# fx-erick/uncertainty-vit

Hardware: AMD Instinct MI355X
Metric: pretrain images/sec (ViT-B/16 224, bs=128/GPU) (higher is better)
Workload: dtype bf16

## Files before the change

### include/uvit.h

```cpp
#ifndef UVIT_H
#define UVIT_H
#include <stddef.h>
#include <stdint.h>

#ifdef __cplusplus
extern "C" {
#endif

#define UVIT_VERSION 100
#define UVIT_MAX_DEPTH 64

typedef struct uvit_engine uvit_engine;
typedef void* uvit_stream;

typedef struct uvit_config {
    int32_t img_size, patch_size, in_chans, embed_dim, depth, num_heads, mlp_hidden;
    int32_t use_shared_rel_pos_bias;
    int32_t use_abs_pos_emb;
    int32_t batch;
    float ln_eps;
    float attn_drop_rate;
    float drop_path_rate;
    int32_t bias_chunk;
    int32_t two_stream;
// ... 3 lines not shown
    char name[96];
    int64_t offset;
    int64_t numel;
    int32_t ndim;
    int32_t decay;
    int64_t shape[4];
} uvit_layout_entry;

typedef struct uvit_buffers {
    float* params;
    float* grads;
    float* adam_m;
    float* adam_v;
    float* ema;
    void* params_bf16;
    void* params_bf16_t;
    void* ema_bf16;
    const int32_t* rel_index;
    void* workspace;
    int64_t workspace_bytes;
} uvit_buffers;

typedef struct uvit_step_params {
    int32_t target_layers[UVIT_MAX_DEPTH];
    int32_t n_target_layers;
    int32_t target_layer_norm_last;
    int32_t post_target_layer_norm;
    int32_t l2_loss;
    float l1_beta;
    float loss_scale;
    float clip_grad;
    float lr, weight_decay, beta1, beta2, eps;
    int32_t opt_step;
    float ema_decay;
    int32_t do_ema;
    float grad_scale;
    uint32_t seed;
    uint32_t it;
    int32_t train_dropout;
    float lambda_pretraining;
    const float* sched_dev;
    int32_t sched_len, sched_index;
    int32_t layer_results_fc;
    float var_w0, var_margin0;
    int32_t target_batch_norm, target_instance_norm, post_target_instance_norm;
    int32_t n_rows_hint;
} uvit_step_params;

int uvit_version(void);
const char* uvit_source_hash(void);

int uvit_layout_count(const uvit_config* cfg);
int uvit_layout_get(const uvit_config* cfg, int index, uvit_layout_entry* out);
int64_t uvit_arena_numel(const uvit_config* cfg, int64_t* n_decay_out);
int64_t uvit_workspace_bytes(const uvit_config* cfg);

uvit_engine* uvit_engine_create(const uvit_config* cfg, const uvit_buffers* bufs, uvit_stream stream, int* err_out);
void uvit_engine_destroy(uvit_engine* e);

int uvit_engine_sync_shadows(uvit_engine* e, int which, uvit_stream stream);

int uvit_engine_forward_features(uvit_engine* e, int which, const float* images, const int64_t* mask, int batch,
                                 int train_dropout, uint32_t seed, uint32_t it, uvit_stream stream);
int uvit_engine_forward_tail(uvit_engine* e, int which, int batch, int first_layer, int train_dropout, uint32_t seed, uint32_t it,
                             uvit_stream stream);
int uvit_engine_head(uvit_engine* e, int which, int all_tokens, float* out, int32_t* count_dev, uvit_stream stream);

void* uvit_engine_ws_ptr(uvit_engine* e, const char* name, int layer);
int uvit_engine_compact_rows(uvit_engine* e);

int uvit_step_begin(uvit_engine* e, const float* images, const int64_t* mask, const uvit_step_params* hp,
                    uvit_stream stream);
int uvit_step_backward_layer(uvit_engine* e, int layer, const uvit_step_params* hp, uvit_stream stream);
int uvit_step_wait_layer_grads(uvit_engine* e, int layer, uvit_stream stream);
int uvit_step_backward_embed(uvit_engine* e, uvit_stream stream);
int uvit_step_update(uvit_engine* e, const uvit_step_params* hp, uvit_stream stream);
int uvit_train_step(uvit_engine* e, const float* images, const int64_t* mask, const uvit_step_params* hp,
                    uvit_stream stream);
typedef struct uvit_tuning { int32_t nt_variant, tn_variant, tn_split_target, wgrad_group_chunks, nt_group, nt_persist; } uvit_tuning;
void uvit_tuning_default(uvit_tuning* out);
int uvit_engine_set_tuning(uvit_engine* e, const uvit_tuning* t);
int uvit_engine_set_streams(uvit_engine* e, int dual);
int uvit_engine_set_drop_path_rows(uvit_engine* e, int on);
int uvit_drop_path_kept_counts(int depth, float drop_path_rate, int draws_per_block, int batch, uint32_t seed, uint32_t it, int32_t* out);
int uvit_engine_profile(uvit_engine* e, int enable, int max_launches);
int uvit_engine_profile_read(uvit_engine* e, double* total_ms, int* launches, double* flops_per_launch);
int uvit_engine_profile_read_kind(uvit_engine* e, int kind, double* total_ms, int* launches, double* flops_per_launch,
                                  double* bytes_per_launch);
int uvit_engine_read_stats_async(uvit_engine* e, float* host_out2, uvit_stream stream);
int uvit_engine_read_stats(uvit_engine* e, float* host_out2, uvit_stream stream);

typedef struct uvit_gemm_epilogue {
    void* out; void* out2; const float* bias; const float* bias2; const float* gamma; const float* resid;
    const float* rowscale; const void* aux; const int64_t* mask; const float* mask_token;
    int32_t ldo, tokens, patches;
    int32_t row0;
} uvit_gemm_epilogue;
enum { UVIT_EPI_BF16 = 0, UVIT_EPI_QKV = 1, UVIT_EPI_GELU = 2, UVIT_EPI_RESID = 3, UVIT_EPI_F32 = 4,
       UVIT_EPI_PATCH = 5, UVIT_EPI_DGELU = 6, UVIT_EPI_QKV_ELU = 7,
       UVIT_EPI_GELU_DG = 8,
       UVIT_EPI_MULAUX = 9 };

int uvit_op_gemm_nt(int mode, const void* A_bf16, const void* W_bf16, int M, int N, int K, int lda, int ldw,
                    const uvit_gemm_epilogue* epi, uvit_stream stream);
int uvit_op_gemm_nt_tuned(int mode, const void* A_bf16, const void* W_bf16, int M, int N, int K, int lda, int ldw,
                          const uvit_gemm_epilogue* epi, const uvit_tuning* tune, int* tail_rows, uvit_stream stream);
typedef struct uvit_gemm_nt_plan_info { int32_t kernel, rows, grid, tail_rows; } uvit_gemm_nt_plan_info;
int uvit_op_gemm_nt_plan(int mode, int M, int N, int K, int lda, int ldw, int ldo, int row_list,
                         const uvit_tuning* tuning, int num_cu, uvit_gemm_nt_plan_info* out);
int uvit_op_gemm_nt_sched(int mode, const void* A_bf16, const void* W_bf16, int M, int N, int K, int lda, int ldw,
                          const uvit_gemm_epilogue* epi, const uvit_tuning* tune, uint32_t* tile_counters, uvit_stream stream);
int uvit_op_gemm_tn(const void* Y_bf16, const void* X_bf16, int M, int N, int K, int ldy, int ldx, float* C, int ldc,
                    const uvit_tuning* tune, uvit_stream stream);
typedef struct uvit_wgrad_problem {
    const void* Y_bf16; const void* X_bf16; float* C; float* bias; float* bias2;
    int32_t bias_end, bias2_begin, M, N, K, ldy, ldx, ldc;
} uvit_wgrad_problem;
int uvit_op_wgrad_group(const uvit_wgrad_problem* problems, int count, const uvit_tuning* tune, uvit_stream stream);
int uvit_op_attn_fwd(const void* qkv, const float* biasP, void* out, float* lse, int B, int H, int N, int NP,
                     float scale, float p_drop, uint32_t seed, uint32_t layer, uvit_stream stream);
int64_t uvit_op_attn_bwd_ws_bytes(int B, int H, int N);
int uvit_op_attn_bwd(const void* qkv, const void* o_fwd, const void* d_o, const float* biasP, const float* lse,
                           float* delta, void* dqkv, float* dbias_slab, int accumulate_slab, void* ds_workspace, int B, int H,
                           int N, int NP, float scale, float p_drop, uint32_t seed, uint32_t layer, uvit_stream stream);
int uvit_op_attn_fwd_hd(const void* qkv, const float* biasP, void* out, float* lse, int B, int H, int N, int NP, int head_dim,
                        float scale, float p_drop, uint32_t seed, uint32_t layer, uvit_stream stream);
int uvit_op_attn_bwd_hd(const void* qkv, const void* o_fwd, const void* d_o, const float* biasP, const float* lse,
                        float* delta, void* dqkv, float* dbias_slab, int accumulate_slab, void* ds_workspace, int B, int H,
                        int N, int NP, int head_dim, float scale, float p_drop, uint32_t seed, uint32_t layer, uvit_stream stream);
int uvit_op_attn2_fwd(const void* qkv_m, const void* qkv_c, const float* biasP, void* out_m, void* out_c, float* lse, int B, int H,
                      int N, int NP, float scale, float p_drop, uint32_t seed, uint32_t layer, uvit_stream stream);
int64_t uvit_op_attn2_bwd_ws_bytes(int B, int H, int N);
int uvit_op_attn2_bwd(const void* qkv_m, const void* qkv_c, const void* o_m, const void* o_c, const void* d_m, const void* d_c,
                      const float* biasP, const float* lse, float* delta, void* dqkv_m, void* dqkv_c, float* dbias_slab,
                      int accumulate_slab, void* ds_workspace, int B, int H, int N, int NP, float scale, float p_drop, uint32_t seed,
                      uint32_t layer, uvit_stream stream);
int uvit_op_relpos_gather(const float* table, const int32_t* index, float* biasP, int H, int N, int NP, uvit_stream stream);
int uvit_op_relpos_scatter(const float* slab, int nslab, const int32_t* index, float* dtable, int H, int N, int NP,
                           uvit_stream stream);
int uvit_op_ln_fwd(const float* x, const float* w, const float* b, void* y_bf16, float* mean, float* rstd, int M, int C,
                   float eps, uvit_stream stream);
int uvit_op_ln_bwd(const void* dy_bf16, const float* x, const float* mean, const float* rstd, const float* w,
                   const float* dres, float* dx, float* dw, float* db, int M, int C, uvit_stream stream);
int uvit_op_ln_fwd_walk(const float* x, const float* w, const float* b, void* y_bf16, float* mean, float* rstd, int M, int C,
                        float eps, const int32_t* rowidx, const int32_t* count, const int32_t* pos, float* xcopy, int tokens,
                        uvit_stream stream);
typedef struct uvit_ls_rider {
    const void* y; const float* gamma; const float* rowscale; void* dy; float* dgamma; float* dbias;
    int32_t tokens; const int32_t* pos; const int32_t* cnt; int32_t pad_base; void* pad2; int32_t pad2_cols;
} uvit_ls_rider;
int uvit_op_ln_bwd_walk(const void* dy_bf16, const float* x, const float* mean, const float* rstd, const float* w, const float* dres,
                        float* dx, float* dw, float* db, int M, int C, int nrep, int64_t rep_stride, const int32_t* rowidx,
                        const int32_t* count, const int32_t* pos, const uvit_ls_rider* next, uvit_stream stream);
int uvit_op_ls_bwd(const float* dx, const uvit_ls_rider* rider, int M, int C, int nrep, int64_t rep_stride, const int32_t* rowidx,
                   const int32_t* count, uvit_stream stream);
int uvit_op_colsum(const void* y_bf16, int ld, int col0, int ncols, int M, float* out, int nrep, int64_t rep_stride, uvit_stream stream);
int uvit_op_reduce_replicas(const float* rep, float* out, int64_t n, int nrep, int64_t stride, uvit_stream stream);
int uvit_op_droppath_lists(const float* scales, int32_t* pos, int32_t* bmap, int32_t* rows, int32_t* cnt, int nlists, int B, int tokens,
                           int rows_stride, const int32_t* host_counts, uvit_stream stream);
int uvit_op_gemm_nt_rows(int mode, const void* A_bf16, const void* W_bf16, int M, int N, int K, int lda, int ldw,
                         const uvit_gemm_epilogue* epi, const int32_t* rowmap, const int32_t* rowcount, const uvit_tuning* tune,
                         uvit_stream stream);
typedef struct uvit_wgrad_split { float* bias_s1; float* bias2_s1; int32_t s1_row; } uvit_wgrad_split;
int uvit_op_wgrad_group_split(const uvit_wgrad_problem* problems, const uvit_wgrad_split* split, int count, const uvit_tuning* tune,
                              uvit_stream stream);
int uvit_op_token_bwd(const float* dx, const int64_t* mask, void* dpatch_bf16, float* dcls, float* dmask_token, int B, int P, int C,
                      uvit_stream stream);
typedef struct uvit_transpose_desc { const void* src; void* dst; int32_t rows, cols, tile0, pad; } uvit_transpose_desc;
int uvit_op_transpose_batch(const uvit_transpose_desc* descs_dev, int ndesc, int total_tiles, uvit_stream stream);
int uvit_op_ema(float* ema, const float* params, void* ema_bf16, int64_t n, float decay, uvit_stream stream);
int uvit_op_sumsq(const float* g, int64_t n, double* out, uvit_stream stream);
int uvit_op_adamw(float* p, const float* g, float* m, float* v, void* p_bf16, int64_t n, int64_t n_decay, float lr,
                  float wd, float b1, float b2, float eps, int step, const double* sumsq, float max_norm,
                  float grad_scale, float* gnorm_out, uvit_stream stream);
int uvit_op_smooth_l1(const float* out, const float* target, const int32_t* count_dev, float beta, int l2,
                      float loss_scale, float* loss, void* dout_bf16, int Mmax, int C, uvit_stream stream);
int uvit_op_wasserstein_loss(const float* out_m, const float* out_c, const float* tgt_m, const float* tgt_c,
                             const int32_t* count_dev, float lam, float loss_scale, float* scratch, float* loss,
                             void* dout_m_bf16, void* dout_c_bf16, int Mmax, int C, uvit_stream stream);
int uvit_op_target_accum(const float* x, const int32_t* rowidx, const int32_t* count, float* acc, int first, int Mmax,
                         int C, float eps, uvit_stream stream);
int uvit_op_variance_loss(const float* out, const int32_t* count_dev, float w, float margin, float loss_scale, float* scratch,
                          float* loss, float* std_loss0_out, void* dout_bf16, int Mmax, int C, uvit_stream stream);
int uvit_op_target_finalize(float* acc, const int32_t* count, int n_layers, int post_ln, int Mmax, int C, float eps,
                            uvit_stream stream);
int uvit_op_mask_compact(const int64_t* mask, int32_t* rowidx, int32_t* count, int B, int P, uvit_stream stream);
int uvit_op_synth_batch(float* images, int64_t* mask, int B, int chans, int img_size, int patches, int n_mask, uint32_t seed,
                        uint32_t it, uvit_stream stream);
int uvit_op_im2col(const float* img, void* cols_bf16, int B, int Cin, int img_size, int patch, uvit_stream stream);
int uvit_op_droppath(float* scales, const float* rates_dev, int depth, int B, uint32_t seed, uint32_t step,
                     uvit_stream stream);
int uvit_op_cast_bf16(const float* src, void* dst_bf16, int64_t n, uvit_stream stream);

#define UVIT_AUG_LANCZOS 1
#define UVIT_AUG_BILINEAR 2
#define UVIT_AUG_BICUBIC 3
#define UVIT_AUG_HAMMING 5
#define UVIT_AUG_BRIGHTNESS 0
#define UVIT_AUG_CONTRAST 1
#define UVIT_AUG_SATURATION 2
typedef struct uvit_augment_desc {
    int64_t offset;
    int32_t h, w;
    int32_t flip;
    int32_t crop_x, crop_y, crop_w, crop_h;
    int32_t resize_w, resize_h;
    int32_t win_x, win_y;
    int32_t filter;
    int32_t n_jitter;
    int32_t jitter_op[3];
    float jitter_factor[3];
    int32_t reserved;
// ... 116 lines not shown
```

### uncertainty-vit_amd/csrc/attention.hip

```cpp
#include <mutex>
#include <type_traits>
#include "attn_common.h"
#include "uvit_internal.h"

#define IMG_PIECES (ROWS_PAD / 8)

#define TAIL_BYTES (ROWS_PAD * 32)
#define TAIL_PIECES (ROWS_PAD / 32)
__device__ __forceinline__ int tail_off(int row, int slot) { return row * 32 + ((slot ^ ((row >> 2) & 2)) << 3); }

__device__ __forceinline__ void dma_tail32(char* tail, int rb, const bf16* src, size_t stride, int n_valid, int lane) {
    const int row = 32 * rb + (lane >> 1);
    const int half = (lane & 1) ^ ((row >> 3) & 1);
    const int r = row < n_valid ? row : n_valid - 1;
    __builtin_amdgcn_global_load_lds(GLB_PTR(void, src + (size_t)r * stride + 64 + half * 8), LDS_PTR(void, tail + rb * 1024), 16, 0, 0);
}

__device__ __forceinline__ bf16x8 tail_row(const char* tail, int row, int g) {
    const bf16x8 v = *(const bf16x8*)(tail + row * 32 + (((g & 1) ^ ((row >> 3) & 1)) << 4));
    const bf16x8 z = {};
    return g < 2 ? v : z;
}
__device__ __forceinline__ bf16x8 col_frag_tail(const char* tail, int r_lo, int r_hi, int lane) {
    const int g = lane >> 4, q = (lane >> 2) & 3, p = lane & 3;
    const s16x4 lo = __builtin_amdgcn_ds_read_tr16_b64_v4i16(LDS_PTR(s16x4, tail + tail_off(r_lo + 4 * g + q, p)));
    const s16x4 hi = __builtin_amdgcn_ds_read_tr16_b64_v4i16(LDS_PTR(s16x4, tail + tail_off(r_hi + 4 * g + q, p)));
    typedef __attribute__((ext_vector_type(8))) short s16x8;
    const s16x8 v = {lo[0], lo[1], lo[2], lo[3], hi[0], hi[1], hi[2], hi[3]};
    return __builtin_bit_cast(bf16x8, v);
}

#ifdef ATTN_DEBUG
extern "C" int uvit_debug_attn_fwd(const void* qkv, const float* biasP, void* out, float* lse, int B, int H, int N, int NP, float scale,
                                   float p_drop, void* stream) {
    return uvit_attn_fwd_launch(qkv, biasP, out, lse, B, H, N, NP, scale, p_drop, 1u, 0u, (hipStream_t)stream, nullptr);
}
#endif

template <int HDK, int NW, bool HAS_BIAS>
__global__ __launch_bounds__(NW * 64, 4)
void attn_fwd_kernel(const bf16* __restrict__ qkv, const float* __restrict__ biasP, bf16* __restrict__ out,
                     float* __restrict__ lse, int H, int N, int NP, float scale, uint32_t drop_thr,
                     float inv_keep, uint32_t drop_key, int ncu, const int* __restrict__ bmap) {
    constexpr int NDT = HDK / 16;
    extern __shared__ __attribute__((aligned(16))) char smem[];
    char* kimg = smem;
    char* vimg = smem + IMG_BYTES;
    char* ktail = smem + 2 * IMG_BYTES;
    char* vtail = ktail + TAIL_BYTES;
    const int tid = threadIdx.x, lane = tid & 63, wave = __builtin_amdgcn_readfirstlane(tid >> 6);
    const int g = lane >> 4, li = lane & 15;
    const int bh = blockIdx.x, b = bh / H, h = bh - b * H;
    const int C = H * HDK;
    const size_t ld = 3 * (size_t)C;
    const bf16* base = qkv + (size_t)b * N * ld + h * HDK;
    const uint32_t bh_rng = (uint32_t)__builtin_amdgcn_readfirstlane(bmap ? bmap[b] * H + h : bh);
    if (blockIdx.x >= (unsigned)ncu && blockIdx.x < 2u * (unsigned)ncu) __builtin_amdgcn_s_sleep(127);
    bf16x8 qn[2];
    if constexpr (HDK == 64) {
        const int q0 = wave * 16 + li, qr0 = q0 < N ? q0 : N - 1;
        qn[0] = *(const bf16x8*)(base + (size_t)qr0 * ld + g * 8);
        qn[1] = *(const bf16x8*)(base + (size_t)qr0 * ld + 32 + g * 8);
    }
    for (int p = wave; p < 2 * IMG_PIECES; p += NW) {
        const int img = p / IMG_PIECES, rb = p - img * IMG_PIECES;
        dma_rows8(smem + img * IMG_BYTES, rb, base + (size_t)(1 + img) * C, ld, 0, N, lane);
    }
    if constexpr (HDK == 80) {
        for (int p = wave; p < 2 * TAIL_PIECES; p += NW) {
            const int img = p / TAIL_PIECES, rb = p - img * TAIL_PIECES;
            dma_tail32(ktail + img * TAIL_BYTES, rb, base + (size_t)(1 + img) * C, ld, N, lane);
        }
    }
    asm volatile("s_waitcnt vmcnt(0)" ::: "memory");
    if constexpr (HDK == 64) { landed(qn[0]); landed(qn[1]); }
    __syncthreads();
    const int nt = (N + 15) >> 4, nt2 = (nt + 1) >> 1;

    for (int qt = wave; qt < nt; qt += NW) {
        const int q = qt * 16 + li;
        bf16x8 qf[2], qtf;
        if constexpr (HDK == 64) {
            qf[0] = qn[0]; qf[1] = qn[1];
        } else {
            const int qr = q < N ? q : N - 1;
            qf[0] = *(const bf16x8*)(base + (size_t)qr * ld + g * 8);
            qf[1] = *(const bf16x8*)(base + (size_t)qr * ld + 32 + g * 8);
            const bf16x8 qt0 = *(const bf16x8*)(base + (size_t)qr * ld + 64 + 8 * (g & 1)), qz = {};
            qtf = g < 2 ? qt0 : qz;
        }
        float s[NT_MAX][4];
#pragma unroll
        for (int t = 0; t < NT_MAX; ++t) {
            if constexpr (HAS_BIAS) {
                if (t < nt) {
                    const float4 bv = *(const float4*)(biasP + ((size_t)h * NP + q) * NP + t * 16 + 4 * g);
                    s[t][0] = bv.x; s[t][1] = bv.y; s[t][2] = bv.z; s[t][3] = bv.w;
                }
            }
        }
        if constexpr (HDK == 64) {
            if (qt + NW < nt) {
                const int q1 = (qt + NW) * 16 + li, qr1 = q1 < N ? q1 : N - 1;
                qn[0] = *(const bf16x8*)(base + (size_t)qr1 * ld + g * 8);
                qn[1] = *(const bf16x8*)(base + (size_t)qr1 * ld + 32 + g * 8);
            }
        }
        float mx = NEG_BIG;
        const float c = scale * LOG2E;
#pragma unroll
        for (int t = 0; t < NT_MAX; ++t) {
            if (t < nt) {
                f32x4 a = {0.f, 0.f, 0.f, 0.f};
                a = __builtin_amdgcn_mfma_f32_16x16x32_bf16(row_frag(kimg, t * 16 + li, g), qf[0], a, 0, 0, 0);
                a = __builtin_amdgcn_mfma_f32_16x16x32_bf16(row_frag(kimg, t * 16 + li, 4 + g), qf[1], a, 0, 0, 0);
                if constexpr (HDK == 80) a = __builtin_amdgcn_mfma_f32_16x16x32_bf16(tail_row(ktail, t * 16 + li, g), qtf, a, 0, 0, 0);
#pragma unroll
                for (int r = 0; r < 4; ++r) {
                    float bb;
                    if constexpr (HAS_BIAS) bb = s[t][r]; else bb = (t * 16 + 4 * g + r) < N ? 0.f : NEG_BIG;
                    const float v = a[r] * c + bb;
                    s[t][r] = v;
                    mx = fmaxf(mx, v);
                }
            } else {
#pragma unroll
                for (int r = 0; r < 4; ++r) s[t][r] = 0.f;
            }
        }
        mx = group_max4(mx);
        float sum = 0.f;
#pragma unroll
        for (int t = 0; t < NT_MAX; ++t) {
            if (t < nt) {
#pragma unroll
                for (int r = 0; r < 4; ++r) {
                    const float p = __builtin_amdgcn_exp2f(s[t][r] - mx);
                    s[t][r] = p;
                    sum += p;
                }
            }
        }
        sum = group_sum4(sum);
        if (g == 0 && q < N) lse[(size_t)bh * N + q] = mx + __builtin_amdgcn_logf(sum);
        f32x4 o[NDT];
#pragma unroll
        for (int dt = 0; dt < NDT; ++dt) o[dt] = f32x4{0.f, 0.f, 0.f, 0.f};
        const uint32_t rowpair = (bh_rng * N + q) * (uint32_t)(NP >> 1);
#pragma unroll
        for (int ks = 0; ks < (NT_MAX + 1) / 2; ++ks) {
            if (ks < nt2) {
                const int t0 = 2 * ks, t1 = 2 * ks + 1;
                float pa[4], pb[4];
#pragma unroll
                for (int r = 0; r < 4; ++r) { pa[r] = s[t0][r]; pb[r] = t1 < NT_MAX ? s[t1 < NT_MAX ? t1 : 0][r] : 0.f; }
                if (drop_thr) {
                    bool k4[4];
                    keep4(drop_key, rowpair, t0 * 16 + 4 * g, drop_thr, k4);
#pragma unroll
                    for (int r = 0; r < 4; ++r) pa[r] = k4[r] ? pa[r] : 0.f;
                    keep4(drop_key, rowpair, t1 * 16 + 4 * g, drop_thr, k4);
#pragma unroll
                    for (int r = 0; r < 4; ++r) pb[r] = k4[r] ? pb[r] : 0.f;
                }
                const bf16x8 pf = pack8(pa, pb);
#pragma unroll
                for (int dt = 0; dt < 4; ++dt) {
                    const bf16x8 vf = col_frag(vimg, t0 * 16, t1 * 16, dt * 16, lane);
                    o[dt] = __builtin_amdgcn_mfma_f32_16x16x32_bf16(vf, pf, o[dt], 0, 0, 0);
                }
                if constexpr (HDK == 80)
                    o[4] = __builtin_amdgcn_mfma_f32_16x16x32_bf16(col_frag_tail(vtail, t0 * 16, t1 * 16, lane), pf, o[4], 0, 0, 0);
            }
        }
        if constexpr (HDK == 64) {
            asm volatile("s_waitcnt vmcnt(0)" ::: "memory");
            landed(qn[0]); landed(qn[1]);
        }
        if (q < N) {
            const float f = inv_keep / sum;
            bf16* dst = out + ((size_t)b * N + q) * C + h * HDK + 4 * g;
#pragma unroll
            for (int dt = 0; dt < NDT; ++dt) {
                bf16x4 v = {f2bf(o[dt][0] * f), f2bf(o[dt][1] * f), f2bf(o[dt][2] * f), f2bf(o[dt][3] * f)};
                *(bf16x4*)(dst + dt * 16) = v;
            }
        }
    }
}

#define FB_WAVES 13
#define FB_ROWS (NT_MAX * 16)
#ifdef ATTN_STAMP
__device__ unsigned long long g_attn_stamps[2048 * 2 * 16 * 2];
#define ASTAMP(k) do { unsigned long long t_; asm volatile("s_memtime %0\n\ts_waitcnt lgkmcnt(0)" : "=s"(t_) :: "memory"); \
        if (lane == 0 && (wave == 0 || wave == 8) && blockIdx.x < 2048) g_attn_stamps[(blockIdx.x * 2 + (wave >> 3)) * 16 + (k)] = t_; } while (0)
#define BSTAMP(k) do { if (i == 3) { unsigned long long t_; asm volatile("s_memtime %0\n\ts_waitcnt lgkmcnt(0)" : "=s"(t_) :: "memory"); \
        if (lane == 0 && (wave == 0 || wave == 8) && blockIdx.x < 2048) g_attn_stamps[2048 * 32 + (blockIdx.x * 2 + (wave >> 3)) * 16 + (k)] = t_; } } while (0)
#define ASTAMP_ID() do { if (lane == 0 && wave == 0 && blockIdx.x < 2048) \
        g_attn_stamps[blockIdx.x * 32 + 15] = __builtin_amdgcn_s_getreg(4 | (31 << 11)) | ((unsigned long long)__builtin_amdgcn_s_getreg(20 | (31 << 11)) << 32); } while (0)
extern "C" int uvit_debug_attn_stamps(unsigned long long* host_out) {
    return hipMemcpyFromSymbol(host_out, HIP_SYMBOL(g_attn_stamps), sizeof(g_attn_stamps)) == hipSuccess ? 0 : -3;
}
extern "C" int uvit_debug_attn_bwd_fused(const void* qkv, const void* o, const void* d_o, const float* biasP, const float* lse, float* delta,
                                         void* dqkv, void* ds_ws, float* slab, int B, int H, int N, float p_drop, void* stream) {
    (void)slab;
    return uvit_attn_bwd_fused_launch(qkv, o, d_o, biasP, lse, delta, dqkv, ds_ws, ds_ws != nullptr, B, H, N, 208, 0.125f, p_drop, 1u, 0u, (hipStream_t)stream, nullptr);
}
#else
#define ASTAMP(k)
#define BSTAMP(k)
#define ASTAMP_ID()
#endif
#define FB_IMG (FB_ROWS * 128)
#define FB_SB (FB_ROWS * 64)

constexpr int fb_lds(int hd) { return hd == 80 ? 4 * FB_IMG + 4 * TAIL_BYTES + 2 * FB_SB : 4 * FB_IMG + 4 * FB_SB; }

__device__ __forceinline__ int sb_off(int q, int slot) {
    const int f = (((q >> 2) & 1) << 2) | (((q >> 3) & 1) << 1) | ((q >> 1) & 1);
    return q * 64 + ((slot ^ f) << 3);
}
__device__ __forceinline__ bf16x8 sb_col_frag(const char* sb, int r_lo, int r_hi, int tt, bool has_hi, int lane) {
    const int g = lane >> 4, q = (lane >> 2) & 3, p = lane & 3;
    const s16x4 lo = __builtin_amdgcn_ds_read_tr16_b64_v4i16(LDS_PTR(s16x4, sb + sb_off(r_lo + 4 * g + q, 4 * tt + p)));
    s16x4 hi = __builtin_amdgcn_ds_read_tr16_b64_v4i16(LDS_PTR(s16x4, sb + sb_off(r_hi + 4 * g + q, 4 * tt + p)));
    if (!has_hi) hi = s16x4{0, 0, 0, 0};
    typedef __attribute__((ext_vector_type(8))) short s16x8;
    const s16x8 v = {lo[0], lo[1], lo[2], lo[3], hi[0], hi[1], hi[2], hi[3]};
    return __builtin_bit_cast(bf16x8, v);
}

template <int HDK, bool HAS_BIAS, int NT_C>
__global__ __launch_bounds__(FB_WAVES * 64)
void attn_bwd_fused_kernel(const bf16* __restrict__ qkv, const bf16* __restrict__ o_fwd, const bf16* __restrict__ d_o,
                           const float* __restrict__ biasP, const float* __restrict__ lse, float* __restrict__ delta,
                           bf16* __restrict__ dqkv, bf16* __restrict__ ds_out, int H, int N, int NP, float scale,
                           uint32_t drop_thr, float inv_keep, uint32_t drop_key, const int* __restrict__ bmap) {
    constexpr int NDT = HDK / 16;
    constexpr int BW = 2 * NDT;
    extern __shared__ __attribute__((aligned(16))) char smem[];
    char* const kimg = smem;
    char* const vimg = smem + FB_IMG;
    char* const qimg = smem + 2 * FB_IMG;
    char* const doimg = smem + 3 * FB_IMG;
    char* const ktail = smem + 4 * FB_IMG;
    char* const vtail = ktail + TAIL_BYTES;
    char* const qtail = ktail + 2 * TAIL_BYTES;
    char* const dotail = ktail + 3 * TAIL_BYTES;
    char* const pbuf = smem + 4 * FB_IMG + 4 * TAIL_BYTES;
    char* const dbuf = pbuf + FB_SB;
    const int tid = threadIdx.x, lane = tid & 63, wave = __builtin_amdgcn_readfirstlane(tid >> 6);
    const int g = lane >> 4, li = lane & 15;
    const int bh = blockIdx.x, b = bh / H, h = bh - b * H;
    const int C = H * HDK;
    const size_t ld = 3 * (size_t)C;
    const int nt = NT_C ? NT_C : (N + 15) >> 4;
    const int nsteps = (nt + 1) >> 1;
    const bf16* base = qkv + (size_t)b * N * ld + h * HDK;
    const bf16* dobase = d_o + (size_t)b * N * C + h * HDK;
    const bool active = NT_C ? true : wave < nt;
    const int q = wave * 16 + li, qr = q < N ? q : N - 1;
    ASTAMP(0); ASTAMP_ID();

    for (int p = wave; p < 4 * (FB_ROWS / 8); p += FB_WAVES) {
        int img, rb;
        if (p < 2 * (FB_ROWS / 8)) { img = p & 1; rb = p >> 1; } else { img = 2 + (p >= 3 * (FB_ROWS / 8)); rb = p - img * (FB_ROWS / 8); }
        if (rb * 8 >= nt * 16) continue;
        if (img == 3) dma_rows8(doimg, rb, dobase, (size_t)C, 0, N, lane);
        else dma_rows8(smem + img * FB_IMG, rb, base + (img == 2 ? 0 : (size_t)(1 + img) * C), ld, 0, N, lane);
    }
    if constexpr (HDK == 80) {
        for (int p = wave; p < 4 * TAIL_PIECES; p += FB_WAVES) {
            const int img = p / TAIL_PIECES, rb = p - img * TAIL_PIECES;
            if (rb * 32 >= nt * 16) continue;
            if (img == 3) dma_tail32(dotail, rb, dobase, (size_t)C, N, lane);
            else dma_tail32(ktail + img * TAIL_BYTES, rb, base + (img == 2 ? 0 : (size_t)(1 + img) * C), ld, N, lane);
        }
    }
    float dl = 0.f, lse_q = 1e30f;
    if (active) {
        const size_t orow = ((size_t)b * N + qr) * C + h * HDK;
#pragma unroll
        for (int kk = 0; kk < 2; ++kk) {
            const bf16x8 dof = *(const bf16x8*)(d_o + orow + kk * 32 + g * 8);
            const bf16x8 of = *(const bf16x8*)(o_fwd + orow + kk * 32 + g * 8);
#pragma unroll
            for (int j = 0; j < 8; ++j) dl += bf2f(dof[j]) * bf2f(of[j]);
        }
        if constexpr (HDK == 80) {
            const bf16x4 dof = *(const bf16x4*)(d_o + orow + 64 + g * 4);
            const bf16x4 of = *(const bf16x4*)(o_fwd + orow + 64 + g * 4);
#pragma unroll
            for (int j = 0; j < 4; ++j) dl += bf2f(dof[j]) * bf2f(of[j]);
        }
        dl = group_sum4(dl);
        if (q < N) {
            lse_q = lse[(size_t)bh * N + q];
            if (g == 0) delta[(size_t)bh * N + q] = dl;
        }
    }
    const uint32_t bh_rng = (uint32_t)__builtin_amdgcn_readfirstlane(bmap ? bmap[b] * H + h : bh);
    const uint32_t rowpair = (bh_rng * N + q) * (uint32_t)(NP >> 1);
    const float cs = scale * LOG2E;
    const float* brow = HAS_BIAS ? biasP + ((size_t)h * NP + (q < NP ? q : NP - 1)) * NP + 4 * g : nullptr;
    float4 bnext[2];
    auto bias_fetch = [&](int i) {
#pragma unroll
        for (int tt = 0; tt < 2; ++tt) {
            const int t = 2 * i + tt;
            if constexpr (HAS_BIAS) {
                bnext[tt] = (t < nt && active) ? *(const float4*)(brow + t * 16) : make_float4(NEG_BIG, NEG_BIG, NEG_BIG, NEG_BIG);
            } else {
                const int k0 = t * 16 + 4 * g;
                bnext[tt] = make_float4(k0 < N ? 0.f : NEG_BIG, k0 + 1 < N ? 0.f : NEG_BIG, k0 + 2 < N ? 0.f : NEG_BIG, k0 + 3 < N ? 0.f : NEG_BIG);
            }
        }
    };
    bias_fetch(0);
    asm volatile("s_waitcnt vmcnt(0)" ::: "memory");
    ASTAMP(1);
    __syncthreads();
    ASTAMP(2);

    f32x4 dq[NDT];
#pragma unroll
    for (int dt = 0; dt < NDT; ++dt) dq[dt] = f32x4{0.f, 0.f, 0.f, 0.f};
    const int pj = HDK == 64 ? wave >> 2 : wave / 5, dtj = HDK == 64 ? wave & 3 : wave - 5 * pj;

    enum { A_COMPUTE = 1, A_FINISH = 2 };
    float step_p[2][4], step_ds[2][4];
    auto A_step = [&](int i, auto parts, float (&pdv)[2][4], float (&dsv)[2][4]) {
        char* pb = HDK == 64 ? smem + 4 * FB_IMG + (i & 1) * FB_SB : pbuf;
        char* db = HDK == 64 ? pb + 2 * FB_SB : dbuf;
        const int t0 = 2 * i;
        const bool has1 = t0 + 1 < nt;
        if constexpr (decltype(parts)::value & A_COMPUTE) {
            const float4 bcur[2] = {bnext[0], bnext[1]};
            if (i + 1 < nsteps) bias_fetch(i + 1);
            BSTAMP(4);
            bool k4[2][4] = {{true, true, true, true}, {true, true, true, true}};
#ifndef ATTN_HAZARD_DEMO
            if (drop_thr) {
                keep4(drop_key, rowpair, t0 * 16 + 4 * g, drop_thr, k4[0]);
                keep4(drop_key, rowpair, t0 * 16 + 16 + 4 * g, drop_thr, k4[1]);
            }
#endif
            BSTAMP(5);
            const int row0 = t0 * 16 + li, row1 = (has1 ? t0 + 1 : t0) * 16 + li;
            f32x4 sacc[2], dp[2];
            {
                const bf16x8 k00 = row_frag(kimg, row0, g), k01 = row_frag(kimg, row0, 4 + g);
                const bf16x8 k10 = row_frag(kimg, row1, g), k11 = row_frag(kimg, row1, 4 + g);
                const bf16x8 qf0 = row_frag(qimg, q, g), qf1 = row_frag(qimg, q, 4 + g);
                const f32x4 z = {0.f, 0.f, 0.f, 0.f};
                sacc[0] = __builtin_amdgcn_mfma_f32_16x16x32_bf16(k00, qf0, z, 0, 0, 0);
                sacc[1] = __builtin_amdgcn_mfma_f32_16x16x32_bf16(k10, qf0, z, 0, 0, 0);
                sacc[0] = __builtin_amdgcn_mfma_f32_16x16x32_bf16(k01, qf1, sacc[0], 0, 0, 0);
                sacc[1] = __builtin_amdgcn_mfma_f32_16x16x32_bf16(k11, qf1, sacc[1], 0, 0, 0);
                if constexpr (HDK == 80) {
                    const bf16x8 qt = tail_row(qtail, q, g);
                    sacc[0] = __builtin_amdgcn_mfma_f32_16x16x32_bf16(tail_row(ktail, row0, g), qt, sacc[0], 0, 0, 0);
                    sacc[1] = __builtin_amdgcn_mfma_f32_16x16x32_bf16(tail_row(ktail, row1, g), qt, sacc[1], 0, 0, 0);
                }
            }
            __builtin_amdgcn_sched_barrier(0);
            BSTAMP(6);
            {
                const bf16x8 v00 = row_frag(vimg, row0, g), v01 = row_frag(vimg, row0, 4 + g);
                const bf16x8 v10 = row_frag(vimg, row1, g), v11 = row_frag(vimg, row1, 4 + g);
                const bf16x8 do0 = row_frag(doimg, q, g), do1 = row_frag(doimg, q, 4 + g);
                const f32x4 z = {0.f, 0.f, 0.f, 0.f};
                dp[0] = __builtin_amdgcn_mfma_f32_16x16x32_bf16(v00, do0, z, 0, 0, 0);
                dp[1] = __builtin_amdgcn_mfma_f32_16x16x32_bf16(v10, do0, z, 0, 0, 0);
                dp[0] = __builtin_amdgcn_mfma_f32_16x16x32_bf16(v01, do1, dp[0], 0, 0, 0);
                dp[1] = __builtin_amdgcn_mfma_f32_16x16x32_bf16(v11, do1, dp[1], 0, 0, 0);
                if constexpr (HDK == 80) {
                    const bf16x8 dot = tail_row(dotail, q, g);
                    dp[0] = __builtin_amdgcn_mfma_f32_16x16x32_bf16(tail_row(vtail, row0, g), dot, dp[0], 0, 0, 0);
                    dp[1] = __builtin_amdgcn_mfma_f32_16x16x32_bf16(tail_row(vtail, row1, g), dot, dp[1], 0, 0, 0);
                }
            }
            BSTAMP(7);
#ifdef ATTN_HAZARD_DEMO
            if (drop_thr) {
                keep4(drop_key, rowpair, t0 * 16 + 4 * g, drop_thr, k4[0]);
                keep4(drop_key, rowpair, t0 * 16 + 16 + 4 * g, drop_thr, k4[1]);
            }
#endif
#pragma unroll
            for (int tt = 0; tt < 2; ++tt) {
                const float bb[4] = {bcur[tt].x, bcur[tt].y, bcur[tt].z, bcur[tt].w};
#pragma unroll
                for (int r = 0; r < 4; ++r) {
                    const float p = __builtin_amdgcn_exp2f(sacc[tt][r] * cs + bb[r] - lse_q);
                    const float pd = k4[tt][r] ? p * inv_keep : 0.f;
                    pdv[tt][r] = pd;
                    dsv[tt][r] = pd * dp[tt][r] - p * dl;
                }
            }
        }
        if constexpr (decltype(parts)::value & A_FINISH) {
#pragma unroll
            for (int tt = 0; tt < 2; ++tt) {
                if (tt == 0 || has1) {
                    const bf16x4 pv = {f2bf(pdv[tt][0]), f2bf(pdv[tt][1]), f2bf(pdv[tt][2]), f2bf(pdv[tt][3])};
                    const bf16x4 dv = {f2bf(dsv[tt][0]), f2bf(dsv[tt][1]), f2bf(dsv[tt][2]), f2bf(dsv[tt][3])};
                    *(bf16x4*)(pb + sb_off(q, 4 * tt + g)) = pv;
                    *(bf16x4*)(db + sb_off(q, 4 * tt + g)) = dv;
                }
            }
            const bf16x8 dsf = pack8(dsv[0], dsv[1]);
            __builtin_amdgcn_sched_barrier(0);
            BSTAMP(8);
#pragma unroll
            for (int dt = 0; dt < 4; ++dt) {
                const bf16x8 kt = col_frag(kimg, t0 * 16, has1 ? t0 * 16 + 16 : t0 * 16, dt * 16, lane);
                dq[dt] = __builtin_amdgcn_mfma_f32_16x16x32_bf16(kt, dsf, dq[dt], 0, 0, 0);
            }
            if constexpr (HDK == 80)
                dq[4] = __builtin_amdgcn_mfma_f32_16x16x32_bf16(col_frag_tail(ktail, t0 * 16, has1 ? t0 * 16 + 16 : t0 * 16, lane),
                                                                 dsf, dq[4], 0, 0, 0);
            BSTAMP(9);
        }
    };

    auto B_step = [&](int i) {
        const char* pb = HDK == 64 ? smem + 4 * FB_IMG + (i & 1) * FB_SB : pbuf;
        const char* sb = pj ? (HDK == 64 ? pb + 2 * FB_SB : dbuf) : pb;
        const char* img = pj ? qimg : doimg;
        const char* timg = pj ? qtail : dotail;
        const bool has1 = 2 * i + 1 < nt;
        f32x4 acc[2] = {f32x4{0.f, 0.f, 0.f, 0.f}, f32x4{0.f, 0.f, 0.f, 0.f}};
        auto kstep = [&](int ks, auto is_tail) {
            const bool hk = 2 * ks + 1 < nt;
            const int r_lo = 32 * ks, r_hi = hk ? r_lo + 16 : r_lo;
            bf16x8 a;
            if constexpr (decltype(is_tail)::value) a = col_frag_tail(timg, r_lo, r_hi, lane);
            else a = col_frag(img, r_lo, r_hi, dtj * 16, lane);
            const bf16x8 b0 = sb_col_frag(sb, r_lo, r_hi, 0, hk, lane);
            const bf16x8 b1 = sb_col_frag(sb, r_lo, r_hi, 1, hk, lane);
            acc[0] = __builtin_amdgcn_mfma_f32_16x16x32_bf16(a, b0, acc[0], 0, 0, 0);
            acc[1] = __builtin_amdgcn_mfma_f32_16x16x32_bf16(a, b1, acc[1], 0, 0, 0);
        };
        auto kloop = [&](auto is_tail) {
            if constexpr (NT_C != 0) {
#pragma unroll
                for (int ks = 0; ks < (NT_C + 1) / 2; ++ks) kstep(ks, is_tail);
            } else {
                for (int ks = 0; ks < nsteps; ++ks) kstep(ks, is_tail);
            }
        };
        if constexpr (HDK == 80) {
            if (dtj == 4) kloop(std::true_type{});
            else kloop(std::false_type{});
        } else if constexpr (NT_C != 0) {
#pragma unroll
            for (int ks = 0; ks < (NT_C + 1) / 2; ++ks) kstep(ks, std::false_type{});
        } else {
            for (int ks = 0; ks < nsteps; ++ks) kstep(ks, std::false_type{});
        }
        HAZARD_PAD();
        char* dst = pj ? kimg : vimg;
        char* tdst = pj ? ktail : vtail;
        const float sc = pj ? scale : 1.0f;
#pragma unroll
        for (int tt = 0; tt < 2; ++tt) {
            if (tt == 0 || has1) {
                const int row = 32 * i + 16 * tt + li;
                const bf16x4 v = {f2bf(acc[tt][0] * sc), f2bf(acc[tt][1] * sc), f2bf(acc[tt][2] * sc), f2bf(acc[tt][3] * sc)};
                if (HDK == 80 && dtj == 4) *(bf16x4*)(tdst + tail_off(row, g)) = v;
                else *(bf16x4*)(dst + img_off(row, 2 * dtj + (g >> 1)) + ((g & 1) << 3)) = v;
            }
        }
    };
    auto store_rows = [&](int i, int sw) {
        for (int c = sw; c < 2 * NDT; c += FB_WAVES - BW) {
            if (HDK == 80 && c >= 8) {
                const int img = c - 8, row = 32 * i + (lane >> 1), hl = lane & 1;
// ... 38 lines not shown
            if (i > 0) stream_ds(i - 1, sw);
            BSTAMP(2);
            if constexpr (HDK == 64) if (i < nsteps && active) A_step(i, Both{}, step_p, step_ds);
        }
        if constexpr (HDK == 80) {
            if (i < nsteps && active) A_step(i, Compute{}, step_p, step_ds);
            asm volatile("s_waitcnt lgkmcnt(0)" ::: "memory");
            __builtin_amdgcn_s_barrier();
            asm volatile("" ::: "memory");
            if (i < nsteps && active) A_step(i, Finish{}, step_p, step_ds);
        }
        asm volatile("s_waitcnt lgkmcnt(0)" ::: "memory");
        BSTAMP(10);
        __builtin_amdgcn_s_barrier();
        asm volatile("" ::: "memory");
        BSTAMP(11);
        ASTAMP(3 + i);
    }
    if (wave >= BW) store_rows(nsteps - 1, wave - BW);
    if (active) {
        if constexpr (HDK == 80) {
            const bf16x4 v = {f2bf(dq[4][0] * scale), f2bf(dq[4][1] * scale), f2bf(dq[4][2] * scale), f2bf(dq[4][3] * scale)};
            if (q < N) *(bf16x4*)(dqkv + ((size_t)b * N + q) * ld + h * HDK + 64 + 4 * g) = v;
        }
#pragma unroll
        for (int dt = 0; dt < 4; ++dt) {
            const bf16x4 v = {f2bf(dq[dt][0] * scale), f2bf(dq[dt][1] * scale), f2bf(dq[dt][2] * scale), f2bf(dq[dt][3] * scale)};
            *(bf16x4*)(qimg + img_off(q, 2 * dt + (g >> 1)) + ((g & 1) << 3)) = v;
        }
        asm volatile("s_waitcnt lgkmcnt(0)" ::: "memory");
#pragma unroll
        for (int k = 0; k < 2; ++k) {
            const int row = wave * 16 + (lane >> 3) + 8 * k, ch = lane & 7;
            const uint4 v = *(const uint4*)(qimg + img_off(row, ch));
            if (row < N) *(uint4*)(dqkv + ((size_t)b * N + row) * ld + h * HDK + ch * 8) = v;
        }
    }
    ASTAMP(13);
}

#define DBR_PARTS 4
__global__ __launch_bounds__(256)
void attn_dbias_reduce_kernel(const bf16* __restrict__ ds, float* __restrict__ slab, int B, int H, int N, int NP) {
    __shared__ float tile[32][65];
    const int nt = (N + 15) >> 4, nsteps = (nt + 1) >> 1;
    const int qb = blockIdx.x & 3, hi = blockIdx.x >> 2, i = hi % nsteps, h = hi / nsteps;
    const int tid = threadIdx.x, ql = tid >> 2, c = tid & 3, q = qb * 64 + ql;
    const int per = (B + DBR_PARTS - 1) / DBR_PARTS, b0 = blockIdx.y * per, b1 = min(B, b0 + per);
    float acc[8];
#pragma unroll
    for (int j = 0; j < 8; ++j) acc[j] = 0.f;
    if (q < N) {
        const char* p = (const char*)ds + ((size_t)h * nsteps + i) * FB_SB + q * 64 + c * 16;
        const size_t bstride = (size_t)H * nsteps * FB_SB;
#pragma unroll 8
        for (int b = b0; b < b1; ++b) {
            const bf16x8 v = *(const bf16x8*)(p + b * bstride);
#pragma unroll
            for (int j = 0; j < 8; ++j) acc[j] += bf2f(v[j]);
        }
    }
    const int f = (((q >> 2) & 1) << 2) | (((q >> 3) & 1) << 1) | ((q >> 1) & 1);
#pragma unroll
    for (int e = 0; e < 2; ++e) {
        const int slot = (2 * c + e) ^ f;
#pragma unroll
        for (int j = 0; j < 4; ++j) tile[4 * slot + j][ql] = acc[4 * e + j];
    }
    __syncthreads();
    const int lane = tid & 63, w = tid >> 6, qo = qb * 64 + lane;
#pragma unroll
    for (int k = 0; k < 8; ++k) {
        const int key = 32 * i + w * 8 + k;
        if (key < N && qo < N) atomicAdd(slab + ((size_t)h * NP + key) * NP + qo, tile[w * 8 + k][lane]);
    }
}


#define FWD_WAVES 7
constexpr int fwd_lds(int hd) { return 2 * IMG_BYTES + (hd == 80 ? 2 * TAIL_BYTES : 0); }

template <int HDK>
struct AttnKernels {
    static auto fwd(bool has_bias) { return has_bias ? attn_fwd_kernel<HDK, FWD_WAVES, true> : attn_fwd_kernel<HDK, FWD_WAVES, false>; }
    static auto bwd(bool has_bias, bool full) {
        if (full) return has_bias ? attn_bwd_fused_kernel<HDK, true, NT_MAX> : attn_bwd_fused_kernel<HDK, false, NT_MAX>;
        return has_bias ? attn_bwd_fused_kernel<HDK, true, 0> : attn_bwd_fused_kernel<HDK, false, 0>;
    }
    static void lds_init() {
        for (bool has_bias : {false, true}) {
            (void)hipFuncSetAttribute((const void*)fwd(has_bias), hipFuncAttributeMaxDynamicSharedMemorySize, fwd_lds(HDK));
            for (bool full : {false, true})
                (void)hipFuncSetAttribute((const void*)bwd(has_bias, full), hipFuncAttributeMaxDynamicSharedMemorySize, fb_lds(HDK));
        }
    }
};

static std::once_flag g_attn_once;
static int g_attn_ncu = 256;
static void attn_init_impl() {
    int dev = 0; hipDeviceProp_t prop;
    if (hipGetDevice(&dev) == hipSuccess && hipGetDeviceProperties(&prop, dev) == hipSuccess && prop.multiProcessorCount > 0)
        g_attn_ncu = prop.multiProcessorCount;
    AttnKernels<64>::lds_init();
    AttnKernels<80>::lds_init();
}
static void attn_init_once() { std::call_once(g_attn_once, attn_init_impl); }

static int attn_check(int B, int H, int N, int head_dim) {
    if ((head_dim != 64 && head_dim != 80) || B <= 0 || H <= 0 || N <= 0 || N > NT_MAX * 16) return UVIT_ERR_SHAPE;
    return UVIT_OK;
}

template <int HDK>
static void attn_fwd_go(const void* qkv, const float* biasP, void* out, float* lse, int B, int H, int N, int NP, float scale,
                        uint32_t thr, float inv_keep, uint32_t key, hipStream_t s, const int* bmap) {
    hipLaunchKernelGGL(AttnKernels<HDK>::fwd(biasP != nullptr), dim3(B * H), dim3(FWD_WAVES * 64), fwd_lds(HDK), s, (const bf16*)qkv,
                       biasP, (bf16*)out, lse, H, N, NP, scale, thr, inv_keep, key, g_attn_ncu, bmap);
}

int uvit_attn_fwd_launch(const void* qkv, const float* biasP, void* out, float* lse, int B, int H, int N, int NP,
                         float scale, float p_drop, uint32_t seed, uint32_t layer, hipStream_t s, const int* bmap, int head_dim) {
    int rc = attn_check(B, H, N, head_dim); if (rc) return rc;
    attn_init_once();
    const uint32_t thr = p_drop > 0.f ? uvit_drop_threshold16(p_drop) : 0u;
    const float inv_keep = p_drop > 0.f ? 1.0f / (1.0f - p_drop) : 1.0f;
    const uint32_t key = uvit_layer_key(seed, layer);
    if (head_dim == 80) attn_fwd_go<80>(qkv, biasP, out, lse, B, H, N, NP, scale, thr, inv_keep, key, s, bmap);
    else attn_fwd_go<64>(qkv, biasP, out, lse, B, H, N, NP, scale, thr, inv_keep, key, s, bmap);
    return uvit_check_launch();
}

size_t uvit_attn_bwd_fused_ws_bytes(int B, int H, int N) {
    const int nt = (N + 15) / 16, nsteps = (nt + 1) / 2;
    return (size_t)B * H * nsteps * FB_SB;
}

template <int HDK>
static void attn_bwd_go(const void* qkv, const void* o_fwd, const void* d_o, const float* biasP, const float* lse, float* delta,
                        void* dqkv, bf16* dsw, int B, int H, int N, int NP, float scale, uint32_t thr, float inv_keep, uint32_t key,
                        hipStream_t s, const int* bmap) {
    hipLaunchKernelGGL(AttnKernels<HDK>::bwd(biasP != nullptr, (N + 15) / 16 == NT_MAX), dim3(B * H), dim3(FB_WAVES * 64), fb_lds(HDK), s,
                       (const bf16*)qkv, (const bf16*)o_fwd, (const bf16*)d_o, biasP, lse, delta, (bf16*)dqkv, dsw, H, N, NP, scale, thr,
                       inv_keep, key, bmap);
}

int uvit_attn_bwd_fused_launch(const void* qkv, const void* o_fwd, const void* d_o, const float* biasP, const float* lse,
                               float* delta, void* dqkv, void* ds_ws, int want_ds, int B, int H, int N, int NP, float scale,
                               float p_drop, uint32_t seed, uint32_t layer, hipStream_t s, const int* bmap, int head_dim) {
    int rc = attn_check(B, H, N, head_dim); if (rc) return rc;
    if (NP < NT_MAX * 16 || (want_ds && !ds_ws)) return UVIT_ERR_ARG;
    attn_init_once();
    const uint32_t thr = p_drop > 0.f ? uvit_drop_threshold16(p_drop) : 0u;
    const float inv_keep = p_drop > 0.f ? 1.0f / (1.0f - p_drop) : 1.0f;
    const uint32_t key = uvit_layer_key(seed, layer);
    bf16* dsw = want_ds ? (bf16*)ds_ws : nullptr;
    if (head_dim == 80) attn_bwd_go<80>(qkv, o_fwd, d_o, biasP, lse, delta, dqkv, dsw, B, H, N, NP, scale, thr, inv_keep, key, s, bmap);
    else attn_bwd_go<64>(qkv, o_fwd, d_o, biasP, lse, delta, dqkv, dsw, B, H, N, NP, scale, thr, inv_keep, key, s, bmap);
    return uvit_check_launch();
}

int uvit_attn_dbias_reduce_launch(const void* ds_ws, float* dbias_slab, int accumulate, int B, int H, int N, int NP, hipStream_t s) {
    int rc = attn_check(B, H, N, 64); if (rc) return rc;
    if (!ds_ws || !dbias_slab || NP < NT_MAX * 16) return UVIT_ERR_ARG;
    if (!accumulate) { rc = uvit_zero_launch(dbias_slab, (size_t)H * NP * NP * sizeof(float), s); if (rc) return rc; }
    const int nt = (N + 15) / 16, nsteps = (nt + 1) / 2;
    hipLaunchKernelGGL(attn_dbias_reduce_kernel, dim3(H * nsteps * 4, DBR_PARTS), dim3(256), 0, s, (const bf16*)ds_ws, dbias_slab, B, H, N, NP);
    return uvit_check_launch();
}
```

### uncertainty-vit_amd/csrc/attn_common.h

```cpp
#pragma once
#include "common.h"

#ifdef ATTN_NO_HAZARD_PAD
#define HAZARD_PAD()
#else
#define HAZARD_PAD() asm volatile("s_nop 15\n\ts_nop 7" ::: "memory")
#endif
#define NT_MAX 13
#define ROWS_PAD 224
#define IMG_BYTES (ROWS_PAD * 128)
#define LOG2E 1.4426950408889634f
#define NEG_BIG (-1e30f)

__device__ __forceinline__ int img_off(int row, int chunk) { return row * 128 + ((chunk ^ (row & 7)) << 4); }

__device__ __forceinline__ bf16x8 row_frag(const char* img, int row, int chunk) {
    return *(const bf16x8*)(img + img_off(row, chunk));
}

__device__ __forceinline__ bf16x8 col_frag(const char* img, int r_lo, int r_hi, int col0, int lane) {
    const int g = lane >> 4, q = (lane >> 2) & 3, p = lane & 3;
    const int chunk = (col0 >> 3) + (p >> 1), within = (p & 1) << 3;
    const int ra = r_lo + 4 * g + q, rb = r_hi + 4 * g + q;
    const s16x4 lo = __builtin_amdgcn_ds_read_tr16_b64_v4i16(LDS_PTR(s16x4, img + img_off(ra, chunk) + within));
    const s16x4 hi = __builtin_amdgcn_ds_read_tr16_b64_v4i16(LDS_PTR(s16x4, img + img_off(rb, chunk) + within));
    typedef __attribute__((ext_vector_type(8))) short s16x8;
    const s16x8 v = {lo[0], lo[1], lo[2], lo[3], hi[0], hi[1], hi[2], hi[3]};
    return __builtin_bit_cast(bf16x8, v);
}

__device__ __forceinline__ void dma_rows8(char* img, int rb, const bf16* src, size_t stride, int row0, int n_valid, int lane) {
    const int row = row0 + 8 * rb + (lane >> 3);
    const int chunk = (lane & 7) ^ (lane >> 3);
    const int r = row < n_valid ? row : n_valid - 1;
    __builtin_amdgcn_global_load_lds(GLB_PTR(void, src + (size_t)r * stride + chunk * 8), LDS_PTR(void, img + rb * 1024), 16, 0, 0);
}

__device__ __forceinline__ void landed(bf16x8& v) { asm volatile("" : "+v"(v)); }

__device__ __forceinline__ bf16x8 pack8(const float* a, const float* b) {
    bf16x8 v = {f2bf(a[0]), f2bf(a[1]), f2bf(a[2]), f2bf(a[3]), f2bf(b[0]), f2bf(b[1]), f2bf(b[2]), f2bf(b[3])};
    return v;
}

__device__ __forceinline__ uint32_t pair_hash(uint32_t key32, uint32_t pidx) {
    uint32_t x = (pidx ^ key32) * 0x9E3779B1u;
    x ^= x >> 15; x *= 0x85EBCA77u; x ^= x >> 13;
    return x;
}
__device__ __forceinline__ void keep4(uint32_t key32, uint32_t rowpair, int kbase, uint32_t thr16, bool (&k)[4]) {
    const uint32_t h0 = pair_hash(key32, rowpair + (kbase >> 1)), h1 = pair_hash(key32, rowpair + (kbase >> 1) + 1);
    k[0] = (h0 & 0xFFFFu) >= thr16; k[1] = (h0 >> 16) >= thr16;
    k[2] = (h1 & 0xFFFFu) >= thr16; k[3] = (h1 >> 16) >= thr16;
}
__device__ __forceinline__ bool keep1(uint32_t key32, uint32_t rowpair, int key, uint32_t thr16) {
    const uint32_t h = pair_hash(key32, rowpair + (key >> 1));
    return ((key & 1) ? (h >> 16) : (h & 0xFFFFu)) >= thr16;
}

__device__ __forceinline__ float group_sum4(float v) {
    v += __shfl_xor(v, 16, 64);
    v += __shfl_xor(v, 32, 64);
    return v;
}
__device__ __forceinline__ float group_max4(float v) {
    v = fmaxf(v, __shfl_xor(v, 16, 64));
    v = fmaxf(v, __shfl_xor(v, 32, 64));
    return v;
}
```

### uncertainty-vit_amd/csrc/engine.hip

```cpp
#include <hip/hip_runtime.h>
#include <math.h>
#include <stdio.h>
#include <stdlib.h>
#include <string.h>

#include <string>
#include <vector>

#include "../../include/uvit.h"
#include "common.h"
#include "uvit_internal.h"

#define CHECK(x) do { int _rc = (x); if (_rc) return _rc; } while (0)
#define NREP 32
#define RP(off) (e->grep + ((off) - e->lo.n_decay))
#define HIPCHECK(x) do { if ((x) != hipSuccess) return UVIT_ERR_LAUNCH; } while (0)
#define GEMM_NT(...) uvit_gemm_nt_launch(__VA_ARGS__, &e->tune)
#define GEMM_TN(...) uvit_gemm_tn_launch(__VA_ARGS__, &e->tune)
#define GEMM_TN_GROUP(...) uvit_gemm_tn_group_launch(__VA_ARGS__, &e->tune)

struct LayerOff { size_t n1w, n1b, qkvw, qb[2], vb[2], projw[2], projb[2], g1, n2w, n2b, fc1w, fc1b, fc2w, fc2b, g2, cqkvw; };
struct Layout {
    size_t cls[2], mask_tok[2], pew[2], peb[2], relt, normw, normb, lmw[2], lmb[2], pos;
    LayerOff L[UVIT_MAX_DEPTH];
    size_t n_total, n_decay, n_live;
    std::vector<uvit_layout_entry> entries;
};

static size_t align64(size_t x) { return (x + 63) & ~(size_t)63; }

static int cfg_ok(const uvit_config* c) {
    if (!c) return UVIT_ERR_ARG;
    if (c->depth < 1 || c->depth > UVIT_MAX_DEPTH || c->num_heads < 1) return UVIT_ERR_SHAPE;
    if (c->embed_dim != c->num_heads * 64 && (c->two_stream || c->embed_dim != c->num_heads * 80)) return UVIT_ERR_SHAPE;
    if (c->embed_dim % 64 || c->mlp_hidden % 64 || c->patch_size % 8 || c->img_size % c->patch_size) return UVIT_ERR_SHAPE;
    if ((c->in_chans * c->patch_size * c->patch_size) % 64) return UVIT_ERR_SHAPE;
    const int g = c->img_size / c->patch_size;
    if (g * g + 1 > 208 || c->batch < 1) return UVIT_ERR_SHAPE;
    if (c->use_abs_pos_emb && c->two_stream) return UVIT_ERR_SHAPE;
    return UVIT_OK;
}

static void build_layout(const uvit_config* c, Layout& lo) {
    const int64_t C = c->embed_dim, Hd = c->mlp_hidden, g = c->img_size / c->patch_size;
    size_t off = 0;
    auto add = [&](const std::string& name, std::vector<int64_t> shape, int decay) -> size_t {
        uvit_layout_entry e;
        memset(&e, 0, sizeof(e));
        snprintf(e.name, sizeof(e.name), "%s", name.c_str());
        e.offset = (int64_t)off; e.ndim = (int)shape.size(); e.decay = decay; e.numel = 1;
        for (size_t i = 0; i < shape.size(); ++i) { e.shape[i] = shape[i]; e.numel *= shape[i]; }
        lo.entries.push_back(e);
        const size_t at = off;
        off = align64(off + (size_t)e.numel);
        return at;
    };
    auto blk = [](int i, const char* s) { return "blocks." + std::to_string(i) + "." + s; };
    const bool two = c->two_stream != 0;
    lo.mask_tok[0] = add("mask_token", {1, 1, C}, 1);
    if (two) lo.mask_tok[1] = add("cov_mask_token", {1, 1, C}, 1);
    if (two) lo.cls[1] = add("cov_cls_token", {1, 1, C}, 1);
    if (c->use_shared_rel_pos_bias) lo.relt = add("rel_pos_bias.relative_position_bias_table", {(2 * g - 1) * (2 * g - 1) + 3, c->num_heads}, 1);
    else lo.relt = (size_t)-1;
    lo.pew[0] = add("patch_embed.proj.weight", {C, c->in_chans, c->patch_size, c->patch_size}, 1);
    if (two) lo.pew[1] = add("cov_patch_embed.proj.weight", {C, c->in_chans, c->patch_size, c->patch_size}, 1);
    for (int i = 0; i < c->depth; ++i) {
        lo.L[i].qkvw = add(blk(i, "attn.qkv.weight"), {3 * C, C}, 1);
        lo.L[i].projw[0] = add(blk(i, "attn.proj.weight"), {C, C}, 1);
        if (two) lo.L[i].projw[1] = add(blk(i, "attn.cov_proj.weight"), {C, C}, 1);
        lo.L[i].fc1w = add(blk(i, "mlp.fc1.weight"), {Hd, C}, 1);
        lo.L[i].fc2w = add(blk(i, "mlp.fc2.weight"), {C, Hd}, 1);
    }
    lo.lmw[0] = add("lm_head.weight", {C, C}, 1);
    if (two) lo.lmw[1] = add("cov_lm_head.weight", {C, C}, 1);
    lo.n_decay = off;
    lo.cls[0] = add("cls_token", {1, 1, C}, 0);
    lo.pos = c->use_abs_pos_emb ? add("pos_embed", {1, g * g + 1, C}, 0) : (size_t)-1;
    lo.peb[0] = add("patch_embed.proj.bias", {C}, 0);
    if (two) lo.peb[1] = add("cov_patch_embed.proj.bias", {C}, 0);
    for (int i = 0; i < c->depth; ++i) {
        lo.L[i].g1 = add(blk(i, "gamma_1"), {C}, 0);
        lo.L[i].g2 = add(blk(i, "gamma_2"), {C}, 0);
        lo.L[i].n1w = add(blk(i, "norm1.weight"), {C}, 0);
        lo.L[i].n1b = add(blk(i, "norm1.bias"), {C}, 0);
        lo.L[i].qb[0] = add(blk(i, "attn.q_bias"), {C}, 0);
        lo.L[i].vb[0] = add(blk(i, "attn.v_bias"), {C}, 0);
        if (two) { lo.L[i].qb[1] = add(blk(i, "attn.cov_q_bias"), {C}, 0); lo.L[i].vb[1] = add(blk(i, "attn.cov_v_bias"), {C}, 0); }
        lo.L[i].projb[0] = add(blk(i, "attn.proj.bias"), {C}, 0);
        if (two) lo.L[i].projb[1] = add(blk(i, "attn.cov_proj.bias"), {C}, 0);
        lo.L[i].n2w = add(blk(i, "norm2.weight"), {C}, 0);
        lo.L[i].n2b = add(blk(i, "norm2.bias"), {C}, 0);
        lo.L[i].fc1b = add(blk(i, "mlp.fc1.bias"), {Hd}, 0);
        lo.L[i].fc2b = add(blk(i, "mlp.fc2.bias"), {C}, 0);
    }
    lo.normw = add("norm.weight", {C}, 0);
    lo.normb = add("norm.bias", {C}, 0);
    lo.lmb[0] = add("lm_head.bias", {C}, 0);
    if (two) lo.lmb[1] = add("cov_lm_head.bias", {C}, 0);
    lo.n_live = off;
    if (two)
        for (int i = 0; i < c->depth; ++i) lo.L[i].cqkvw = add(blk(i, "attn.cov_qkv.weight"), {3 * C, C}, 2);
    lo.n_total = off;
}

struct LayerActs {
    bf16 *ln1, *qkv, *attn, *projout, *ln2, *h, *a, *mlpout;
    float *mean1, *rstd1, *mean2, *rstd2, *lse;
};

struct uvit_engine {
    uvit_config cfg;
    uvit_buffers buf;
    Layout lo;
    int B, P, N, NP, C, Hd, H, Kpe, M, Mpad, BP, BPpad;
    int head_dim;
    float attn_scale;
    int S;
    GemmTune tune;
    int cur_B;
    int tail_which = -1, tail_B = 0, tail_first = 0;
    bf16* cols;
    float* X[UVIT_MAX_DEPTH + 1];
    float* XM[UVIT_MAX_DEPTH];
    LayerActs acts[UVIT_MAX_DEPTH];
    LayerActs tacts;
    float *tX[2], *tXM;
    int *rowidx, *count;
    bf16 *normed[2], *dout[2], *dnormed[2], *dpatch[2];
    float *meanF[2], *rstdF[2], *outputs[2], *targets[2];
    float *biasP_s, *biasP_t, *slabs, *delta;
    void* ds_ws[2] = {nullptr, nullptr};
    float *dXa, *dXb;
    bf16 *dY1[2], *dY2[2], *dH[2], *dLN, *dAttn, *dqkv[2];
    float *dp_scales, *dp_rates;
    int *dpl_pos = nullptr, *dpl_bmap = nullptr, *dpl_rows = nullptr, *dpl_cnt = nullptr;
    size_t dpl_stride = 0;
    int dpl_K[128] = {};
    bool dpl_enable = true;
    bool dpl_on = false;
    std::vector<float> dp_rates_host;
    float *loss, *gnorm; double* sumsq;
    float* wl_scratch;
    float *dense_v, *dense_acc; int *idrows, *idcount;
    float* var_scratch;
    int* poisoned;
    TransposeDesc* tdesc; int n_tdesc, n_ttiles;
    int64_t* mask_copy;
    unsigned* tile_cnt = nullptr;
    float* grep;
    size_t n_nd;
    bool slab_started;
    bool last_dropout; uint32_t last_seed;
    int bwd_next = -1;
    int compact_R = 0;
    bool dual = true;
    hipStream_t aux = nullptr, aux_eq = nullptr, aux_lo = nullptr;
    hipEvent_t ev_fork = nullptr, ev_teacher = nullptr, ev_x = nullptr;
    hipEvent_t ev_wdone[UVIT_MAX_DEPTH] = {};
    hipEvent_t ev_ds = nullptr;
    bool prof_on = false;
    std::vector<hipEvent_t> prof_ev;
    std::vector<int> prof_kind;
    std::vector<int> prof_rows;
    size_t prof_used = 0;
    size_t rows_all() const { return (size_t)(S - 1) * Mpad + M; }
    size_t rows_alloc() const { return (size_t)S * Mpad; }
};

struct Bump {
    char* base; size_t off, cap;
    template <typename T> T* take(size_t n) {
        off = (off + 255) & ~(size_t)255;
        T* p = base ? (T*)(base + off) : nullptr;
        off += n * sizeof(T);
        return p;
    }
};

static size_t roundup(size_t x, size_t m) { return (x + m - 1) / m * m; }
static std::vector<float> dp_rates_linspace(int depth, float rate);

static void plan_workspace(uvit_engine* e, Bump& b) {
    const uvit_config& c = e->cfg;
    const size_t Mp = e->rows_alloc(), C = e->C, Hd = e->Hd, BPp = e->BPpad;
    auto acts = [&](LayerActs& a) {
        a.ln1 = b.take<bf16>(Mp * C); a.qkv = b.take<bf16>(Mp * 3 * C); a.attn = b.take<bf16>(Mp * C);
        a.projout = b.take<bf16>(Mp * C); a.ln2 = b.take<bf16>(Mp * C); a.h = b.take<bf16>(Mp * Hd);
        a.a = b.take<bf16>(Mp * Hd); a.mlpout = b.take<bf16>(Mp * C);
        a.mean1 = b.take<float>(Mp); a.rstd1 = b.take<float>(Mp); a.mean2 = b.take<float>(Mp); a.rstd2 = b.take<float>(Mp);
        a.lse = b.take<float>((size_t)e->B * e->H * e->N);
    };
    e->cols = b.take<bf16>(BPp * e->Kpe);
    for (int i = 0; i <= c.depth; ++i) e->X[i] = b.take<float>(Mp * C);
    for (int i = 0; i < c.depth; ++i) { e->XM[i] = b.take<float>(Mp * C); acts(e->acts[i]); }
    acts(e->tacts);
    e->tX[0] = b.take<float>(Mp * C); e->tX[1] = b.take<float>(Mp * C); e->tXM = b.take<float>(Mp * C);
    e->rowidx = b.take<int>(e->BP + 64); e->count = b.take<int>(64);
    for (int st = 0; st < e->S; ++st) {
        e->normed[st] = b.take<bf16>(BPp * C); e->dout[st] = b.take<bf16>(BPp * C); e->dnormed[st] = b.take<bf16>(BPp * C);
        e->dpatch[st] = b.take<bf16>(BPp * C);
        e->meanF[st] = b.take<float>(BPp); e->rstdF[st] = b.take<float>(BPp);
        e->outputs[st] = b.take<float>(BPp * C); e->targets[st] = b.take<float>(BPp * C);
    }
    const size_t bias_n = (size_t)e->H * e->NP * e->NP;
    e->biasP_s = b.take<float>(bias_n); e->biasP_t = b.take<float>(bias_n);
    e->slabs = b.take<float>(bias_n);
    e->delta = b.take<float>((size_t)e->B * e->H * e->N);
    if (e->cfg.use_shared_rel_pos_bias)
        for (int k = 0; k < 2; ++k)
            e->ds_ws[k] = b.take<char>(e->S == 1 ? uvit_attn_bwd_fused_ws_bytes(e->B, e->H, e->N) : uvit_attn2_bwd_ws_bytes(e->B, e->H, e->N));
    e->dXa = b.take<float>(Mp * C); e->dXb = b.take<float>(Mp * C);
    for (int k = 0; k < 2; ++k) {
        e->dY1[k] = b.take<bf16>(Mp * C); e->dY2[k] = b.take<bf16>(Mp * C); e->dH[k] = b.take<bf16>(Mp * Hd);
        e->dqkv[k] = b.take<bf16>(Mp * 3 * C);
    }
    e->dLN = b.take<bf16>(Mp * C); e->dAttn = b.take<bf16>(Mp * C);
    e->dp_scales = b.take<float>((size_t)c.depth * 2 * e->S * e->B); e->dp_rates = b.take<float>(c.depth);
    if ((size_t)c.depth * 2 * e->S <= 128) {
        const size_t nl = (size_t)c.depth * 2 * e->S;
        e->dpl_stride = roundup((size_t)e->B * e->N, 64);
        e->dpl_pos = b.take<int>(nl * e->B); e->dpl_bmap = b.take<int>(nl * e->B);
        e->dpl_rows = b.take<int>(nl * e->dpl_stride); e->dpl_cnt = b.take<int>(2 * nl + 64);
    }
    e->loss = b.take<float>(64); e->gnorm = e->loss + 1; e->sumsq = (double*)(e->loss + 2);
    e->wl_scratch = b.take<float>(16 + BPp);
    e->poisoned = b.take<int>(64);
    e->var_scratch = b.take<float>(2 * C + 16);
    e->dense_v = b.take<float>(BPp * C); e->dense_acc = b.take<float>(BPp * C);
    e->idrows = b.take<int>(e->BP + 64); e->idcount = b.take<int>(64);
    e->tdesc = b.take<TransposeDesc>(7 * c.depth + 4);
    e->mask_copy = b.take<int64_t>(e->BP + 64);
    e->grep = b.take<float>((size_t)NREP * e->n_nd);
    e->tile_cnt = b.take<unsigned>(64);
}

// ... 11 lines not shown
    e->n_nd = tmp_lo.n_live - tmp_lo.n_decay;
}

extern "C" void uvit_engine_destroy(uvit_engine* e);
extern "C" int uvit_version(void) { return UVIT_VERSION; }
#ifndef UVIT_SRC_HASH
#define UVIT_SRC_HASH "unknown"
#endif
extern "C" const char* uvit_source_hash(void) { return UVIT_SRC_HASH; }

extern "C" int uvit_layout_count(const uvit_config* cfg) {
    if (cfg_ok(cfg)) return UVIT_ERR_SHAPE;
    Layout lo; build_layout(cfg, lo);
    return (int)lo.entries.size();
}
extern "C" int uvit_layout_get(const uvit_config* cfg, int index, uvit_layout_entry* out) {
    if (cfg_ok(cfg) || !out) return UVIT_ERR_SHAPE;
    Layout lo; build_layout(cfg, lo);
    if (index < 0 || index >= (int)lo.entries.size()) return UVIT_ERR_ARG;
    *out = lo.entries[index];
    return UVIT_OK;
}
extern "C" int64_t uvit_arena_numel(const uvit_config* cfg, int64_t* n_decay_out) {
    if (cfg_ok(cfg)) return UVIT_ERR_SHAPE;
    Layout lo; build_layout(cfg, lo);
    if (n_decay_out) *n_decay_out = (int64_t)lo.n_decay;
    return (int64_t)lo.n_total;
}
extern "C" int64_t uvit_workspace_bytes(const uvit_config* cfg) {
    if (cfg_ok(cfg)) return UVIT_ERR_SHAPE;
    uvit_engine tmp;
    tmp.cfg = *cfg;
    fill_dims(&tmp);
    Bump b{nullptr, 0, 0};
    plan_workspace(&tmp, b);
    return (int64_t)roundup(b.off, 4096) + 4096;
}

extern "C" uvit_engine* uvit_engine_create(const uvit_config* cfg, const uvit_buffers* bufs, uvit_stream stream, int* err_out) {
    auto fail = [&](int rc) -> uvit_engine* { if (err_out) *err_out = rc; return nullptr; };
    if (cfg_ok(cfg) || !bufs) return fail(UVIT_ERR_SHAPE);
    if (!bufs->params || !bufs->grads || !bufs->adam_m || !bufs->adam_v || !bufs->ema || !bufs->params_bf16 ||
        !bufs->params_bf16_t || !bufs->ema_bf16 || !bufs->workspace) return fail(UVIT_ERR_ARG);
    if (cfg->use_shared_rel_pos_bias && !bufs->rel_index) return fail(UVIT_ERR_ARG);
    if (bufs->workspace_bytes < uvit_workspace_bytes(cfg)) return fail(UVIT_ERR_WORKSPACE);
    uvit_engine* e = new uvit_engine();
    e->cfg = *cfg; e->buf = *bufs;
    fill_dims(e);
    build_layout(cfg, e->lo);
    Bump b{(char*)bufs->workspace, 0, (size_t)bufs->workspace_bytes};
    plan_workspace(e, b);
    hipStream_t s = (hipStream_t)stream;
    if (hipMemsetAsync(bufs->workspace, 0, b.off, s) != hipSuccess) { delete e; return fail(UVIT_ERR_LAUNCH); }
    std::vector<float> rates = dp_rates_linspace(cfg->depth, cfg->drop_path_rate);
    e->dp_rates_host = rates;
    if (const char* v = getenv("UVIT_DP_ROWS")) e->dpl_enable = v[0] != '0';
    std::vector<TransposeDesc> td;
    int tiles = 0;
    const char* src = (const char*)bufs->params_bf16; char* dst = (char*)bufs->params_bf16_t;
    auto addT = [&](size_t off, int rows, int cols) {
        TransposeDesc d; d.src = src + off * 2; d.dst = dst + off * 2; d.rows = rows; d.cols = cols; d.tile0 = tiles; d.pad = 0;
        tiles += ((rows + 63) / 64) * ((cols + 63) / 64);
        td.push_back(d);
    };
    for (int i = 0; i < cfg->depth; ++i) {
        addT(e->lo.L[i].qkvw, 3 * e->C, e->C); addT(e->lo.L[i].projw[0], e->C, e->C);
        addT(e->lo.L[i].fc1w, e->Hd, e->C); addT(e->lo.L[i].fc2w, e->C, e->Hd);
        if (e->S == 2) addT(e->lo.L[i].projw[1], e->C, e->C);
    }
    for (int st = 0; st < e->S; ++st) addT(e->lo.lmw[st], e->C, e->C);
    e->n_tdesc = (int)td.size(); e->n_ttiles = tiles;
    {
        std::vector<int> idr(e->BP);
        for (int i = 0; i < e->BP; ++i) idr[i] = i;
        const int cnt = e->BP;
        if (hipMemcpyAsync(e->idrows, idr.data(), idr.size() * sizeof(int), hipMemcpyHostToDevice, s) != hipSuccess ||
            hipMemcpyAsync(e->idcount, &cnt, sizeof(int), hipMemcpyHostToDevice, s) != hipSuccess ||
            hipStreamSynchronize(s) != hipSuccess) { delete e; return fail(UVIT_ERR_LAUNCH); }
    }
    if (hipMemcpyAsync(e->dp_rates, rates.data(), rates.size() * sizeof(float), hipMemcpyHostToDevice, s) != hipSuccess ||
        hipMemcpyAsync(e->tdesc, td.data(), td.size() * sizeof(TransposeDesc), hipMemcpyHostToDevice, s) != hipSuccess ||
        hipStreamSynchronize(s) != hipSuccess) { delete e; return fail(UVIT_ERR_LAUNCH); }
    e->slab_started = false; e->last_dropout = false; e->last_seed = 0;
    {
        const char* env = getenv("UVIT_SINGLE_STREAM");
        e->dual = !(env && env[0] == '1');
        int lo = 0, hi = 0; (void)hipDeviceGetStreamPriorityRange(&lo, &hi);
        bool ok = hipStreamCreateWithFlags(&e->aux_eq, hipStreamNonBlocking) == hipSuccess &&
                  hipStreamCreateWithPriority(&e->aux_lo, hipStreamNonBlocking, lo) == hipSuccess;
        e->aux = e->aux_eq;
        auto mk = [&](hipEvent_t* ev) { ok = ok && hipEventCreateWithFlags(ev, hipEventDisableTiming) == hipSuccess; };
        mk(&e->ev_fork); mk(&e->ev_teacher); mk(&e->ev_ds); mk(&e->ev_x);
        for (int i = 0; i < cfg->depth; ++i) mk(&e->ev_wdone[i]);
        if (!ok) { uvit_engine_destroy(e); return fail(UVIT_ERR_LAUNCH); }
    }
    if (err_out) *err_out = UVIT_OK;
    return e;
}

extern "C" void uvit_engine_destroy(uvit_engine* e) {
    if (!e) return;
    for (hipEvent_t ev : e->prof_ev) (void)hipEventDestroy(ev);
    if (e->aux_eq) { (void)hipStreamSynchronize(e->aux_eq); (void)hipStreamDestroy(e->aux_eq); }
    if (e->aux_lo) { (void)hipStreamSynchronize(e->aux_lo); (void)hipStreamDestroy(e->aux_lo); }
    if (e->ev_fork) (void)hipEventDestroy(e->ev_fork);
    if (e->ev_teacher) (void)hipEventDestroy(e->ev_teacher);
    if (e->ev_ds) (void)hipEventDestroy(e->ev_ds);
    if (e->ev_x) (void)hipEventDestroy(e->ev_x);
    for (int i = 0; i < UVIT_MAX_DEPTH; ++i) if (e->ev_wdone[i]) (void)hipEventDestroy(e->ev_wdone[i]);
    delete e;
}

static int tune_from_abi(const uvit_tuning* t, GemmTune& g) {
    if (!t) { g = GemmTune(); return UVIT_OK; }
    if ((t->nt_variant != 0 && t->nt_variant != 1 && t->nt_variant != 3 && t->nt_variant != 5 && t->nt_variant != 6 && t->nt_variant != 7) ||
        (t->tn_variant != 0 && t->tn_variant != 1 && t->tn_variant != 3) || t->tn_split_target < 0 || t->wgrad_group_chunks < 0 || t->nt_group < 0 || t->nt_group > 64 || (t->nt_persist != 0 && t->nt_persist != 1))
        return UVIT_ERR_ARG;
    g.nt_variant = t->nt_variant; g.tn_variant = t->tn_variant;
    g.tn_target = t->tn_split_target > 0 ? t->tn_split_target : 512; g.group_chunks = t->wgrad_group_chunks; g.nt_group = t->nt_group; g.nt_persist = t->nt_persist;
    return UVIT_OK;
}

extern "C" void uvit_tuning_default(uvit_tuning* out) {
    if (!out) return;
    const GemmTune d;
    out->nt_variant = d.nt_variant; out->tn_variant = d.tn_variant; out->tn_split_target = d.tn_target; out->wgrad_group_chunks = d.group_chunks; out->nt_group = d.nt_group; out->nt_persist = d.nt_persist;
}

extern "C" int uvit_engine_set_tuning(uvit_engine* e, const uvit_tuning* t) {
    if (!e) return UVIT_ERR_ARG;
    return tune_from_abi(t, e->tune);
}

extern "C" int uvit_engine_set_streams(uvit_engine* e, int dual) {
    if (!e || dual < 0 || dual > 2) return UVIT_ERR_ARG;
    hipStream_t next = dual == 2 ? e->aux_lo : e->aux_eq;
    if (next != e->aux && e->aux) HIPCHECK(hipStreamSynchronize(e->aux));
    e->aux = next;
    e->dual = dual != 0;
    return UVIT_OK;
}

extern "C" int uvit_engine_set_drop_path_rows(uvit_engine* e, int on) {
    if (!e) return UVIT_ERR_ARG;
    e->dpl_enable = on != 0;
    return UVIT_OK;
}

extern "C" int uvit_engine_profile(uvit_engine* e, int enable, int max_launches) {
    if (!e) return UVIT_ERR_ARG;
    if (enable && e->prof_ev.empty()) {
        e->prof_ev.resize((size_t)(max_launches > 0 ? max_launches : 4096) * 2);
        e->prof_kind.assign(e->prof_ev.size() / 2, -1);
        e->prof_rows.assign(e->prof_ev.size() / 2, 0);
        for (auto& ev : e->prof_ev) if (hipEventCreate(&ev) != hipSuccess) return UVIT_ERR_LAUNCH;
    }
    e->prof_on = enable != 0;
    if (enable) e->prof_used = 0;
    return UVIT_OK;
}

enum { UVIT_PROF_FC1_T = 0, UVIT_PROF_FC1_S = 1, UVIT_PROF_PROJ = 2, UVIT_PROF_FC2 = 3, UVIT_PROF_KINDS = 4 };

extern "C" int uvit_engine_profile_read_kind(uvit_engine* e, int kind, double* total_ms, int* launches, double* flops_per_launch,
                                             double* bytes_per_launch) {
    if (!e || !total_ms || !launches || kind >= UVIT_PROF_KINDS) return UVIT_ERR_ARG;
    double t = 0.0, rows = 0.0; int n = 0;
    for (size_t i = 0; i + 1 < e->prof_used; i += 2) {
        const int k = e->prof_kind[i / 2];
        if (kind < 0 ? (k != UVIT_PROF_FC1_T && k != UVIT_PROF_FC1_S) : k != kind) continue;
        float ms = 0.f;
        if (hipEventElapsedTime(&ms, e->prof_ev[i], e->prof_ev[i + 1]) != hipSuccess) return UVIT_ERR_LAUNCH;
        t += ms; ++n; rows += e->prof_rows[i / 2];
    }
    *total_ms = t; *launches = n;
    const double M1 = n ? rows / n : (double)e->cur_B * e->N, Mall = M1, C = e->C, Hd = e->Hd;
    double fl = 0.0, by = 0.0;
    if (kind < 0 || kind == UVIT_PROF_FC1_T || kind == UVIT_PROF_FC1_S) {
        fl = 2.0 * Mall * Hd * C;
        by = 2.0 * (Mall * C + Hd * C + Mall * Hd * (kind == UVIT_PROF_FC1_T ? 1.0 : kind == UVIT_PROF_FC1_S ? 2.0 : 1.5));
    } else if (kind == UVIT_PROF_PROJ) {
        fl = 2.0 * M1 * C * C;
        by = 2.0 * (M1 * C + C * C) + 8.0 * M1 * C;
    } else {
        fl = 2.0 * M1 * C * Hd;
        by = 2.0 * (M1 * Hd + C * Hd) + 8.0 * M1 * C;
    }
    if (flops_per_launch) *flops_per_launch = fl;
    if (bytes_per_launch) *bytes_per_launch = by;
    return UVIT_OK;
}
extern "C" int uvit_engine_profile_read(uvit_engine* e, double* total_ms, int* launches, double* flops_per_launch) {
    return uvit_engine_profile_read_kind(e, -1, total_ms, launches, flops_per_launch, nullptr);
}

extern "C" int uvit_engine_sync_shadows(uvit_engine* e, int which, uvit_stream stream) {
    if (!e) return UVIT_ERR_ARG;
    hipStream_t s = (hipStream_t)stream;
    if (which & 1) {
        CHECK(uvit_cast_bf16_launch(e->buf.params, e->buf.params_bf16, e->lo.n_total, s));
        CHECK(uvit_transpose_batch_launch(e->tdesc, e->n_tdesc, e->n_ttiles, s));
    }
    if (which & 2) CHECK(uvit_cast_bf16_launch(e->buf.ema, e->buf.ema_bf16, e->lo.n_total, s));
    return UVIT_OK;
}

struct Weights { const float* f; const bf16* b; };
static Weights weights_of(const uvit_engine* e, int which) {
    return which ? Weights{e->buf.ema, (const bf16*)e->buf.ema_bf16} : Weights{e->buf.params, (const bf16*)e->buf.params_bf16};
}

static int dp_draw(const uvit_engine* e, int l, int st, int branch) { return 2 * e->S * l + 2 * st + branch; }
static const float* dp_ptr(uvit_engine* e, bool on, int l, int st, int branch, int Bc) {
    return on ? e->dp_scales + (size_t)dp_draw(e, l, st, branch) * Bc : nullptr;
}

struct DpList { const int *pos, *bmap, *rows, *cnt; int K; };
static void dp_list_get(const uvit_engine* e, int l, int st, int branch, DpList& d) {
    const int lb = dp_draw(e, l, st, branch);
    d.pos = e->dpl_pos + (size_t)lb * e->B; d.bmap = e->dpl_bmap + (size_t)lb * e->B;
    d.rows = e->dpl_rows + (size_t)lb * e->dpl_stride; d.cnt = e->dpl_cnt + lb; d.K = e->dpl_K[lb];
}
static void dp_kept_counts(const float* rates, int depth, int nbr, int B, uint32_t seed, uint32_t it, int* out) {
    for (int l = 0; l < depth; ++l)
        for (int br = 0; br < nbr; ++br) {
            const float r = rates[l];
            int K = B;
            if (r > 0.f) {
// ... 37 lines not shown
enum Pass { PASS_DENSE, PASS_TEACHER, PASS_STUDENT };
struct BranchRows {
    RowMode mode = ROWS_ALL;
    int K = 0;
    int n[2] = {0, 0};
    size_t off[2] = {0, 0};
    int rows = 0;
    int red = 0;
    DpList d[2] = {};
    const int* rowmap[2] = {nullptr, nullptr};
    const int* rowcnt[2] = {nullptr, nullptr};
};
static BranchRows branch_rows(const uvit_engine* e, int l, int branch, Pass pass, int Bc) {
    const int S = e->S;
    BranchRows r;
    r.K = Bc; r.n[0] = r.n[1] = Bc * e->N; r.off[1] = e->Mpad;
    if (pass != PASS_DENSE && branch == 1 && l == e->cfg.depth - 1 && e->compact_R > 0) {
        r.mode = ROWS_MASKED; r.n[0] = e->compact_R; r.rowmap[0] = e->rowidx; r.rowcnt[0] = e->count;
    } else if (pass == PASS_STUDENT && e->dpl_on && (S == 1 || branch == 1)) {
        DpList d[2] = {};
        bool none = false, some = false;
        for (int st = 0; st < S; ++st) {
            dp_list_get(e, l, st, branch, d[st]);
            none = none || d[st].K == 0; some = some || d[st].K < e->B;
        }
        if (!none && some) {
            r.mode = S == 1 ? ROWS_LIST : ROWS_LIST2;
            r.K = d[0].K;
            for (int st = 0; st < S; ++st) { r.d[st] = d[st]; r.n[st] = d[st].K * e->N; r.rowmap[st] = d[st].rows; r.rowcnt[st] = d[st].cnt; }
            r.off[1] = r.n[0];
        }
    }
    r.rows = (int)(r.off[S - 1] + r.n[S - 1]);
    r.red = (int)roundup(r.rows, 64);
    return r;
}

struct Draw { bool on; uint32_t seed, it; };
struct FwdPass {
    Pass kind;
    Pass rows;
    int which;
    Weights w;
    float* biasP;
    unsigned* tile_cnt;
    Draw draw;
    bool dp_on; float pdrop;
    uint32_t aseed;
    int Bc; hipStream_t s;
    const uvit_step_params* hp;
    bool dense;
};
static FwdPass fwd_pass(uvit_engine* e, Pass kind, int which, int Bc, Draw draw, const uvit_step_params* hp, hipStream_t s) {
    FwdPass p;
    p.kind = kind; p.which = which; p.w = weights_of(e, which); p.biasP = which ? e->biasP_t : e->biasP_s;
    p.tile_cnt = e->tile_cnt + (kind == PASS_TEACHER ? 16 : 0);
    const bool train = draw.on && !which;
    p.dp_on = train && e->cfg.drop_path_rate > 0.f; p.pdrop = train ? e->cfg.attn_drop_rate : 0.f;
    p.aseed = uvit_hash32(draw.seed ^ (draw.it * 0x85EBCA6Bu + 0x1234567u));
    p.draw = draw; p.Bc = Bc; p.s = s; p.hp = hp;
    p.dense = hp && (hp->target_batch_norm || hp->target_instance_norm || hp->post_target_instance_norm || !hp->target_layer_norm_last);
    p.rows = p.dense ? PASS_DENSE : kind;
    return p;
}

static int forward_layer(uvit_engine* e, const FwdPass& p, int l, const float* x_in, float* x_mid, float* x_out, LayerActs& a) {
    const LayerOff& o = e->lo.L[l];
    const Weights& w = p.w; hipStream_t s = p.s;
    const int Bc = p.Bc, M = Bc * e->N, C = e->C, Hd = e->Hd, S = e->S;
    const size_t Mp = e->Mpad;
    const bool save = p.kind == PASS_STUDENT;
    const BranchRows at = branch_rows(e, l, 0, p.rows, Bc), ml = branch_rows(e, l, 1, p.rows, Bc);
    LnFwd n1; n1.x = x_in; n1.w = w.f + o.n1w; n1.b = w.f + o.n1b; n1.y = a.ln1; n1.mean = a.mean1; n1.rstd = a.rstd1; n1.M = at.rows; n1.C = C;
    n1.eps = e->cfg.ln_eps;
    if (at.mode == ROWS_LIST) { n1.pos = at.d[0].pos; n1.xcopy = x_mid; n1.tokens = e->N; n1.M = M; }
    CHECK(uvit_ln_fwd_launch(n1, s));
    for (int st = 0; st < S; ++st) {
        GemmEpi q; q.out = a.qkv + at.off[st] * 3 * C; q.bias = w.f + o.qb[st]; q.bias2 = w.f + o.vb[st]; q.ldo = 3 * C;
        q.tile_counter = p.tile_cnt;
        CHECK(GEMM_NT(st ? EPI_QKV_ELU : EPI_QKV, a.ln1 + at.off[st] * C, w.b + o.qkvw, at.n[st], 3 * C, C, C, C, &q, s));
    }
    if (S == 1) {
        CHECK(uvit_attn_fwd_launch(a.qkv, p.biasP, a.attn, a.lse, at.K, e->H, e->N, e->NP, e->attn_scale, p.pdrop, p.aseed, (uint32_t)l, s, at.d[0].bmap,
                                   e->head_dim));
    } else {
        CHECK(uvit_attn2_fwd_launch(a.qkv, a.qkv + Mp * 3 * C, p.biasP, a.attn, a.attn + Mp * C, a.lse, Bc, e->H, e->N, e->NP, 0.125f,
                                    p.pdrop, p.aseed, (uint32_t)l, s));
    }
    auto prof_begin = [&](int kind, int rows) -> bool {
        if (!(e->prof_on && e->prof_used + 2 <= e->prof_ev.size())) return false;
        e->prof_kind[e->prof_used / 2] = kind; e->prof_rows[e->prof_used / 2] = rows;
        (void)hipEventRecord(e->prof_ev[e->prof_used], s);
        return true;
    };
    auto prof_end = [&](bool on) { if (on) { (void)hipEventRecord(e->prof_ev[e->prof_used + 1], s); e->prof_used += 2; } };
    for (int st = 0; st < S; ++st) {
        GemmEpi pj; pj.out = x_mid + st * Mp * C; pj.out2 = save ? a.projout + st * Mp * C : nullptr; pj.bias = w.f + o.projb[st];
        pj.gamma = w.f + o.g1; pj.resid = x_in + st * Mp * C; pj.rowscale = dp_ptr(e, p.dp_on, l, st, 0, Bc); pj.ldo = C; pj.tokens = e->N;
        pj.rowmap = at.rowmap[st]; pj.rowcount = at.rowcnt[st];
        const bool pp = prof_begin(UVIT_PROF_PROJ, at.n[st]);
        CHECK(GEMM_NT(EPI_RESID, a.attn + at.off[st] * C, w.b + o.projw[st], at.n[st], C, C, C, C, &pj, s));
        prof_end(pp);
    }
    LnFwd n2; n2.x = x_mid; n2.w = w.f + o.n2w; n2.b = w.f + o.n2b; n2.y = a.ln2; n2.mean = a.mean2; n2.rstd = a.rstd2; n2.M = ml.rows; n2.C = C;
    n2.eps = e->cfg.ln_eps;
    if (ml.mode == ROWS_LIST || ml.mode == ROWS_LIST2) {
        n2.tokens = e->N; n2.M = M;
        for (int st = 0; st < S; ++st) {
            n2.x = x_mid + st * Mp * C; n2.pos = ml.d[st].pos; n2.xcopy = x_out + st * Mp * C;
            n2.y = a.ln2 + ml.off[st] * C; n2.mean = a.mean2 + ml.off[st]; n2.rstd = a.rstd2 + ml.off[st];
            CHECK(uvit_ln_fwd_launch(n2, s));
        }
    } else {
        n2.rowidx = ml.rowmap[0]; n2.count = ml.rowcnt[0];
        CHECK(uvit_ln_fwd_launch(n2, s));
    }
    GemmEpi f1; f1.out = a.a; f1.out2 = save ? a.h : nullptr; f1.bias = w.f + o.fc1b; f1.ldo = Hd; f1.tile_counter = p.tile_cnt;
    const bool prof = prof_begin(save ? UVIT_PROF_FC1_S : UVIT_PROF_FC1_T, ml.rows);
    CHECK(GEMM_NT(save ? EPI_GELU_DG : EPI_GELU, a.ln2, w.b + o.fc1w, ml.rows, Hd, C, C, C, &f1, s));
    prof_end(prof);
    for (int st = 0; st < S; ++st) {
        GemmEpi f2; f2.out = x_out + st * Mp * C; f2.out2 = save ? a.mlpout + st * Mp * C : nullptr; f2.bias = w.f + o.fc2b;
        f2.gamma = w.f + o.g2; f2.resid = x_mid + st * Mp * C; f2.rowscale = dp_ptr(e, p.dp_on, l, st, 1, Bc); f2.ldo = C; f2.tokens = e->N;
        f2.rowmap = ml.rowmap[st]; f2.rowcount = ml.rowcnt[st];
        const bool pf2 = prof_begin(UVIT_PROF_FC2, ml.n[st]);
        CHECK(GEMM_NT(EPI_RESID, a.a + ml.off[st] * Hd, w.b + o.fc2w, ml.n[st], C, Hd, Hd, Hd, &f2, s));
        prof_end(pf2);
    }
    return UVIT_OK;
}

static int embed(uvit_engine* e, const Weights& w, const int64_t* mask, float* x0, int Bc, hipStream_t s) {
    for (int st = 0; st < e->S; ++st) {
        float* x = x0 + (size_t)st * e->Mpad * e->C;
        GemmEpi pe; pe.out = x; pe.bias = w.f + e->lo.peb[st]; pe.mask = mask; pe.mask_token = w.f + e->lo.mask_tok[st]; pe.ldo = e->C; pe.patches = e->P;
        CHECK(GEMM_NT(EPI_PATCH, e->cols, w.b + e->lo.pew[st], Bc * e->P, e->C, e->Kpe, e->Kpe, e->Kpe, &pe, s));
        CHECK(uvit_set_cls_launch(x, w.f + e->lo.cls[st], nullptr, Bc, e->N, e->C, s));
        if (e->cfg.use_abs_pos_emb) CHECK(uvit_add_pos_launch(x, w.f + e->lo.pos, Bc, e->N, e->C, s));
    }
    return UVIT_OK;
}

struct TargetBuild { bool dense; int n; };
static int targets_after_layer(uvit_engine* e, const FwdPass& p, TargetBuild& t, int l, const float* xout) {
    const uvit_step_params* hp = p.hp; const int Bc = p.Bc; hipStream_t s = p.s;
    if (t.dense && Bc != e->B) return UVIT_ERR_ARG;
    for (int k = 0; k < hp->n_target_layers; ++k) {
        if (hp->target_layers[k] != l) continue;
        const float* sub = hp->layer_results_fc ? e->tXM : nullptr;
        for (int st = t.dense ? 1 : 0; st < e->S; ++st)
            CHECK(uvit_target_accum_launch(xout + (size_t)st * e->Mpad * e->C, e->rowidx, e->count, e->targets[st], t.n == 0,
                                           Bc * e->P, e->C, 1e-5f, s, sub ? sub + (size_t)st * e->Mpad * e->C : nullptr,
                                           hp->target_layer_norm_last ? 1 : 0));
        if (t.dense) {
            CHECK(uvit_gather_patch_rows_launch(xout, sub, e->dense_v, Bc, e->P, e->C, s));
            if (hp->target_batch_norm) CHECK(uvit_colnorm_launch(e->dense_v, 1, Bc * e->P, e->C, 1e-5f, s));
            if (hp->target_instance_norm) CHECK(uvit_colnorm_launch(e->dense_v, Bc, e->P, e->C, 1e-5f, s));
            if (hp->target_layer_norm_last)
                CHECK(uvit_target_accum_launch(e->dense_v, e->idrows, e->idcount, e->dense_acc, t.n == 0, Bc * e->P, e->C, 1e-5f, s));
            else CHECK(uvit_axpy_rows_launch(e->dense_acc, e->dense_v, t.n == 0, (size_t)Bc * e->P * e->C, s));
        }
        ++t.n;
    }
    return UVIT_OK;
}
static int targets_finalize(uvit_engine* e, const FwdPass& p, const TargetBuild& t) {
    const uvit_step_params* hp = p.hp; const int Bc = p.Bc; hipStream_t s = p.s;
    if (t.n != hp->n_target_layers) return UVIT_ERR_ARG;
    for (int st = t.dense ? 1 : 0; st < e->S; ++st)
        CHECK(uvit_target_finalize_launch(e->targets[st], e->count, t.n, hp->post_target_layer_norm, Bc * e->P, e->C, 1e-5f, s));
    if (t.dense) {
        const bool pin = hp->post_target_instance_norm != 0;
        CHECK(uvit_target_finalize_launch(e->dense_acc, e->idcount, t.n, hp->post_target_layer_norm && !pin, Bc * e->P, e->C, 1e-5f, s));
        if (pin) {
            CHECK(uvit_colnorm_launch(e->dense_acc, Bc, e->P, e->C, 1e-5f, s));
            if (hp->post_target_layer_norm)
                CHECK(uvit_target_finalize_launch(e->dense_acc, e->idcount, 1, 1, Bc * e->P, e->C, 1e-5f, s));
        }
        CHECK(uvit_gather_masked_rows_launch(e->dense_acc, e->rowidx, e->count, e->targets[0], Bc * e->P, e->P, e->C, s));
    }
    return UVIT_OK;
}

static int run_forward(uvit_engine* e, const FwdPass& p, const float* images, const int64_t* mask) {
    const int Bc = p.Bc; hipStream_t s = p.s;
    if (Bc < 1 || Bc > e->B) return UVIT_ERR_SHAPE;
    if (p.kind == PASS_DENSE) CHECK(uvit_im2col_launch(images, e->cols, Bc, e->cfg.in_chans, e->cfg.img_size, e->cfg.patch_size, s));
    CHECK(uvit_relpos_gather_launch(e->cfg.use_shared_rel_pos_bias ? p.w.f + e->lo.relt : nullptr, e->buf.rel_index, p.biasP,
                                    e->H, e->N, e->NP, s));
    if (p.dp_on) CHECK(uvit_droppath_launch(e->dp_scales, e->dp_rates, e->cfg.depth, 2 * e->S, Bc, p.draw.seed, p.draw.it, s));
    if (!p.which) {
        e->dpl_on = false;
        if (p.dp_on && p.kind == PASS_STUDENT && e->dpl_enable && Bc == e->B) CHECK(dp_lists_begin(e, p.draw.seed, p.draw.it, Bc, s));
        e->last_dropout = p.draw.on; e->last_seed = p.aseed;
    }
    const bool keep = p.kind != PASS_TEACHER;
    CHECK(embed(e, p.w, mask, keep ? e->X[0] : e->tX[0], Bc, s));
    TargetBuild tb{p.dense, 0};
    for (int l = 0; l < e->cfg.depth; ++l) {
        float* xout = keep ? e->X[l + 1] : e->tX[(l + 1) & 1];
        CHECK(forward_layer(e, p, l, keep ? e->X[l] : e->tX[l & 1], keep ? e->XM[l] : e->tXM, xout, keep ? e->acts[l] : e->tacts));
        if (!keep) CHECK(targets_after_layer(e, p, tb, l, xout));
    }
    if (!keep) CHECK(targets_finalize(e, p, tb));
    e->cur_B = Bc;
    return UVIT_OK;
}

extern "C" int uvit_engine_forward_features(uvit_engine* e, int which, const float* images, const int64_t* mask, int batch,
                                            int train_dropout, uint32_t seed, uint32_t it, uvit_stream stream) {
    if (!e || !images || (which != 0 && which != 1)) return UVIT_ERR_ARG;
    hipStream_t s = (hipStream_t)stream;
    e->tail_which = -1;
    if (mask) CHECK(uvit_mask_compact_launch(mask, e->rowidx, e->count, batch, e->P, s));
    const FwdPass drop_in = fwd_pass(e, PASS_DENSE, which, batch, Draw{train_dropout != 0, seed, it}, nullptr, s);
    CHECK(run_forward(e, drop_in, images, mask));
    e->tail_which = which; e->tail_B = batch; e->tail_first = e->cfg.depth;
    return UVIT_OK;
}

extern "C" int uvit_engine_forward_tail(uvit_engine* e, int which, int batch, int first_layer, int train_dropout, uint32_t seed,
                                        uint32_t it, uvit_stream stream) {
    if (!e || (which != 0 && which != 1)) return UVIT_ERR_ARG;
    if (e->S != 1) return UVIT_ERR_SHAPE;
    if (first_layer < 0 || first_layer >= e->cfg.depth) return UVIT_ERR_ARG;
    if (e->tail_which != which || e->tail_B != batch || batch < 1 || batch > e->B) return UVIT_ERR_ARG;
    if (first_layer > e->tail_first) return UVIT_ERR_ARG;
    hipStream_t s = (hipStream_t)stream;
    FwdPass p = fwd_pass(e, PASS_DENSE, which, batch, Draw{train_dropout != 0, seed, it}, nullptr, s);
    p.dp_on = false;
    e->tail_which = -1;
    for (int l = first_layer; l < e->cfg.depth; ++l)
        CHECK(forward_layer(e, p, l, e->X[l], e->XM[l], e->X[l + 1], e->acts[l]));
    e->tail_which = which; e->tail_first = first_layer;
    return UVIT_OK;
}

static int head_forward(uvit_engine* e, const Weights& w, int Bc, int st, bool all_tokens, float* out, hipStream_t s, int rows = 0) {
    const int BP = rows > 0 ? rows : Bc * e->P;
    const float* x = e->X[e->cfg.depth] + (size_t)st * e->Mpad * e->C;
    const size_t lmw = e->lo.lmw[st], lmb = e->lo.lmb[st];
    LnFwd fn; fn.x = x; fn.w = w.f + e->lo.normw; fn.b = w.f + e->lo.normb; fn.C = e->C; fn.eps = e->cfg.ln_eps;
    if (all_tokens) {
        fn.y = e->acts[0].ln1; fn.mean = e->acts[0].mean1; fn.rstd = e->acts[0].rstd1; fn.M = Bc * e->N;
        CHECK(uvit_ln_fwd_launch(fn, s));
        for (int b = 0; b < Bc; ++b) {
            GemmEpi h; h.out = out + (size_t)b * e->P * e->C; h.bias = w.f + lmb; h.ldo = e->C;
            CHECK(GEMM_NT(EPI_F32, e->acts[0].ln1 + ((size_t)b * e->N + 1) * e->C, w.b + lmw, e->P, e->C, e->C,
                                      e->C, e->C, &h, s));
        }
        return UVIT_OK;
    }
    fn.rowidx = e->rowidx; fn.count = e->count; fn.y = e->normed[st]; fn.mean = e->meanF[st]; fn.rstd = e->rstdF[st]; fn.M = BP;
    CHECK(uvit_ln_fwd_launch(fn, s));
    GemmEpi h; h.out = out; h.bias = w.f + lmb; h.ldo = e->C;
    CHECK(GEMM_NT(EPI_F32, e->normed[st], w.b + lmw, BP, e->C, e->C, e->C, e->C, &h, s));
    return UVIT_OK;
}

extern "C" int uvit_engine_head(uvit_engine* e, int which, int all_tokens, float* out, int32_t* count_dev, uvit_stream stream) {
    if (!e || !out) return UVIT_ERR_ARG;
    hipStream_t s = (hipStream_t)stream;
    const int st = (which >> 1) & 1;
    if (st >= e->S) return UVIT_ERR_ARG;
    CHECK(head_forward(e, weights_of(e, which & 1), e->cur_B, st, all_tokens != 0, out, s));
    if (count_dev && !all_tokens) HIPCHECK(hipMemcpyAsync(count_dev, e->count, sizeof(int), hipMemcpyDeviceToDevice, s));
    return UVIT_OK;
}

extern "C" int uvit_engine_compact_rows(uvit_engine* e) { return e ? e->compact_R : 0; }

extern "C" void* uvit_engine_ws_ptr(uvit_engine* e, const char* name, int layer) {
    if (!e || !name) return nullptr;
    const std::string n(name);
    const size_t cov = (size_t)e->Mpad * e->C;
    if (n == "x" && layer >= 0 && layer <= e->cfg.depth) return e->X[layer];
    if (n == "xm" && layer >= 0 && layer < e->cfg.depth) return e->XM[layer];
// ... 81 lines not shown
        CHECK(GEMM_NT(EPI_BF16, e->dout[st], wt + lmw, Rh, C, C, C, C, &d, s));
        LnBwd fn; fn.dy = e->dnormed[st]; fn.x = e->X[e->cfg.depth] + (size_t)st * e->Mpad * C; fn.rowidx = e->rowidx; fn.count = e->count;
        fn.mean = e->meanF[st]; fn.rstd = e->rstdF[st]; fn.w = e->buf.params + lo.normw; fn.dx = e->dXa + (size_t)st * e->Mpad * C;
        fn.dw = RP(lo.normw); fn.db = RP(lo.normb); fn.M = Rh; fn.C = C; fn.nrep = NREP; fn.rep_stride = e->n_nd;
        CHECK(uvit_ln_bwd_launch(fn, s));
    }
    return UVIT_OK;
}

extern "C" int uvit_step_backward_layer(uvit_engine* e, int l, const uvit_step_params* hp, uvit_stream stream) {
    if (!e || l < 0 || l >= e->cfg.depth || l != e->bwd_next) return UVIT_ERR_ARG;
    (void)hp;
    e->bwd_next = l - 1;
    hipStream_t s = (hipStream_t)stream;
    const LayerOff& o = e->lo.L[l];
    LayerActs& a = e->acts[l];
    const int M = e->M, C = e->C, Hd = e->Hd, S = e->S;
    const size_t Mp = e->Mpad;
    float* g = e->buf.grads;
    const float* pf = e->buf.params;
    const bf16* wt = (const bf16*)e->buf.params_bf16_t;
    const bool dp_on = e->last_dropout && e->cfg.drop_path_rate > 0.f;
    const float pdrop = e->last_dropout ? e->cfg.attn_drop_rate : 0.f;
    const int par = l & 1;
    hipStream_t ws = e->dual ? e->aux : s;
    if (e->dual && l + 2 < e->cfg.depth) HIPCHECK(hipStreamWaitEvent(s, e->ev_wdone[l + 2], 0));
    bf16 *dY1 = e->dY1[par], *dY2 = e->dY2[par], *dH = e->dH[par], *dqkv = e->dqkv[par];
    const BranchRows at = branch_rows(e, l, 0, PASS_STUDENT, e->B), ml = branch_rows(e, l, 1, PASS_STUDENT, e->B);
    const BranchRows nx = l > 0 ? branch_rows(e, l - 1, 1, PASS_STUDENT, e->B) : BranchRows{};
    const int Mmlp = ml.mode == ROWS_ALL ? ml.rows : ml.red;
    if (S == 2 && ml.mode == ROWS_ALL && Mp > (size_t)M) CHECK(uvit_zero_launch(dY1 + (size_t)M * C, (Mp - M) * C * sizeof(bf16), s));
    TnProb wg[UVIT_TN_GROUP_MAX];
    int nwg = 0;
    {
        TnProb& f2 = wg[nwg++]; f2.Y = dY1; f2.X = a.a; f2.C = g + o.fc2w; f2.M = ml.red; f2.Nn = C; f2.Kk = Hd; f2.ldy = C; f2.ldx = Hd; f2.ldc = Hd;
        TnProb& f1 = wg[nwg++]; f1.Y = dH; f1.X = a.ln2; f1.C = g + o.fc1w; f1.M = ml.red; f1.Nn = Hd; f1.Kk = C; f1.ldy = Hd; f1.ldx = C; f1.ldc = C;
        f1.bias = RP(o.fc1b); f1.bias_end = Hd;
        for (int st = 0; st < S; ++st) {
            TnProb& pj = wg[nwg++]; pj.Y = dY2 + at.off[st] * C; pj.X = a.attn + at.off[st] * C; pj.C = g + o.projw[st];
            pj.M = (int)roundup(at.n[st], 64); pj.Nn = C; pj.Kk = C; pj.ldy = C; pj.ldx = C; pj.ldc = C;
        }
        TnProb& qk = wg[nwg++]; qk.Y = dqkv; qk.X = a.ln1; qk.C = g + o.qkvw; qk.M = at.red; qk.Nn = 3 * C; qk.Kk = C; qk.ldy = 3 * C; qk.ldx = C; qk.ldc = C;
        qk.bias = RP(o.qb[0]); qk.bias_end = C; qk.bias2 = RP(o.vb[0]); qk.bias2_begin = 2 * C;
        if (S == 2) { qk.bias_s1 = RP(o.qb[1]); qk.bias2_s1 = RP(o.vb[1]); qk.s1_row = (int)Mp; }
    }
    auto mlp_rider = [&](int layer, int st, const BranchRows& br, bf16* dY) {
        const LayerOff& L = e->lo.L[layer];
        LsNext n; n.y = e->acts[layer].mlpout + st * Mp * C; n.gamma = pf + L.g2; n.rowscale = dp_ptr(e, dp_on, layer, st, 1, e->B);
        n.dy = dY + br.off[st] * C; n.dgamma = RP(L.g2); n.dbias = RP(L.fc2b); n.tokens = e->N;
        return n;
    };
    if (l == e->cfg.depth - 1)
        for (int st = 0; st < S; ++st)
            CHECK(uvit_ls_bwd_launch(e->dXa + st * Mp * C, mlp_rider(l, st, ml, dY1), (ml.mode == ROWS_ALL || st + 1 < S) ? ml.n[st] : ml.red - (int)ml.off[st],
                                     C, NREP, e->n_nd, s, ml.rowmap[st], ml.rowcnt[st]));
    GemmEpi d1; d1.out = dH; d1.aux = a.h; d1.ldo = Hd;
    CHECK(GEMM_NT(EPI_MULAUX, dY1, wt + o.fc2w, Mmlp, Hd, C, C, C, &d1, s));
    GemmEpi d2; d2.out = e->dLN; d2.ldo = C;
    CHECK(GEMM_NT(EPI_BF16, dH, wt + o.fc1w, Mmlp, C, Hd, Hd, Hd, &d2, s));
    const bool ln2_samples = ml.mode != ROWS_MASKED && (ml.mode != ROWS_ALL || at.mode == ROWS_LIST);
    for (int st = 0; st < S; ++st) {
        const size_t eo = st * Mp * C;
        LnBwd b; b.dy = e->dLN + ml.off[st] * C; b.x = e->XM[l] + eo; b.mean = a.mean2 + ml.off[st]; b.rstd = a.rstd2 + ml.off[st]; b.w = pf + o.n2w;
        b.dres = e->dXa + eo; b.dx = e->dXb + eo; b.dw = RP(o.n2w); b.db = RP(o.n2b); b.C = C; b.nrep = NREP; b.rep_stride = e->n_nd;
        LsNext& n = b.next;
        n.y = a.projout + eo; n.gamma = pf + o.g1; n.rowscale = dp_ptr(e, dp_on, l, st, 0, e->B); n.dy = dY2 + at.off[st] * C;
        n.dgamma = RP(o.g1); n.dbias = RP(o.projb[st]); n.tokens = e->N; n.pos = at.d[st].pos;
        if (ln2_samples) { b.M = M; b.pos = ml.d[st].pos; n.cnt = at.d[st].cnt; if (at.mode == ROWS_LIST) { n.pad2 = dqkv; n.pad2_cols = 3 * C; } }
        else { b.M = ml.n[st]; b.rowidx = ml.rowmap[st]; b.count = ml.rowcnt[st]; }
        CHECK(uvit_ln_bwd_launch(b, s));
    }
    for (int st = 0; st < S; ++st) {
        GemmEpi d3; d3.out = e->dAttn + at.off[st] * C; d3.ldo = C;
        CHECK(GEMM_NT(EPI_BF16, dY2 + at.off[st] * C, wt + o.projw[st], at.n[st], C, C, C, C, &d3, s));
    }
    const float* biasP = e->biasP_s;
    float* slabs = e->cfg.use_shared_rel_pos_bias ? e->slabs : nullptr;
    {
        void* dsw = slabs ? e->ds_ws[par] : nullptr;
        if (S == 1) {
            if (at.mode == ROWS_LIST && ml.mode == ROWS_MASKED && at.red > at.rows)
                CHECK(uvit_zero_launch(dqkv + (size_t)at.rows * 3 * C, (size_t)(at.red - at.rows) * 3 * C * sizeof(bf16), s));
            CHECK(uvit_attn_bwd_fused_launch(a.qkv, a.attn, e->dAttn, biasP, a.lse, e->delta, dqkv, dsw, dsw != nullptr, at.K, e->H,
                                             e->N, e->NP, e->attn_scale, pdrop, e->last_seed, (uint32_t)l, s, at.d[0].bmap, e->head_dim));
        } else {
            CHECK(uvit_attn2_bwd_launch(a.qkv, a.qkv + Mp * 3 * C, a.attn, a.attn + Mp * C, e->dAttn, e->dAttn + Mp * C, biasP, a.lse,
                                        e->delta, dqkv, dqkv + Mp * 3 * C, dsw, dsw != nullptr, e->B, e->H, e->N, e->NP, 0.125f, pdrop,
                                        e->last_seed, (uint32_t)l, s));
        }
        if (dsw) {
            if (e->dual) { HIPCHECK(hipEventRecord(e->ev_ds, s)); HIPCHECK(hipStreamWaitEvent(ws, e->ev_ds, 0)); }
            if (S == 1) CHECK(uvit_attn_dbias_reduce_launch(dsw, slabs, e->slab_started ? 1 : 0, at.K, e->H, e->N, e->NP, ws));
            else CHECK(uvit_attn2_dbias_reduce_launch(dsw, slabs, e->slab_started ? 1 : 0, e->B, e->H, e->N, e->NP, ws));
        }
    }
    e->slab_started = true;
    if (e->dual) { HIPCHECK(hipEventRecord(e->ev_x, s)); HIPCHECK(hipStreamWaitEvent(ws, e->ev_x, 0)); }
    CHECK(wgrad(e, wg, nwg, ws));
    if (e->dual) HIPCHECK(hipEventRecord(e->ev_wdone[l], ws));
    GemmEpi d4; d4.out = e->dLN; d4.ldo = C;
    CHECK(GEMM_NT(EPI_BF16, dqkv, wt + o.qkvw, at.rows, C, 3 * C, 3 * C, 3 * C, &d4, s));
    if (l > 0 && e->dual && l + 1 < e->cfg.depth) HIPCHECK(hipStreamWaitEvent(s, e->ev_wdone[l + 1], 0));
    const bool ln1_samples = at.mode == ROWS_LIST || nx.mode != ROWS_ALL;
    for (int st = 0; st < (l > 0 ? S : 1); ++st) {
        const size_t ro = st * Mp, eo = ro * C;
        LnBwd b; b.dy = e->dLN + eo; b.x = e->X[l] + eo; b.mean = a.mean1 + ro; b.rstd = a.rstd1 + ro; b.w = pf + o.n1w; b.dres = e->dXb + eo;
        b.dx = e->dXa + eo; b.dw = RP(o.n1w); b.db = RP(o.n1b); b.M = l > 0 ? M : (int)e->rows_all(); b.C = C; b.nrep = NREP;
        b.rep_stride = e->n_nd;
        if (ln1_samples) { b.pos = at.d[st].pos; b.next.tokens = e->N; }
        if (l > 0) {
            b.next = mlp_rider(l - 1, st, nx, e->dY1[(l - 1) & 1]);
            b.next.pos = nx.d[st].pos;
            if (st + 1 == S && nx.d[st].cnt) { b.next.cnt = nx.d[st].cnt; b.next.pad_base = (int)nx.off[st]; }
        }
        CHECK(uvit_ln_bwd_launch(b, s));
    }
    return UVIT_OK;
}

extern "C" int uvit_step_backward_embed(uvit_engine* e, uvit_stream stream) {
    if (!e) return UVIT_ERR_ARG;
    hipStream_t s = (hipStream_t)stream;
    Layout& lo = e->lo;
    float* g = e->buf.grads;
    const int C = e->C, BP = e->BP;
    TnProb pe[2];
    for (int st = 0; st < e->S; ++st) {
        CHECK(uvit_token_bwd_launch(e->dXa + (size_t)st * e->Mpad * C, e->mask_copy, e->dpatch[st], g + lo.cls[st], g + lo.mask_tok[st], e->B, e->P, C, s));
        TnProb& q = pe[st]; q.Y = e->dpatch[st]; q.X = e->cols; q.C = g + lo.pew[st]; q.M = (int)roundup(BP, 64); q.Nn = C; q.Kk = e->Kpe;
        q.ldy = C; q.ldx = e->Kpe; q.ldc = e->Kpe; q.bias = RP(lo.peb[st]); q.bias_end = C;
    }
    CHECK(wgrad(e, pe, e->S, s));
    if (e->cfg.use_abs_pos_emb) CHECK(uvit_pos_bwd_launch(e->dXa, g + lo.pos, e->B, e->N, C, s));
    if (e->dual) HIPCHECK(hipStreamWaitEvent(s, e->ev_wdone[0], 0));
    if (e->cfg.use_shared_rel_pos_bias && e->slab_started)
        CHECK(uvit_relpos_scatter_launch(e->slabs, 1, e->buf.rel_index, g + lo.relt, e->H, e->N, e->NP, s));
    CHECK(uvit_reduce_replicas_launch(e->grep, g + lo.n_decay, e->n_nd, NREP, e->n_nd, s));
    CHECK(uvit_poison_if_nonfinite_launch(e->loss, g + lo.n_decay, e->poisoned, s));
    return UVIT_OK;
}

extern "C" int uvit_step_wait_layer_grads(uvit_engine* e, int layer, uvit_stream stream) {
    if (!e || layer < 0 || layer >= e->cfg.depth) return UVIT_ERR_ARG;
    if (e->dual) HIPCHECK(hipStreamWaitEvent((hipStream_t)stream, e->ev_wdone[layer], 0));
    return UVIT_OK;
}

extern "C" int uvit_step_update(uvit_engine* e, const uvit_step_params* hp, uvit_stream stream) {
    if (!e || !hp) return UVIT_ERR_ARG;
    if (hp->sched_dev && (hp->sched_len < 1 || hp->sched_index < 0 || hp->sched_index >= hp->sched_len)) return UVIT_ERR_ARG;
    hipStream_t s = (hipStream_t)stream;
    Layout& lo = e->lo;
    HIPCHECK(hipMemsetAsync(e->sumsq, 0, sizeof(double), s));
    CHECK(uvit_sumsq_launch(e->buf.grads, lo.n_live, e->sumsq, s));
    const float gs = hp->grad_scale > 0.f ? hp->grad_scale : 1.0f;
    CHECK(uvit_adamw_launch(e->buf.params, e->buf.grads, e->buf.adam_m, e->buf.adam_v, e->buf.params_bf16, lo.n_live, lo.n_decay,
                            hp->lr, hp->weight_decay, hp->beta1, hp->beta2, hp->eps, hp->opt_step, e->sumsq, hp->clip_grad, gs,
                            e->gnorm, s, e->loss, (hp->do_ema || hp->sched_dev) ? e->buf.ema : nullptr, e->buf.ema_bf16, hp->ema_decay, e->poisoned,
                            hp->sched_dev, hp->sched_len, hp->sched_index));
    CHECK(uvit_transpose_batch_launch(e->tdesc, e->n_tdesc, e->n_ttiles, s));
    return UVIT_OK;
}

extern "C" int uvit_train_step(uvit_engine* e, const float* images, const int64_t* mask, const uvit_step_params* hp,
                               uvit_stream stream) {
    CHECK(uvit_step_begin(e, images, mask, hp, stream));
    for (int l = e->cfg.depth - 1; l >= 0; --l) CHECK(uvit_step_backward_layer(e, l, hp, stream));
// ... 35 lines not shown
extern "C" int uvit_op_gemm_nt_plan(int mode, int M, int N, int K, int lda, int ldw, int ldo, int row_list, const uvit_tuning* tune,
                                    int num_cu, uvit_gemm_nt_plan_info* out) {
    if (!out || num_cu <= 0) return UVIT_ERR_ARG;
    GemmTune tu;
    const int trc = tune_from_abi(tune, tu);
    if (trc) return trc;
    NtPlan p;
    const int rc = uvit_gemm_nt_plan(mode, M, N, K, lda, ldw, ldo, row_list != 0, &tu, num_cu, &p);
    if (rc == UVIT_OK) { out->kernel = p.kind; out->rows = p.rows; out->grid = p.grid; out->tail_rows = p.tail_rows; }
    return rc;
}
extern "C" int uvit_op_gemm_nt(int mode, const void* A, const void* W, int M, int N, int K, int lda, int ldw,
                               const uvit_gemm_epilogue* ep, uvit_stream st) {
    return uvit_op_gemm_nt_tuned(mode, A, W, M, N, K, lda, ldw, ep, nullptr, nullptr, st);
}
extern "C" int uvit_op_gemm_nt_sched(int mode, const void* A, const void* W, int M, int N, int K, int lda, int ldw,
                                     const uvit_gemm_epilogue* ep, const uvit_tuning* tune, uint32_t* tile_counters, uvit_stream st) {
    if (!ep || !A || !W || !ep->out) return UVIT_ERR_ARG;
    GemmTune tu;
    const int trc = tune_from_abi(tune, tu);
    if (trc) return trc;
    GemmEpi g = epi_from_abi(ep);
    g.tile_counter = tile_counters;
    return uvit_gemm_nt_launch(mode, A, W, M, N, K, lda, ldw, &g, S(st), &tu, nullptr);
}
extern "C" int uvit_op_wgrad_group(const uvit_wgrad_problem* problems, int count, const uvit_tuning* tune, uvit_stream st) {
    if (!problems || count < 1 || count > UVIT_TN_GROUP_MAX) return UVIT_ERR_ARG;
    GemmTune tu;
    const int trc = tune_from_abi(tune, tu);
    if (trc) return trc;
    TnProb pr[UVIT_TN_GROUP_MAX];
    for (int i = 0; i < count; ++i) {
        const uvit_wgrad_problem& q = problems[i];
        if (!q.Y_bf16 || !q.X_bf16 || !q.C) return UVIT_ERR_ARG;
        pr[i].Y = q.Y_bf16; pr[i].X = q.X_bf16; pr[i].C = q.C; pr[i].bias = q.bias; pr[i].bias2 = q.bias2;
        pr[i].bias_end = q.bias_end; pr[i].bias2_begin = q.bias2_begin;
        pr[i].M = q.M; pr[i].Nn = q.N; pr[i].Kk = q.K; pr[i].ldy = q.ldy; pr[i].ldx = q.ldx; pr[i].ldc = q.ldc;
    }
    return uvit_gemm_tn_group_launch(pr, count, S(st), &tu);
}

extern "C" int uvit_op_gemm_tn(const void* Y, const void* X, int M, int N, int K, int ldy, int ldx, float* C, int ldc,
                               const uvit_tuning* tune, uvit_stream st) {
    if (!Y || !X || !C) return UVIT_ERR_ARG;
    GemmTune tu;
    const int trc = tune_from_abi(tune, tu);
    if (trc) return trc;
    if (hipMemsetAsync(C, 0, (size_t)N * ldc * sizeof(float), S(st)) != hipSuccess) return UVIT_ERR_LAUNCH;
    return uvit_gemm_tn_launch(Y, X, M, N, K, ldy, ldx, C, ldc, 1, S(st), &tu);
}
extern "C" int uvit_op_attn_fwd(const void* qkv, const float* biasP, void* out, float* lse, int B, int H, int N, int NP,
                                float scale, float p_drop, uint32_t seed, uint32_t layer, uvit_stream st) {
    if (!qkv || !out || !lse) return UVIT_ERR_ARG;
    return uvit_attn_fwd_launch(qkv, biasP, out, lse, B, H, N, NP, scale, p_drop, seed, layer, S(st));
}
extern "C" int64_t uvit_op_attn_bwd_ws_bytes(int B, int H, int N) {
    if (B < 1 || H < 1 || N < 1 || N > 208) return UVIT_ERR_SHAPE;
    return (int64_t)uvit_attn_bwd_fused_ws_bytes(B, H, N);
}
extern "C" int uvit_op_attn_bwd(const void* qkv, const void* o_fwd, const void* d_o, const float* biasP, const float* lse,
                                      float* delta, void* dqkv, float* slab, int acc, void* ds_ws, int B, int H, int N, int NP,
                                      float scale, float p_drop, uint32_t seed, uint32_t layer, uvit_stream st) {
    if (!qkv || !o_fwd || !d_o || !lse || !delta || !dqkv || (slab && !ds_ws)) return UVIT_ERR_ARG;
    CHECK(uvit_attn_bwd_fused_launch(qkv, o_fwd, d_o, biasP, lse, delta, dqkv, ds_ws, slab != nullptr, B, H, N, NP, scale, p_drop, seed, layer, S(st)));
    if (slab) CHECK(uvit_attn_dbias_reduce_launch(ds_ws, slab, acc, B, H, N, NP, S(st)));
    return UVIT_OK;
}
extern "C" int uvit_op_attn_fwd_hd(const void* qkv, const float* biasP, void* out, float* lse, int B, int H, int N, int NP, int head_dim,
                                   float scale, float p_drop, uint32_t seed, uint32_t layer, uvit_stream st) {
    if (!qkv || !out || !lse) return UVIT_ERR_ARG;
    if (head_dim != 64 && head_dim != 80) return UVIT_ERR_SHAPE;
    return uvit_attn_fwd_launch(qkv, biasP, out, lse, B, H, N, NP, scale, p_drop, seed, layer, S(st), nullptr, head_dim);
}
extern "C" int uvit_op_attn_bwd_hd(const void* qkv, const void* o_fwd, const void* d_o, const float* biasP, const float* lse,
                                   float* delta, void* dqkv, float* slab, int acc, void* ds_ws, int B, int H, int N, int NP, int head_dim,
                                   float scale, float p_drop, uint32_t seed, uint32_t layer, uvit_stream st) {
    if (!qkv || !o_fwd || !d_o || !lse || !delta || !dqkv || (slab && !ds_ws)) return UVIT_ERR_ARG;
    if (head_dim != 64 && head_dim != 80) return UVIT_ERR_SHAPE;
    CHECK(uvit_attn_bwd_fused_launch(qkv, o_fwd, d_o, biasP, lse, delta, dqkv, ds_ws, slab != nullptr, B, H, N, NP, scale, p_drop, seed, layer,
                                     S(st), nullptr, head_dim));
    if (slab) CHECK(uvit_attn_dbias_reduce_launch(ds_ws, slab, acc, B, H, N, NP, S(st)));
    return UVIT_OK;
}
extern "C" int uvit_op_attn2_fwd(const void* qkv_m, const void* qkv_c, const float* biasP, void* out_m, void* out_c, float* lse, int B,
                                 int H, int N, int NP, float scale, float p_drop, uint32_t seed, uint32_t layer, uvit_stream st) {
    if (!qkv_m || !qkv_c || !out_m || !out_c || !lse) return UVIT_ERR_ARG;
    return uvit_attn2_fwd_launch(qkv_m, qkv_c, biasP, out_m, out_c, lse, B, H, N, NP, scale, p_drop, seed, layer, S(st));
}
extern "C" int64_t uvit_op_attn2_bwd_ws_bytes(int B, int H, int N) {
    if (B <= 0 || H <= 0 || N <= 0) return UVIT_ERR_SHAPE;
    return (int64_t)uvit_attn2_bwd_ws_bytes(B, H, N);
}
extern "C" int uvit_op_attn2_bwd(const void* qkv_m, const void* qkv_c, const void* o_m, const void* o_c, const void* d_m, const void* d_c,
                                 const float* biasP, const float* lse, float* delta, void* dqkv_m, void* dqkv_c, float* slab, int acc,
                                 void* ds_ws, int B, int H, int N, int NP, float scale, float p_drop, uint32_t seed, uint32_t layer,
                                 uvit_stream st) {
    if (!qkv_m || !qkv_c || !o_m || !o_c || !d_m || !d_c || !lse || !delta || !dqkv_m || !dqkv_c || (slab && !ds_ws)) return UVIT_ERR_ARG;
    CHECK(uvit_attn2_bwd_launch(qkv_m, qkv_c, o_m, o_c, d_m, d_c, biasP, lse, delta, dqkv_m, dqkv_c, ds_ws, slab != nullptr, B, H, N, NP,
                                scale, p_drop, seed, layer, S(st)));
    if (slab) CHECK(uvit_attn2_dbias_reduce_launch(ds_ws, slab, acc, B, H, N, NP, S(st)));
    return UVIT_OK;
}
extern "C" int uvit_op_relpos_gather(const float* t, const int32_t* idx, float* biasP, int H, int N, int NP, uvit_stream st) {
    return uvit_relpos_gather_launch(t, idx, biasP, H, N, NP, S(st));
}
extern "C" int uvit_op_relpos_scatter(const float* slab, int nslab, const int32_t* idx, float* dt, int H, int N, int NP, uvit_stream st) {
    return uvit_relpos_scatter_launch(slab, nslab, idx, dt, H, N, NP, S(st));
}
extern "C" int uvit_op_ln_fwd(const float* x, const float* w, const float* b, void* y, float* mean, float* rstd, int M, int C,
                              float eps, uvit_stream st) {
    LnFwd p; p.x = x; p.w = w; p.b = b; p.y = (bf16*)y; p.mean = mean; p.rstd = rstd; p.M = M; p.C = C; p.eps = eps;
    return uvit_ln_fwd_launch(p, S(st));
}
extern "C" int uvit_op_ln_bwd(const void* dy, const float* x, const float* mean, const float* rstd, const float* w,
                              const float* dres, float* dx, float* dw, float* db, int M, int C, uvit_stream st) {
    LnBwd p; p.dy = (const bf16*)dy; p.x = x; p.mean = mean; p.rstd = rstd; p.w = w; p.dres = dres; p.dx = dx; p.dw = dw; p.db = db; p.M = M; p.C = C;
    return uvit_ln_bwd_launch(p, S(st));
}
static LsNext ls_from_abi(const uvit_ls_rider* r) {
    LsNext n;
    if (!r) return n;
    n.y = (const bf16*)r->y; n.gamma = r->gamma; n.rowscale = r->rowscale; n.dy = (bf16*)r->dy; n.dgamma = r->dgamma; n.dbias = r->dbias;
    n.tokens = r->tokens; n.pos = r->pos; n.cnt = r->cnt; n.pad_base = r->pad_base; n.pad2 = (bf16*)r->pad2; n.pad2_cols = r->pad2_cols;
    return n;
}
extern "C" int uvit_op_ln_fwd_walk(const float* x, const float* w, const float* b, void* y, float* mean, float* rstd, int M, int C, float eps,
                                   const int32_t* rowidx, const int32_t* count, const int32_t* pos, float* xcopy, int tokens, uvit_stream st) {
    if (!x || !w || !b || !y || (!mean != !rstd)) return UVIT_ERR_ARG;
    LnFwd p; p.x = x; p.w = w; p.b = b; p.y = (bf16*)y; p.mean = mean; p.rstd = rstd; p.M = M; p.C = C; p.eps = eps;
    p.rowidx = rowidx; p.count = count; p.pos = pos; p.xcopy = xcopy; p.tokens = tokens;
    return uvit_ln_fwd_launch(p, S(st));
}
extern "C" int uvit_op_ln_bwd_walk(const void* dy, const float* x, const float* mean, const float* rstd, const float* w, const float* dres,
                                   float* dx, float* dw, float* db, int M, int C, int nrep, int64_t rep_stride, const int32_t* rowidx,
                                   const int32_t* count, const int32_t* pos, const uvit_ls_rider* next, uvit_stream st) {
    if (!dy || !x || !mean || !rstd || !w || !dx || !dw || !db || nrep < 1 || rep_stride < 0) return UVIT_ERR_ARG;
    if (next && next->dy && (!next->y || !next->gamma || !next->dgamma || !next->dbias)) return UVIT_ERR_ARG;
    LnBwd p; p.dy = (const bf16*)dy; p.x = x; p.mean = mean; p.rstd = rstd; p.w = w; p.dres = dres; p.dx = dx; p.dw = dw; p.db = db;
    p.M = M; p.C = C; p.nrep = nrep; p.rep_stride = (size_t)rep_stride; p.rowidx = rowidx; p.count = count; p.pos = pos;
    p.next = ls_from_abi(next);
    return uvit_ln_bwd_launch(p, S(st));
}
extern "C" int uvit_op_ls_bwd(const float* dx, const uvit_ls_rider* r, int M, int C, int nrep, int64_t rep_stride, const int32_t* rowidx,
                              const int32_t* count, uvit_stream st) {
    if (!dx || !r || !r->y || !r->gamma || !r->dy || !r->dgamma || !r->dbias || nrep < 1 || rep_stride < 0) return UVIT_ERR_ARG;
    if (M <= 0 || C <= 0 || r->tokens <= 0) return UVIT_ERR_SHAPE;
    return uvit_ls_bwd_launch(dx, ls_from_abi(r), M, C, nrep, (size_t)rep_stride, S(st), rowidx, count);
}
extern "C" int uvit_op_colsum(const void* y, int ld, int col0, int ncols, int M, float* out, int nrep, int64_t rep_stride, uvit_stream st) {
    if (!y || !out || nrep < 1 || rep_stride < 0) return UVIT_ERR_ARG;
    if (M <= 0 || ncols <= 0 || col0 < 0 || col0 + ncols > ld) return UVIT_ERR_SHAPE;
    return uvit_colsum_launch(y, ld, col0, ncols, M, out, nrep, (size_t)rep_stride, S(st));
}
extern "C" int uvit_op_reduce_replicas(const float* rep, float* out, int64_t n, int nrep, int64_t stride, uvit_stream st) {
    if (!rep || !out || n < 0 || nrep < 0 || stride < 0) return UVIT_ERR_ARG;
    return uvit_reduce_replicas_launch(rep, out, (size_t)n, nrep, (size_t)stride, S(st));
}
extern "C" int uvit_op_droppath_lists(const float* scales, int32_t* pos, int32_t* bmap, int32_t* rows, int32_t* cnt, int nlists, int B,
                                      int tokens, int rows_stride, const int32_t* host_counts, uvit_stream st) {
    if (!scales || !pos || !bmap || !rows || !cnt || !host_counts || B < 1 || tokens < 1) return UVIT_ERR_ARG;
    return uvit_droppath_lists_launch(scales, pos, bmap, rows, cnt, nlists, B, tokens, rows_stride, host_counts, S(st));
}
extern "C" int uvit_op_gemm_nt_rows(int mode, const void* A, const void* W, int M, int N, int K, int lda, int ldw, const uvit_gemm_epilogue* ep,
                                    const int32_t* rowmap, const int32_t* rowcount, const uvit_tuning* tune, uvit_stream st) {
    if (!A || !W || !ep || !ep->out || !ep->resid || !rowmap || !rowcount || mode != UVIT_EPI_RESID) return UVIT_ERR_ARG;
    GemmTune tu;
// ... 80 lines not shown
```

### uncertainty-vit_amd/csrc/uvit_internal.h

```cpp
#pragma once
#include <hip/hip_runtime.h>
#include <stdint.h>
#include "common.h"

enum { EPI_BF16 = 0, EPI_QKV = 1, EPI_GELU = 2, EPI_RESID = 3, EPI_F32 = 4, EPI_PATCH = 5, EPI_DGELU = 6, EPI_QKV_ELU = 7,
       EPI_GELU_DG = 8,
       EPI_MULAUX = 9 };

struct GemmEpi {
    void* out = nullptr;
    void* out2 = nullptr;
    const float* bias = nullptr;
    const float* bias2 = nullptr;
    const float* gamma = nullptr;
    const float* resid = nullptr;
    const float* rowscale = nullptr;
    const void* aux = nullptr;
    const int64_t* mask = nullptr;
    const float* mask_token = nullptr;
    int ldo = 0;
    int tokens = 1;
    int patches = 1;
    int row0 = 0;
    int ngroup = 0;
    const int* rowmap = nullptr;
    const int* rowcount = nullptr;
    unsigned* tile_counter = nullptr;
};

struct GemmTune {
    int nt_variant = 3;
    int tn_variant = 3;
    int tn_target = 512;
    int group_chunks = 0;
    int nt_group = 0;
    int nt_persist = 1;
};
enum { NT_128 = 0, NT_256 = 1, NT_256P = 2, NT_320 = 3, NT_RING128 = 4, NT_RING160 = 5, NT_KINDS = 6 };
struct NtPlan { int kind; int rows; int grid; int tail_rows; };
int uvit_gemm_nt_plan(int mode, int M, int N, int K, int lda, int ldw, int ldo, bool row_list, const GemmTune* tune, int num_cu,
                      NtPlan* out);
int uvit_gemm_nt_launch(int mode, const void* A, const void* W, int M, int N, int K, int lda, int ldw,
                        const GemmEpi* epi, hipStream_t s, const GemmTune* tune = nullptr, int* tail_rows_out = nullptr);
int uvit_gemm_tn_launch(const void* Y, const void* X, int M, int Nn, int Kk, int ldy, int ldx, float* C,
                        int ldc, int allow_split, hipStream_t s, const GemmTune* tune = nullptr);

#define UVIT_TN_GROUP_MAX 6
struct TnProb {
    const void* Y = nullptr;
    const void* X = nullptr;
    float* C = nullptr;
    float* bias = nullptr;
    float* bias2 = nullptr;
    int bias_end = 0, bias2_begin = 0;
    float* bias_s1 = nullptr; float* bias2_s1 = nullptr; int s1_row = 0;
    int M = 0, Nn = 0, Kk = 0, ldy = 0, ldx = 0, ldc = 0;
    int nm = 0, tiles_n = 0, tiles_k = 0, chunk_steps = 0, chunks = 0;
};
struct TnGroup { TnProb p[UVIT_TN_GROUP_MAX]; int nprob = 0; int max_chunks = 0; };
bool uvit_gemm_tn_group_ok(const TnProb* probs, int n, const GemmTune* tune = nullptr);
int uvit_gemm_tn_group_launch(const TnProb* probs, int n, hipStream_t s, const GemmTune* tune = nullptr);

int uvit_attn_fwd_launch(const void* qkv, const float* biasP, void* out, float* lse, int B, int H, int N, int NP,
                         float scale, float p_drop, uint32_t seed, uint32_t layer, hipStream_t s, const int* bmap = nullptr,
                         int head_dim = 64);
size_t uvit_attn_bwd_fused_ws_bytes(int B, int H, int N);
int uvit_attn_bwd_fused_launch(const void* qkv, const void* o_fwd, const void* d_o, const float* biasP, const float* lse,
                               float* delta, void* dqkv, void* ds_ws, int want_ds, int B, int H, int N, int NP, float scale,
                               float p_drop, uint32_t seed, uint32_t layer, hipStream_t s, const int* bmap = nullptr,
                               int head_dim = 64);
int uvit_attn_dbias_reduce_launch(const void* ds_ws, float* dbias_slab, int accumulate, int B, int H, int N, int NP, hipStream_t s);

int uvit_attn2_fwd_launch(const void* qkv_m, const void* qkv_c, const float* biasP, void* out_m, void* out_c, float* lse,
                          int B, int H, int N, int NP, float scale, float p_drop, uint32_t seed, uint32_t layer, hipStream_t s);
size_t uvit_attn2_bwd_ws_bytes(int B, int H, int N);
int uvit_attn2_bwd_launch(const void* qkv_m, const void* qkv_c, const void* o_m, const void* o_c, const void* d_m, const void* d_c,
                          const float* biasP, const float* lse, float* delta, void* dqkv_m, void* dqkv_c, void* ds_ws, int want_ds,
                          int B, int H, int N, int NP, float scale, float p_drop, uint32_t seed, uint32_t layer, hipStream_t s);
int uvit_attn2_dbias_reduce_launch(const void* ds_ws, float* dbias_slab, int accumulate, int B, int H, int N, int NP, hipStream_t s);

struct LnFwd {
    const float* x = nullptr;
    const float* w = nullptr;
    const float* b = nullptr;
    bf16* y = nullptr;
    float* mean = nullptr;
    float* rstd = nullptr;
    int M = 0, C = 0;
    float eps = 0.f;
    const int* rowidx = nullptr;
    const int* count = nullptr;
    const int* pos = nullptr;
    float* xcopy = nullptr;
    int tokens = 0;
};
int uvit_ln_fwd_launch(const LnFwd& p, hipStream_t s);

struct LsNext {
    const bf16* y = nullptr;
    const float* gamma = nullptr;
    const float* rowscale = nullptr;
    bf16* dy = nullptr;
    float* dgamma = nullptr;
    float* dbias = nullptr;
    int tokens = 0;
    const int* pos = nullptr;
    const int* cnt = nullptr;
    int pad_base = 0;
    bf16* pad2 = nullptr;
    int pad2_cols = 0;
};
struct LnBwd {
    const bf16* dy = nullptr;
    const float* x = nullptr;
    const float* mean = nullptr;
    const float* rstd = nullptr;
    const float* w = nullptr;
    const float* dres = nullptr;
    float* dx = nullptr;
    float* dw = nullptr;
    float* db = nullptr;
    int M = 0, C = 0;
    int nrep = 1;
    size_t rep_stride = 0;
    const int* rowidx = nullptr;
    const int* count = nullptr;
    const int* pos = nullptr;
    LsNext next;
};
int uvit_ln_bwd_launch(const LnBwd& p, hipStream_t s);
int uvit_reduce_replicas_launch(const float* rep, float* out, size_t n, int nrep, size_t stride, hipStream_t s);
int uvit_target_accum_launch(const float* x, const int* rowidx, const int* count, float* acc, int first, int Mmax,
                             int C, float eps, hipStream_t s, const float* sub = nullptr,
                             int ln = 1);
int uvit_variance_loss_launch(const float* out, const int* count, float w, float margin, float loss_scale, float* scratch,
                              float* loss, float* std_loss0_out, void* dout_bf16, int Mmax, int C, hipStream_t s);
int uvit_gather_patch_rows_launch(const float* x, const float* sub, float* v, int B, int P, int C, hipStream_t s);
int uvit_colnorm_launch(float* v, int groups, int rows, int C, float eps, hipStream_t s);
int uvit_axpy_rows_launch(float* acc, const float* v, int first, size_t n, hipStream_t s);
int uvit_gather_masked_rows_launch(const float* dense, const int* rowidx, const int* count, float* out, int Mmax, int P, int C,
                                   hipStream_t s);
int uvit_target_finalize_launch(float* acc, const int* count, int n_layers, int post_ln, int Mmax, int C, float eps,
                                hipStream_t s);

int uvit_im2col_launch(const float* img, void* cols_bf16, int B, int Cin, int img_size, int patch, hipStream_t s);
int uvit_mask_compact_launch(const int64_t* mask, int* rowidx, int* count, int B, int P, hipStream_t s);
int uvit_set_cls_launch(float* x, const float* cls, const float* pos, int B, int N, int C, hipStream_t s);
int uvit_relpos_gather_launch(const float* table, const int* index, float* biasP, int H, int N, int NP, hipStream_t s);
int uvit_relpos_scatter_launch(const float* slab, int nslab, const int* index, float* dtable, int H, int N, int NP,
                               hipStream_t s);
int uvit_ls_bwd_launch(const float* dx, const LsNext& ls, int M, int C, int nrep, size_t rep_stride, hipStream_t s,
                       const int* rowidx = nullptr, const int* count = nullptr);
int uvit_rows_guard_launch(const int* count, int limit, float* loss, hipStream_t s);
// ... 35 lines not shown
```

### uncertainty-vit_amd/modeling_cyclical.py

```python
import ctypes as C
import math
import weakref
from functools import partial

import numpy as np
import torch
import torch.nn as nn

from . import native
from .native import Buffers, Config, LayoutEntry, check, cur_stream, lib, ptr

__all__ = ["beit_base_patch16_224", "dist_beit_base_patch16_224", "beit_large_patch16_224", "dist_beit_large_patch16_224",
           "beit_huge_patch16_224", "create_model", "register_model",
           "VisionTransformerForCyclicalTraining", "DistVisionTransformerForCyclicalTraining"]


def _cfg(url="", **kwargs):
    return {"url": url, "num_classes": 1000, "input_size": (3, 224, 224), "pool_size": None, "crop_pct": 0.9,
            "interpolation": "bicubic", "mean": (0.5, 0.5, 0.5), "std": (0.5, 0.5, 0.5), **kwargs}


def trunc_normal_(tensor, mean=0.0, std=1.0):
    with torch.no_grad():
        lo = (1.0 + math.erf(-1.0 / math.sqrt(2.0))) / 2.0
        hi = (1.0 + math.erf(1.0 / math.sqrt(2.0))) / 2.0
        tensor.uniform_(2 * lo - 1, 2 * hi - 1).erfinv_().mul_(std * math.sqrt(2.0)).add_(mean)
        tensor.clamp_(min=mean - std, max=mean + std)
    return tensor


def relative_position_index(ws):
    n_rel = (2 * ws - 1) * (2 * ws - 1) + 3
    ys, xs = np.meshgrid(np.arange(ws), np.arange(ws), indexing="ij")
    ys, xs = ys.reshape(-1), xs.reshape(-1)
    idx = np.zeros((ws * ws + 1,) * 2, dtype=np.int64)
    idx[1:, 1:] = (ys[:, None] - ys[None, :] + ws - 1) * (2 * ws - 1) + (xs[:, None] - xs[None, :] + ws - 1)
    idx[0, :] = n_rel - 3
    idx[:, 0] = n_rel - 2
    idx[0, 0] = n_rel - 1
    return torch.from_numpy(idx)


class _Holder(nn.Module):
    """Container that only exists to give parameters their reference state-dict names."""


class _PatchEmbedInfo(_Holder):
    def __init__(self, img_size, patch_size):
        super().__init__()
        self.img_size = (img_size, img_size)
        self.patch_size = (patch_size, patch_size)
        self.patch_shape = (img_size // patch_size, img_size // patch_size)
        self.num_patches = self.patch_shape[0] * self.patch_shape[1]
        self.proj = _Holder()


class NativeEngine:

    def __init__(self, model, teacher, batch, adam_m=None, adam_v=None):
        L = lib()
        dev = model._arena.device
        if dev.type != "cuda":
            raise native.UvitError("the HIP path needs the model on a GPU (no CPU fallback)")
        n = model._arena.numel()
        self._model, self.teacher, self.batch = weakref.ref(model), teacher, batch
        self.cfg = model._native_config(batch)
        z = lambda dt=torch.float32, k=n: torch.zeros(k, dtype=dt, device=dev)
        self.grads = model._grad_arena if model._grad_arena is not None else z()
        model._grad_arena = self.grads
        self.adam_m = adam_m if adam_m is not None else z()
        self.adam_v = adam_v if adam_v is not None else z()
        self.ema = teacher._arena if teacher is not None else model._arena
        self.params_bf16, self.params_bf16_t, self.ema_bf16 = z(torch.bfloat16), z(torch.bfloat16), z(torch.bfloat16)
        self.rel_index = None
        if model.rel_pos_bias is not None:
            self.rel_index = model.rel_pos_bias.relative_position_index.to(dev, torch.int32).contiguous().view(-1)
        ws = L.uvit_workspace_bytes(C.byref(self.cfg))
        if ws < 0:
            check(int(ws), "uvit_workspace_bytes")
        self.workspace = torch.empty(ws, dtype=torch.uint8, device=dev)
        b = Buffers(model._arena.data_ptr(), self.grads.data_ptr(), self.adam_m.data_ptr(), self.adam_v.data_ptr(),
                    self.ema.data_ptr(), self.params_bf16.data_ptr(), self.params_bf16_t.data_ptr(),
                    self.ema_bf16.data_ptr(), 0 if self.rel_index is None else self.rel_index.data_ptr(),
                    self.workspace.data_ptr(), ws)
        err = C.c_int(0)
        with torch.cuda.device(dev):
            self.h = L.uvit_engine_create(C.byref(self.cfg), C.byref(b), cur_stream(), C.byref(err))
        if not self.h:
            check(err.value or -1, "uvit_engine_create")
        self.h = C.c_void_p(self.h)
        import os
        import torch.distributed as dist
        world = dist.get_world_size() if dist.is_available() and dist.is_initialized() else 1
        self.stream_mode = 0 if os.environ.get("UVIT_SINGLE_STREAM") == "1" else (2 if world == 1 else 1)
        if os.environ.get("UVIT_STREAM_MODE"):
            self.stream_mode = int(os.environ["UVIT_STREAM_MODE"])
        check(L.uvit_engine_set_streams(self.h, self.stream_mode), "set_streams")
        self.drop_path_rows = bool(getattr(model, "drop_path_rows", os.environ.get("UVIT_DP_ROWS", "1") != "0"))
        self.set_drop_path_rows(self.drop_path_rows)
        self.sync_shadows(3)

    @property
    def model(self):
        return self._model()

    def set_drop_path_rows(self, on):
        self.drop_path_rows = bool(on)
        check(lib().uvit_engine_set_drop_path_rows(self.h, 1 if on else 0), "set_drop_path_rows")

    def sync_shadows(self, which=3):
        check(lib().uvit_engine_sync_shadows(self.h, which, cur_stream()), "sync_shadows")

    def compact_rows(self):
        return int(lib().uvit_engine_compact_rows(self.h))

    def ws_tensor(self, name, layer, shape, dtype=torch.float32):
        p = lib().uvit_engine_ws_ptr(self.h, name.encode(), layer)
        if not p:
            raise native.UvitError(f"no workspace buffer {name}[{layer}]")
        off = p - self.workspace.data_ptr()
        n = int(np.prod(shape)) * torch.empty((), dtype=dtype).element_size()
        return self.workspace[off:off + n].view(dtype).view(*shape)

    def __del__(self):
        try:
            if getattr(self, "h", None):
                lib().uvit_engine_destroy(self.h)
                self.h = None
        except Exception:
            pass


class VisionTransformerForCyclicalTraining(nn.Module):
    _two_stream = False

    def __init__(self, img_size=224, patch_size=16, in_chans=3, embed_dim=768, depth=12, num_heads=12, mlp_ratio=4.0,
                 qkv_bias=True, qk_scale=None, drop_rate=0.0, attn_drop_rate=0.0, drop_path_rate=0.0, norm_layer=None,
                 init_values=None, attn_head_dim=None, use_abs_pos_emb=True, use_rel_pos_bias=False,
                 use_shared_rel_pos_bias=False, init_std=0.02, gp_layer=False, gumbel_softmax=False, sinkformer=False,
                 h_sto_trans=False, stosa=False):
        super().__init__()
        self._ctor = dict(img_size=img_size, patch_size=patch_size, in_chans=in_chans, embed_dim=embed_dim, depth=depth,
                          num_heads=num_heads, mlp_ratio=mlp_ratio, qkv_bias=qkv_bias, attn_drop_rate=attn_drop_rate,
                          drop_path_rate=drop_path_rate, norm_layer=norm_layer, init_values=init_values,
                          use_abs_pos_emb=use_abs_pos_emb, use_shared_rel_pos_bias=use_shared_rel_pos_bias, init_std=init_std)
        unsupported = dict(qk_scale=qk_scale, attn_head_dim=attn_head_dim, gp_layer=gp_layer, gumbel_softmax=gumbel_softmax,
                           sinkformer=sinkformer, h_sto_trans=h_sto_trans, stosa=stosa, use_rel_pos_bias=use_rel_pos_bias,
                           use_abs_pos_emb=use_abs_pos_emb and self._two_stream)
        bad = [k for k, v in unsupported.items() if v]
        if bad or not qkv_bias or drop_rate:
            raise NotImplementedError(f"not on the MI355X hot path (SURVEY.md section 8): {bad or 'qkv_bias/drop_rate'}")
        if init_values is None or not init_values > 0:
            raise TypeError("init_values must be > 0 (LayerScale is part of the configured path)")
        head_dims = (64,) if self._two_stream else (64, 80)
        if embed_dim not in [num_heads * d for d in head_dims]:
            raise NotImplementedError(
                f"attention kernels support head_dim {' or '.join(map(str, head_dims))} for this model "
                f"(ViT-B/L: 64, ViT-H: 80); got embed_dim {embed_dim} / num_heads {num_heads}")
        self.num_features = self.embed_dim = embed_dim
        self.depth, self.num_heads, self.mlp_hidden = depth, num_heads, int(embed_dim * mlp_ratio)
        self.img_size, self.in_chans = img_size, in_chans
        self.attn_drop_rate, self.drop_path_rate, self.init_values = attn_drop_rate, drop_path_rate, init_values
        self.ln_eps = 1e-6
        if norm_layer is not None:
            probe = norm_layer(4)
            self.ln_eps = float(getattr(probe, "eps", 1e-6))
        self.init_std = init_std
        self.patch_embed = _PatchEmbedInfo(img_size, patch_size)
        self.stosa = False
        self.use_abs_pos_emb = bool(use_abs_pos_emb)
        if not self.use_abs_pos_emb:
            self.pos_embed = None
        ws = self.patch_embed.patch_shape[0]

        cfg = self._native_config(1)
        L = lib()
        nd = C.c_int64()
        n = L.uvit_arena_numel(C.byref(cfg), C.byref(nd))
        if n < 0:
            check(int(n), "uvit_arena_numel (unsupported model shape)")
        self._n_decay = nd.value
        self._arena = torch.zeros(n, dtype=torch.float32)
        self._grad_arena = None
        self._layout = []
        for i in range(L.uvit_layout_count(C.byref(cfg))):
            e = LayoutEntry()
            check(L.uvit_layout_get(C.byref(cfg), i, C.byref(e)), "uvit_layout_get")
            self._layout.append((e.name.decode(), int(e.offset), int(e.numel), tuple(e.shape[:e.ndim]), int(e.decay)))
        self.blocks = nn.ModuleList()
        for _ in range(depth):
            blk = _Holder()
# ... 272 lines not shown
```

### uncertainty-vit_amd/native.py

```python
import ctypes as C
import os
import subprocess

import torch

_HERE = os.path.dirname(os.path.abspath(__file__))
LIB_PATH = os.path.join(_HERE, "libuvit.so")
MAX_DEPTH = 64


class UvitError(RuntimeError):
    pass


_ERR = {-1: "bad argument", -2: "unsupported shape", -3: "HIP launch/runtime error", -4: "workspace too small"}


def check(rc, what=""):
    if rc != 0:
        raise UvitError(f"libuvit: {what} failed: {_ERR.get(rc, rc)} ({rc})")


class Config(C.Structure):
    _fields_ = [(n, C.c_int32) for n in ("img_size", "patch_size", "in_chans", "embed_dim", "depth", "num_heads",
# ... 26 lines not shown
                ("n_rows_hint", C.c_int32)]


class WgradProblem(C.Structure):
    _fields_ = [("Y", C.c_void_p), ("X", C.c_void_p), ("C", C.c_void_p), ("bias", C.c_void_p), ("bias2", C.c_void_p),
                ("bias_end", C.c_int32), ("bias2_begin", C.c_int32), ("M", C.c_int32), ("N", C.c_int32), ("K", C.c_int32),
                ("ldy", C.c_int32), ("ldx", C.c_int32), ("ldc", C.c_int32)]


class GemmEpilogue(C.Structure):
    _fields_ = [(n, C.c_void_p) for n in ("out", "out2", "bias", "bias2", "gamma", "resid", "rowscale", "aux", "mask",
                                           "mask_token")] + [("ldo", C.c_int32), ("tokens", C.c_int32), ("patches", C.c_int32),
                                                             ("row0", C.c_int32)]


class Tuning(C.Structure):
    _fields_ = [("nt_variant", C.c_int32), ("tn_variant", C.c_int32), ("tn_split_target", C.c_int32),
                ("wgrad_group_chunks", C.c_int32), ("nt_group", C.c_int32), ("nt_persist", C.c_int32)]

    @classmethod
    def default(cls, **over):
        t = cls()
        lib().uvit_tuning_default(C.byref(t))
        for k, v in over.items():
            setattr(t, k, v)
        return t


class GemmNtPlanInfo(C.Structure):
    _fields_ = [("kernel", C.c_int32), ("rows", C.c_int32), ("grid", C.c_int32), ("tail_rows", C.c_int32)]


class LsRider(C.Structure):
    _fields_ = [(n, C.c_void_p) for n in ("y", "gamma", "rowscale", "dy", "dgamma", "dbias")] + \
               [("tokens", C.c_int32), ("pos", C.c_void_p), ("cnt", C.c_void_p), ("pad_base", C.c_int32), ("pad2", C.c_void_p),
                ("pad2_cols", C.c_int32)]


class WgradSplit(C.Structure):
    _fields_ = [("bias_s1", C.c_void_p), ("bias2_s1", C.c_void_p), ("s1_row", C.c_int32)]


class TransposeDesc(C.Structure):
    _fields_ = [("src", C.c_void_p), ("dst", C.c_void_p), ("rows", C.c_int32), ("cols", C.c_int32), ("tile0", C.c_int32),
                ("pad", C.c_int32)]


class AugmentDesc(C.Structure):
    _fields_ = [("offset", C.c_int64)] + \
               [(n, C.c_int32) for n in ("h", "w", "flip", "crop_x", "crop_y", "crop_w", "crop_h", "resize_w", "resize_h", "win_x",
                                          "win_y", "filter", "n_jitter")] + \
               [("jitter_op", C.c_int32 * 3), ("jitter_factor", C.c_float * 3), ("reserved", C.c_int32)]


_vp, _i, _i64, _f, _u32 = C.c_void_p, C.c_int, C.c_int64, C.c_float, C.c_uint32
_PROTOTYPES = {
    "uvit_version": (_i, []),
    "uvit_source_hash": (C.c_char_p, []),
    "uvit_layout_count": (_i, [_vp]),
    "uvit_layout_get": (_i, [_vp, _i, _vp]),
    "uvit_arena_numel": (_i64, [_vp, _vp]),
    "uvit_workspace_bytes": (_i64, [_vp]),
    "uvit_engine_create": (_vp, [_vp, _vp, _vp, _vp]),
    "uvit_engine_destroy": (None, [_vp]),
    "uvit_engine_sync_shadows": (_i, [_vp, _i, _vp]),
    "uvit_engine_forward_features": (_i, [_vp, _i, _vp, _vp, _i, _i, _u32, _u32, _vp]),
    "uvit_engine_forward_tail": (_i, [_vp, _i, _i, _i, _i, _u32, _u32, _vp]),
    "uvit_engine_head": (_i, [_vp, _i, _i, _vp, _vp, _vp]),
    "uvit_engine_ws_ptr": (_vp, [_vp, C.c_char_p, _i]),
    "uvit_engine_compact_rows": (_i, [_vp]),
    "uvit_step_begin": (_i, [_vp, _vp, _vp, _vp, _vp]),
    "uvit_step_backward_layer": (_i, [_vp, _i, _vp, _vp]),
    "uvit_step_backward_embed": (_i, [_vp, _vp]),
    "uvit_step_wait_layer_grads": (_i, [_vp, _i, _vp]),
    "uvit_step_update": (_i, [_vp, _vp, _vp]),
    "uvit_train_step": (_i, [_vp, _vp, _vp, _vp, _vp]),
    "uvit_engine_read_stats": (_i, [_vp, _vp, _vp]),
    "uvit_engine_read_stats_async": (_i, [_vp, _vp, _vp]),
    "uvit_tuning_default": (None, [_vp]),
    "uvit_engine_set_tuning": (_i, [_vp, _vp]),
    "uvit_op_wgrad_group": (_i, [_vp, _i, _vp, _vp]),
    "uvit_engine_set_streams": (_i, [_vp, _i]),
    "uvit_engine_set_drop_path_rows": (_i, [_vp, _i]),
    "uvit_drop_path_kept_counts": (_i, [_i, _f, _i, _i, _u32, _u32, _vp]),
    "uvit_engine_profile": (_i, [_vp, _i, _i]),
    "uvit_engine_profile_read": (_i, [_vp, _vp, _vp, _vp]),
    "uvit_engine_profile_read_kind": (_i, [_vp, _i, _vp, _vp, _vp, _vp]),
    "uvit_op_gemm_nt": (_i, [_i, _vp, _vp, _i, _i, _i, _i, _i, _vp, _vp]),
    "uvit_op_gemm_nt_tuned": (_i, [_i, _vp, _vp, _i, _i, _i, _i, _i, _vp, _vp, _vp, _vp]),
    "uvit_op_gemm_nt_plan": (_i, [_i, _i, _i, _i, _i, _i, _i, _i, _vp, _i, _vp]),
    "uvit_op_gemm_nt_sched": (_i, [_i, _vp, _vp, _i, _i, _i, _i, _i, _vp, _vp, _vp, _vp]),
    "uvit_op_gemm_tn": (_i, [_vp, _vp, _i, _i, _i, _i, _i, _vp, _i, _vp, _vp]),
    "uvit_op_wasserstein_loss": (_i, [_vp, _vp, _vp, _vp, _vp, _f, _f, _vp, _vp, _vp, _vp, _i, _i, _vp]),
    "uvit_op_attn_fwd": (_i, [_vp, _vp, _vp, _vp, _i, _i, _i, _i, _f, _f, _u32, _u32, _vp]),
    "uvit_op_attn_bwd_ws_bytes": (_i64, [_i, _i, _i]),
    "uvit_op_attn_bwd": (_i, [_vp, _vp, _vp, _vp, _vp, _vp, _vp, _vp, _i, _vp, _i, _i, _i, _i, _f, _f, _u32, _u32, _vp]),
    "uvit_op_attn_fwd_hd": (_i, [_vp, _vp, _vp, _vp, _i, _i, _i, _i, _i, _f, _f, _u32, _u32, _vp]),
    "uvit_op_attn_bwd_hd": (_i, [_vp, _vp, _vp, _vp, _vp, _vp, _vp, _vp, _i, _vp, _i, _i, _i, _i, _i, _f, _f, _u32, _u32, _vp]),
    "uvit_op_attn2_fwd": (_i, [_vp, _vp, _vp, _vp, _vp, _vp, _i, _i, _i, _i, _f, _f, _u32, _u32, _vp]),
    "uvit_op_attn2_bwd_ws_bytes": (_i64, [_i, _i, _i]),
    "uvit_op_attn2_bwd": (_i, [_vp] * 12 + [_i, _vp, _i, _i, _i, _i, _f, _f, _u32, _u32, _vp]),
    "uvit_op_relpos_gather": (_i, [_vp, _vp, _vp, _i, _i, _i, _vp]),
    "uvit_op_relpos_scatter": (_i, [_vp, _i, _vp, _vp, _i, _i, _i, _vp]),
    "uvit_op_ln_fwd": (_i, [_vp, _vp, _vp, _vp, _vp, _vp, _i, _i, _f, _vp]),
    "uvit_op_ln_bwd": (_i, [_vp, _vp, _vp, _vp, _vp, _vp, _vp, _vp, _vp, _i, _i, _vp]),
    "uvit_op_ln_fwd_walk": (_i, [_vp, _vp, _vp, _vp, _vp, _vp, _i, _i, _f, _vp, _vp, _vp, _vp, _i, _vp]),
    "uvit_op_ln_bwd_walk": (_i, [_vp] * 9 + [_i, _i, _i, _i64, _vp, _vp, _vp, _vp, _vp]),
    "uvit_op_ls_bwd": (_i, [_vp, _vp, _i, _i, _i, _i64, _vp, _vp, _vp]),
    "uvit_op_colsum": (_i, [_vp, _i, _i, _i, _i, _vp, _i, _i64, _vp]),
    "uvit_op_reduce_replicas": (_i, [_vp, _vp, _i64, _i, _i64, _vp]),
    "uvit_op_droppath_lists": (_i, [_vp, _vp, _vp, _vp, _vp, _i, _i, _i, _i, _vp, _vp]),
    "uvit_op_gemm_nt_rows": (_i, [_i, _vp, _vp, _i, _i, _i, _i, _i, _vp, _vp, _vp, _vp, _vp]),
    "uvit_op_wgrad_group_split": (_i, [_vp, _vp, _i, _vp, _vp]),
    "uvit_op_token_bwd": (_i, [_vp, _vp, _vp, _vp, _vp, _i, _i, _i, _vp]),
    "uvit_op_transpose_batch": (_i, [_vp, _i, _i, _vp]),
    "uvit_op_ema": (_i, [_vp, _vp, _vp, _i64, _f, _vp]),
    "uvit_op_sumsq": (_i, [_vp, _i64, _vp, _vp]),
    "uvit_op_adamw": (_i, [_vp, _vp, _vp, _vp, _vp, _i64, _i64, _f, _f, _f, _f, _f, _i, _vp, _f, _f, _vp, _vp]),
    "uvit_op_smooth_l1": (_i, [_vp, _vp, _vp, _f, _i, _f, _vp, _vp, _i, _i, _vp]),
    "uvit_op_target_accum": (_i, [_vp, _vp, _vp, _vp, _i, _i, _i, _f, _vp]),
    "uvit_op_variance_loss": (_i, [_vp, _vp, _f, _f, _f, _vp, _vp, _vp, _vp, _i, _i, _vp]),
    "uvit_op_target_finalize": (_i, [_vp, _vp, _i, _i, _i, _i, _f, _vp]),
    "uvit_op_mask_compact": (_i, [_vp, _vp, _vp, _i, _i, _vp]),
    "uvit_op_im2col": (_i, [_vp, _vp, _i, _i, _i, _i, _vp]),
    "uvit_op_synth_batch": (_i, [_vp, _vp, _i, _i, _i, _i, _i, _u32, _u32, _vp]),
    "uvit_op_droppath": (_i, [_vp, _vp, _i, _i, _u32, _u32, _vp]),
    "uvit_op_cast_bf16": (_i, [_vp, _vp, _i64, _vp]),
    "uvit_op_augment_ws_bytes": (_i64, [_vp, _i, _i]),
    "uvit_op_augment_batch": (_i, [_vp, _i64, _vp, _i, _i, _vp, _vp, _vp, _vp, _i64, _vp]),
    "uvit_op_probe_pool_ws_bytes": (_i64, [_i, _i, _i]),
    "uvit_op_probe_pool_norm": (_i, [_vp, _vp, _vp, _i, _i, _i, _f, _vp]),
    "uvit_op_probe_logits": (_i, [_vp, _vp, _vp, _vp, _i, _i, _i, _vp]),
    "uvit_op_probe_ce": (_i, [_vp, _vp, _f, _vp, _vp, _vp, _vp, _i, _i, _vp]),
    "uvit_op_probe_head_grad": (_i, [_vp, _vp, _vp, _vp, _i, _i, _i, _vp]),
    "uvit_op_calib_softmax": (_i, [_vp, _vp, _i, _i, _vp]),
    "uvit_op_calib_confidence": (_i, [_vp, _vp, _vp, _i, _i, _vp, _vp, _vp, _vp, _vp, _i, _i, _vp]),
    "uvit_op_calib_tace": (_i, [_vp, _vp, C.c_double, _i, _i, _vp, _vp, _i, _i, _vp]),
    "uvit_op_calib_auroc": (_i, [_vp, _vp, _vp, _vp, _i, _i, _vp]),
    "uvit_op_stability_ranks": (_i, [_vp, _vp, _i, _i, _vp]),
    "uvit_op_stability_sequences": (_i, [_vp, _vp, _i, _i, _i, _i, _vp]),
    "uvit_op_gp_features": (_i, [_vp] * 5 + [_f, _f] + [_vp] * 3 + [_i, _i, _i, _vp]),
    "uvit_op_gp_precision_update": (_i, [_vp, _vp, _i, _i, C.c_double, _vp]),
    "uvit_op_gp_ln_grad_ws_bytes": (_i64, [_i, _i, _i]),
    "uvit_op_gp_ln_grad": (_i, [_vp] * 5 + [_f] + [_vp] * 3 + [_i, _i, _i, _i, _vp]),
    "uvit_op_gp_variance": (_i, [_vp, _vp, C.c_double, _vp, _i, _i, _vp]),
    "uvit_op_gp_mean_field": (_i, [_vp, _vp, C.c_double, _vp, _i, _i, _vp]),
    "uvit_op_het_noise": (_i, [_vp, _vp, _i, _i, _i, _i, _u32, _i, _vp]),
    "uvit_op_het_mc_ws_bytes": (_i64, [_i, _i, _i, _i]),
    "uvit_op_het_mc_forward": (_i, [_vp] * 5 + [_i, _i, _i, _i, _f, _f, _u32, _i, _vp]),
    "uvit_op_het_mc_backward": (_i, [_vp] * 5 + [_i, _i, _i, _i, _f, _f, _u32, _i, _vp]),
    "uvit_op_ens_bag_weights": (_i, [_vp, _i, _i, _u32, _vp]),
    "uvit_op_ens_ce": (_i, [_vp, _vp, _vp, _f, _vp, _vp, _vp, _vp, _i, _i, _i, _vp]),
    "uvit_op_ens_clip": (_i, [_vp, _vp, _i, _i, _i, _f, _vp]),
    "uvit_op_ens_combine": (_i, [_vp, _i, _vp, _vp, _i, _i, _i, _vp]),
    "uvit_op_detect_rows": (_i, [_vp, _vp, _vp, _i64, _i64, _vp, _i, _i, _vp]),
    "uvit_op_detect_column": (_i, [_vp, _i, _i64, _vp, _i, _vp]),
    "uvit_op_detect_ws_bytes": (_i64, [_i, _i]),
    "uvit_op_detect_metrics": (_i, [_vp, _i64, _vp, _i, _i, _vp, _vp, _vp, _i64, _vp]),
    "uvit_op_ts_ws_bytes": (_i64, [_i, _i]),
    "uvit_op_ts_fit": (_i, [_vp, _i64, _vp, _i, _i, C.c_double, C.c_double, C.c_double, _i, _vp, _vp, _i64, _vp]),
    "uvit_op_ts_scale": (_i, [_vp, _vp, _i64, _i64, _vp, _i, _i, _vp]),
    "uvit_op_cp_scores": (_i, [_vp, _i64, _vp, _vp, _i, _i, _i, C.c_double, _i, _vp, _vp]),
    "uvit_op_cp_ws_bytes": (_i64, [_i, _i]),
    "uvit_op_cp_quantile": (_i, [_vp, _i, _vp, _i, _vp, _vp, _i64, _vp]),
    "uvit_op_cp_counter_count": (_i64, [_i, _i]),
    "uvit_op_cp_sets": (_i, [_vp, _i64, _vp, _vp, _i, _i, _i, C.c_double, _i, _vp, _i, _vp, _vp, _vp, _i64, _vp]),
    "uvit_op_cp_finish": (_i, [_vp, _vp, _i, _i, _vp]),
    "uvit_op_lap_factors_ws_bytes": (_i64, [_i, _i, _i]),
    "uvit_op_lap_factors": (_i, [_vp, _vp, _i64, _vp, _vp, _vp, _vp, _vp, _i64, _i, _i, _i, _vp]),
    "uvit_op_lap_prepare": (_i, [_vp, _vp, _vp, C.c_double, _vp, _i, _i, _vp]),
    "uvit_op_lap_variance_ws_bytes": (_i64, [_i, _i, _i]),
    "uvit_op_lap_variance": (_i, [_vp, _vp, _vp, _vp, _vp, _i64, _i, _i, _i, _vp]),
    "uvit_op_lap_probit": (_i, [_vp, _i64, _vp, C.c_double, _vp, _i64, _vp, _i, _i, _vp]),
    "uvit_op_maha_accumulate_ws_bytes": (_i64, [_i, _i, _i]),
    "uvit_op_maha_accumulate": (_i, [_vp] * 8 + [_i64, _i, _i, _i, _vp]),
    "uvit_op_maha_scores_ws_bytes": (_i64, [_i, _i, _i]),
    "uvit_op_maha_scores": (_i, [_vp] * 10 + [_i64, _vp, _vp, _vp, _i64, _i, _i, _i, _vp]),
    "uvit_op_knn_rows": (_i, [_vp] * 5 + [_i, _i, _i, _vp]),
    "uvit_op_knn_search_ws_bytes": (_i64, [_i, _i, _i, _i, _i]),
    "uvit_op_knn_search": (_i, [_vp] * 6 + [_i64, _vp, _i64, _i, _i, _i, _i, _i, _vp]),
    "uvit_op_knn_scores": (_i, [_vp, _vp, _i64, _vp, _i, _vp, _vp, _vp, _i64, _vp, _vp, _i, _i, _i, C.c_double, _vp]),
# ... 89 lines not shown
```

Baseline: 5586.

## Store attention dropout keep bits in forward and reuse them in backward

The forward attention kernel now records the dropout keep mask as packed bits per query row in a workspace buffer. The backward kernel reads those bits instead of re-hashing the RNG for every score element. The forward kernel also gets a specialization for the full tile count with a scheduling barrier. The aim is to remove repeated hash work in backward, at the cost of extra global writes and reads for the bit buffer plus more kernel instantiations. The feature is on by default for student passes.

```diff
diff --git a/include/uvit.h b/include/uvit.h
--- a/include/uvit.h
+++ b/include/uvit.h
@@ -109,6 +109,7 @@
 int uvit_engine_set_tuning(uvit_engine* e, const uvit_tuning* t);
 int uvit_engine_set_streams(uvit_engine* e, int dual);
 int uvit_engine_set_drop_path_rows(uvit_engine* e, int on);
+int uvit_engine_set_attn_keep_bits(uvit_engine* e, int on);
 int uvit_drop_path_kept_counts(int depth, float drop_path_rate, int draws_per_block, int batch, uint32_t seed, uint32_t it, int32_t* out);
 int uvit_engine_profile(uvit_engine* e, int enable, int max_launches);
 int uvit_engine_profile_read(uvit_engine* e, double* total_ms, int* launches, double* flops_per_launch);
@@ -155,6 +156,13 @@
 int uvit_op_attn_bwd_hd(const void* qkv, const void* o_fwd, const void* d_o, const float* biasP, const float* lse,
                         float* delta, void* dqkv, float* dbias_slab, int accumulate_slab, void* ds_workspace, int B, int H,
                         int N, int NP, int head_dim, float scale, float p_drop, uint32_t seed, uint32_t layer, uvit_stream stream);
+int64_t uvit_op_attn_keep_bytes(int B, int H, int N);
+int uvit_op_attn_fwd_ex(const void* qkv, const float* biasP, void* out, float* lse, void* keep_bits, const int* bmap, int generic,
+                        int B, int H, int N, int NP, int head_dim, float scale, float p_drop, uint32_t seed, uint32_t layer,
+                        uvit_stream stream);
+int uvit_op_attn_bwd_ex(const void* qkv, const void* o_fwd, const void* d_o, const float* biasP, const float* lse, float* delta,
+                        void* dqkv, void* ds_workspace, const void* keep_bits, const int* bmap, int B, int H, int N, int NP, int head_dim,
+                        float scale, float p_drop, uint32_t seed, uint32_t layer, uvit_stream stream);
 int uvit_op_attn2_fwd(const void* qkv_m, const void* qkv_c, const float* biasP, void* out_m, void* out_c, float* lse, int B, int H,
                       int N, int NP, float scale, float p_drop, uint32_t seed, uint32_t layer, uvit_stream stream);
 int64_t uvit_op_attn2_bwd_ws_bytes(int B, int H, int N);
diff --git a/uncertainty-vit_amd/csrc/attention.hip b/uncertainty-vit_amd/csrc/attention.hip
--- a/uncertainty-vit_amd/csrc/attention.hip
+++ b/uncertainty-vit_amd/csrc/attention.hip
@@ -37,11 +37,11 @@
 }
 #endif
 
-template <int HDK, int NW, bool HAS_BIAS>
+template <int HDK, int NW, bool HAS_BIAS, int NT_C, bool KEEP>
 __global__ __launch_bounds__(NW * 64, 4)
 void attn_fwd_kernel(const bf16* __restrict__ qkv, const float* __restrict__ biasP, bf16* __restrict__ out,
                      float* __restrict__ lse, int H, int N, int NP, float scale, uint32_t drop_thr,
-                     float inv_keep, uint32_t drop_key, int ncu, const int* __restrict__ bmap) {
+                     float inv_keep, uint32_t drop_key, int ncu, const int* __restrict__ bmap, uint2* __restrict__ keep) {
     constexpr int NDT = HDK / 16;
     extern __shared__ __attribute__((aligned(16))) char smem[];
     char* kimg = smem;
@@ -75,7 +75,7 @@
     asm volatile("s_waitcnt vmcnt(0)" ::: "memory");
     if constexpr (HDK == 64) { landed(qn[0]); landed(qn[1]); }
     __syncthreads();
-    const int nt = (N + 15) >> 4, nt2 = (nt + 1) >> 1;
+    const int nt = NT_C ? NT_C : (N + 15) >> 4, nt2 = (nt + 1) >> 1;
 
     for (int qt = wave; qt < nt; qt += NW) {
         const int q = qt * 16 + li;
@@ -147,6 +147,8 @@
 #pragma unroll
         for (int dt = 0; dt < NDT; ++dt) o[dt] = f32x4{0.f, 0.f, 0.f, 0.f};
         const uint32_t rowpair = (bh_rng * N + q) * (uint32_t)(NP >> 1);
+        const uint32_t thrm1x2 = (drop_thr - 1) * 0x10001u;
+        uint2 kw = make_uint2(0u, 0u);
 #pragma unroll
         for (int ks = 0; ks < (NT_MAX + 1) / 2; ++ks) {
             if (ks < nt2) {
@@ -154,14 +156,29 @@
                 float pa[4], pb[4];
 #pragma unroll
                 for (int r = 0; r < 4; ++r) { pa[r] = s[t0][r]; pb[r] = t1 < NT_MAX ? s[t1 < NT_MAX ? t1 : 0][r] : 0.f; }
-                if (drop_thr) {
-                    bool k4[4];
-                    keep4(drop_key, rowpair, t0 * 16 + 4 * g, drop_thr, k4);
-#pragma unroll
-                    for (int r = 0; r < 4; ++r) pa[r] = k4[r] ? pa[r] : 0.f;
-                    keep4(drop_key, rowpair, t1 * 16 + 4 * g, drop_thr, k4);
-#pragma unroll
-                    for (int r = 0; r < 4; ++r) pb[r] = k4[r] ? pb[r] : 0.f;
+                if constexpr (!KEEP) {
+                    if (drop_thr) {
+                        bool k4[4];
+                        keep4(drop_key, rowpair, t0 * 16 + 4 * g, drop_thr, k4);
+#pragma unroll
+                        for (int r = 0; r < 4; ++r) pa[r] = k4[r] ? pa[r] : 0.f;
+                        keep4(drop_key, rowpair, t1 * 16 + 4 * g, drop_thr, k4);
+#pragma unroll
+                        for (int r = 0; r < 4; ++r) pb[r] = k4[r] ? pb[r] : 0.f;
+                    }
+                } else {
+                    auto draw = [&](int t, float (&pv)[4]) {
+#pragma unroll
+                        for (int hh = 0; hh < 2; ++hh) {
+                            const int j = 2 * t + hh;
+                            const uint32_t f = keep_pair(pair_hash(drop_key, rowpair + ((t * 16 + 4 * g) >> 1) + hh), thrm1x2);
+                            if (j < 16) kw.x |= f << (j & 15); else kw.y |= f << (j & 15);
+                            pv[2 * hh] = __uint_as_float(__float_as_uint(pv[2 * hh]) & keep_mask<0>(f));
+                            pv[2 * hh + 1] = __uint_as_float(__float_as_uint(pv[2 * hh + 1]) & keep_mask<16>(f));
+                        }
+                    };
+                    draw(t0, pa);
+                    if (t1 < NT_MAX) draw(t1, pb);
                 }
                 const bf16x8 pf = pack8(pa, pb);
 #pragma unroll
@@ -171,6 +188,7 @@
                 }
                 if constexpr (HDK == 80)
                     o[4] = __builtin_amdgcn_mfma_f32_16x16x32_bf16(col_frag_tail(vtail, t0 * 16, t1 * 16, lane), pf, o[4], 0, 0, 0);
+                if constexpr (NT_C != 0) __builtin_amdgcn_sched_barrier(0);
             }
         }
         if constexpr (HDK == 64) {
@@ -184,6 +202,10 @@
             for (int dt = 0; dt < NDT; ++dt) {
                 bf16x4 v = {f2bf(o[dt][0] * f), f2bf(o[dt][1] * f), f2bf(o[dt][2] * f), f2bf(o[dt][3] * f)};
                 *(bf16x4*)(dst + dt * 16) = v;
+            }
+            if constexpr (KEEP) {
+                const uint2 pad = keep_pad_bits(N, g);
+                keep[((size_t)bh * N + q) * 4 + g] = make_uint2(kw.x | pad.x, kw.y | pad.y);
             }
         }
     }
@@ -231,12 +253,13 @@
     return __builtin_bit_cast(bf16x8, v);
 }
 
-template <int HDK, bool HAS_BIAS, int NT_C>
+template <int HDK, bool HAS_BIAS, int NT_C, bool KEEP>
 __global__ __launch_bounds__(FB_WAVES * 64)
 void attn_bwd_fused_kernel(const bf16* __restrict__ qkv, const bf16* __restrict__ o_fwd, const bf16* __restrict__ d_o,
                            const float* __restrict__ biasP, const float* __restrict__ lse, float* __restrict__ delta,
                            bf16* __restrict__ dqkv, bf16* __restrict__ ds_out, int H, int N, int NP, float scale,
-                           uint32_t drop_thr, float inv_keep, uint32_t drop_key, const int* __restrict__ bmap) {
+                           uint32_t drop_thr, float inv_keep, uint32_t drop_key, const int* __restrict__ bmap,
+                           const uint2* __restrict__ keep) {
     constexpr int NDT = HDK / 16;
     constexpr int BW = 2 * NDT;
     extern __shared__ __attribute__((aligned(16))) char smem[];
@@ -279,6 +302,7 @@
         }
     }
     float dl = 0.f, lse_q = 1e30f;
+    uint2 kw = make_uint2(~0u, ~0u);
     if (active) {
         const size_t orow = ((size_t)b * N + qr) * C + h * HDK;
 #pragma unroll
@@ -297,6 +321,7 @@
         dl = group_sum4(dl);
         if (q < N) {
             lse_q = lse[(size_t)bh * N + q];
+            if constexpr (KEEP) kw = keep[((size_t)bh * N + q) * 4 + g];
             if (g == 0) delta[(size_t)bh * N + q] = dl;
         }
     }
@@ -340,10 +365,14 @@
             if (i + 1 < nsteps) bias_fetch(i + 1);
             BSTAMP(4);
             bool k4[2][4] = {{true, true, true, true}, {true, true, true, true}};
+            uint32_t kx = 0;
+            if constexpr (KEEP) kx = (i < 4 ? kw.x : kw.y) >> (4 * (i & 3));
 #ifndef ATTN_HAZARD_DEMO
-            if (drop_thr) {
-                keep4(drop_key, rowpair, t0 * 16 + 4 * g, drop_thr, k4[0]);
-                keep4(drop_key, rowpair, t0 * 16 + 16 + 4 * g, drop_thr, k4[1]);
+            if constexpr (!KEEP) {
+                if (drop_thr) {
+                    keep4(drop_key, rowpair, t0 * 16 + 4 * g, drop_thr, k4[0]);
+                    keep4(drop_key, rowpair, t0 * 16 + 16 + 4 * g, drop_thr, k4[1]);
+                }
             }
 #endif
             BSTAMP(5);
@@ -388,13 +417,17 @@
                 keep4(drop_key, rowpair, t0 * 16 + 16 + 4 * g, drop_thr, k4[1]);
             }
 #endif
+            uint32_t km[2][4] = {};
+            if constexpr (KEEP) keep_masks8(kx, km);
 #pragma unroll
             for (int tt = 0; tt < 2; ++tt) {
                 const float bb[4] = {bcur[tt].x, bcur[tt].y, bcur[tt].z, bcur[tt].w};
 #pragma unroll
                 for (int r = 0; r < 4; ++r) {
                     const float p = __builtin_amdgcn_exp2f(sacc[tt][r] * cs + bb[r] - lse_q);
-                    const float pd = k4[tt][r] ? p * inv_keep : 0.f;
+                    float pd;
+                    if constexpr (KEEP) pd = __uint_as_float(__float_as_uint(p * inv_keep) & km[tt][r]);
+                    else pd = k4[tt][r] ? p * inv_keep : 0.f;
                     pdv[tt][r] = pd;
                     dsv[tt][r] = pd * dp[tt][r] - p * dl;
                 }
@@ -599,16 +632,26 @@
 
 template <int HDK>
 struct AttnKernels {
-    static auto fwd(bool has_bias) { return has_bias ? attn_fwd_kernel<HDK, FWD_WAVES, true> : attn_fwd_kernel<HDK, FWD_WAVES, false>; }
-    static auto bwd(bool has_bias, bool full) {
-        if (full) return has_bias ? attn_bwd_fused_kernel<HDK, true, NT_MAX> : attn_bwd_fused_kernel<HDK, false, NT_MAX>;
-        return has_bias ? attn_bwd_fused_kernel<HDK, true, 0> : attn_bwd_fused_kernel<HDK, false, 0>;
-    }
+    template <bool KEEP>
+    static auto fwd_k(bool has_bias, bool full) {
+        if (full) return has_bias ? attn_fwd_kernel<HDK, FWD_WAVES, true, NT_MAX, KEEP> : attn_fwd_kernel<HDK, FWD_WAVES, false, NT_MAX, KEEP>;
+        return has_bias ? attn_fwd_kernel<HDK, FWD_WAVES, true, 0, KEEP> : attn_fwd_kernel<HDK, FWD_WAVES, false, 0, KEEP>;
+    }
+    static auto fwd(bool has_bias, bool full, bool keep) { return keep ? fwd_k<true>(has_bias, full) : fwd_k<false>(has_bias, full); }
+    template <bool KEEP>
+    static auto bwd_k(bool has_bias, bool full) {
+        if (full) return has_bias ? attn_bwd_fused_kernel<HDK, true, NT_MAX, KEEP> : attn_bwd_fused_kernel<HDK, false, NT_MAX, KEEP>;
+        return has_bias ? attn_bwd_fused_kernel<HDK, true, 0, KEEP> : attn_bwd_fused_kernel<HDK, false, 0, KEEP>;
+    }
+    static auto bwd(bool has_bias, bool full, bool keep) { return keep ? bwd_k<true>(has_bias, full) : bwd_k<false>(has_bias, full); }
     static void lds_init() {
         for (bool has_bias : {false, true}) {
-            (void)hipFuncSetAttribute((const void*)fwd(has_bias), hipFuncAttributeMaxDynamicSharedMemorySize, fwd_lds(HDK));
-            for (bool full : {false, true})
-                (void)hipFuncSetAttribute((const void*)bwd(has_bias, full), hipFuncAttributeMaxDynamicSharedMemorySize, fb_lds(HDK));
+            for (bool full : {false, true}) {
+                for (bool keep : {false, true}) {
+                    (void)hipFuncSetAttribute((const void*)fwd(has_bias, full, keep), hipFuncAttributeMaxDynamicSharedMemorySize, fwd_lds(HDK));
+                    (void)hipFuncSetAttribute((const void*)bwd(has_bias, full, keep), hipFuncAttributeMaxDynamicSharedMemorySize, fb_lds(HDK));
+                }
+            }
         }
     }
 };
@@ -631,20 +674,25 @@
 
 template <int HDK>
 static void attn_fwd_go(const void* qkv, const float* biasP, void* out, float* lse, int B, int H, int N, int NP, float scale,
-                        uint32_t thr, float inv_keep, uint32_t key, hipStream_t s, const int* bmap) {
-    hipLaunchKernelGGL(AttnKernels<HDK>::fwd(biasP != nullptr), dim3(B * H), dim3(FWD_WAVES * 64), fwd_lds(HDK), s, (const bf16*)qkv,
-                       biasP, (bf16*)out, lse, H, N, NP, scale, thr, inv_keep, key, g_attn_ncu, bmap);
-}
+                        uint32_t thr, float inv_keep, uint32_t key, hipStream_t s, const int* bmap, uint2* keep, bool generic) {
+    const bool full = (N + 15) / 16 == NT_MAX && !generic;
+    hipLaunchKernelGGL(AttnKernels<HDK>::fwd(biasP != nullptr, full, keep != nullptr), dim3(B * H), dim3(FWD_WAVES * 64), fwd_lds(HDK), s, (const bf16*)qkv,
+                       biasP, (bf16*)out, lse, H, N, NP, scale, thr, inv_keep, key, g_attn_ncu, bmap, keep);
+}
+
+size_t uvit_attn_keep_bytes(int B, int H, int N) { return (size_t)B * H * N * 4 * sizeof(uint2); }
 
 int uvit_attn_fwd_launch(const void* qkv, const float* biasP, void* out, float* lse, int B, int H, int N, int NP,
-                         float scale, float p_drop, uint32_t seed, uint32_t layer, hipStream_t s, const int* bmap, int head_dim) {
+                         float scale, float p_drop, uint32_t seed, uint32_t layer, hipStream_t s, const int* bmap, int head_dim,
+                         void* keep_bits, bool generic) {
     int rc = attn_check(B, H, N, head_dim); if (rc) return rc;
     attn_init_once();
     const uint32_t thr = p_drop > 0.f ? uvit_drop_threshold16(p_drop) : 0u;
     const float inv_keep = p_drop > 0.f ? 1.0f / (1.0f - p_drop) : 1.0f;
     const uint32_t key = uvit_layer_key(seed, layer);
-    if (head_dim == 80) attn_fwd_go<80>(qkv, biasP, out, lse, B, H, N, NP, scale, thr, inv_keep, key, s, bmap);
-    else attn_fwd_go<64>(qkv, biasP, out, lse, B, H, N, NP, scale, thr, inv_keep, key, s, bmap);
+    uint2* keep = thr ? (uint2*)keep_bits : nullptr;
+    if (head_dim == 80) attn_fwd_go<80>(qkv, biasP, out, lse, B, H, N, NP, scale, thr, inv_keep, key, s, bmap, keep, generic);
+    else attn_fwd_go<64>(qkv, biasP, out, lse, B, H, N, NP, scale, thr, inv_keep, key, s, bmap, keep, generic);
     return uvit_check_launch();
 }
 
@@ -656,15 +704,16 @@
 template <int HDK>
 static void attn_bwd_go(const void* qkv, const void* o_fwd, const void* d_o, const float* biasP, const float* lse, float* delta,
                         void* dqkv, bf16* dsw, int B, int H, int N, int NP, float scale, uint32_t thr, float inv_keep, uint32_t key,
-                        hipStream_t s, const int* bmap) {
-    hipLaunchKernelGGL(AttnKernels<HDK>::bwd(biasP != nullptr, (N + 15) / 16 == NT_MAX), dim3(B * H), dim3(FB_WAVES * 64), fb_lds(HDK), s,
+                        hipStream_t s, const int* bmap, const uint2* keep) {
+    hipLaunchKernelGGL(AttnKernels<HDK>::bwd(biasP != nullptr, (N + 15) / 16 == NT_MAX, keep != nullptr), dim3(B * H), dim3(FB_WAVES * 64), fb_lds(HDK), s,
                        (const bf16*)qkv, (const bf16*)o_fwd, (const bf16*)d_o, biasP, lse, delta, (bf16*)dqkv, dsw, H, N, NP, scale, thr,
-                       inv_keep, key, bmap);
+                       inv_keep, key, bmap, keep);
 }
 
 int uvit_attn_bwd_fused_launch(const void* qkv, const void* o_fwd, const void* d_o, const float* biasP, const float* lse,
                                float* delta, void* dqkv, void* ds_ws, int want_ds, int B, int H, int N, int NP, float scale,
-                               float p_drop, uint32_t seed, uint32_t layer, hipStream_t s, const int* bmap, int head_dim) {
+                               float p_drop, uint32_t seed, uint32_t layer, hipStream_t s, const int* bmap, int head_dim,
+                               const void* keep_bits) {
     int rc = attn_check(B, H, N, head_dim); if (rc) return rc;
     if (NP < NT_MAX * 16 || (want_ds && !ds_ws)) return UVIT_ERR_ARG;
     attn_init_once();
@@ -672,8 +721,9 @@
     const float inv_keep = p_drop > 0.f ? 1.0f / (1.0f - p_drop) : 1.0f;
     const uint32_t key = uvit_layer_key(seed, layer);
     bf16* dsw = want_ds ? (bf16*)ds_ws : nullptr;
-    if (head_dim == 80) attn_bwd_go<80>(qkv, o_fwd, d_o, biasP, lse, delta, dqkv, dsw, B, H, N, NP, scale, thr, inv_keep, key, s, bmap);
-    else attn_bwd_go<64>(qkv, o_fwd, d_o, biasP, lse, delta, dqkv, dsw, B, H, N, NP, scale, thr, inv_keep, key, s, bmap);
+    const uint2* keep = thr ? (const uint2*)keep_bits : nullptr;
+    if (head_dim == 80) attn_bwd_go<80>(qkv, o_fwd, d_o, biasP, lse, delta, dqkv, dsw, B, H, N, NP, scale, thr, inv_keep, key, s, bmap, keep);
+    else attn_bwd_go<64>(qkv, o_fwd, d_o, biasP, lse, delta, dqkv, dsw, B, H, N, NP, scale, thr, inv_keep, key, s, bmap, keep);
     return uvit_check_launch();
 }
 
diff --git a/uncertainty-vit_amd/csrc/attn_common.h b/uncertainty-vit_amd/csrc/attn_common.h
--- a/uncertainty-vit_amd/csrc/attn_common.h
+++ b/uncertainty-vit_amd/csrc/attn_common.h
@@ -53,6 +53,28 @@
     k[0] = (h0 & 0xFFFFu) >= thr16; k[1] = (h0 >> 16) >= thr16;
     k[2] = (h1 & 0xFFFFu) >= thr16; k[3] = (h1 >> 16) >= thr16;
 }
+__device__ __forceinline__ uint32_t keep_pair(uint32_t h, uint32_t thrm1x2) {
+    uint32_t d, f;
+    asm("v_pk_sub_u16 %0, %1, %2 clamp" : "=v"(d) : "v"(h), "s"(thrm1x2));
+    asm("v_pk_min_u16 %0, %1, %2" : "=v"(f) : "v"(d), "s"(0x00010001u));
+    return f;
+}
+template <int POS>
+__device__ __forceinline__ uint32_t keep_mask(uint32_t x) {
+    uint32_t m;
+    asm("v_bfe_i32 %0, %1, %2, 1" : "=v"(m) : "v"(x), "n"(POS));
+    return m;
+}
+__device__ __forceinline__ void keep_masks8(uint32_t kx, uint32_t (&m)[2][4]) {
+    m[0][0] = keep_mask<0>(kx); m[0][1] = keep_mask<16>(kx); m[0][2] = keep_mask<1>(kx); m[0][3] = keep_mask<17>(kx);
+    m[1][0] = keep_mask<2>(kx); m[1][1] = keep_mask<18>(kx); m[1][2] = keep_mask<3>(kx); m[1][3] = keep_mask<19>(kx);
+}
+__device__ __forceinline__ uint2 keep_pad_bits(int N, int g) {
+    auto below = [](int n) { n = n > 0 ? n : 0; const int rem = n & 15; return 2 * (n >> 4) + (rem > 0) + (rem > 2); };
+    const int jl = below(N - 4 * g), jh = below(N - 4 * g - 1);
+    const uint32_t ml = jl < 32 ? ~0u << jl : 0u, mh = jh < 32 ? ~0u << jh : 0u;
+    return make_uint2((ml & 0xFFFFu) | (mh << 16), (ml >> 16) | (mh & 0xFFFF0000u));
+}
 __device__ __forceinline__ bool keep1(uint32_t key32, uint32_t rowpair, int key, uint32_t thr16) {
     const uint32_t h = pair_hash(key32, rowpair + (key >> 1));
     return ((key & 1) ? (h >> 16) : (h & 0xFFFFu)) >= thr16;
diff --git a/uncertainty-vit_amd/csrc/engine.hip b/uncertainty-vit_amd/csrc/engine.hip
--- a/uncertainty-vit_amd/csrc/engine.hip
+++ b/uncertainty-vit_amd/csrc/engine.hip
@@ -106,6 +106,7 @@
 struct LayerActs {
     bf16 *ln1, *qkv, *attn, *projout, *ln2, *h, *a, *mlpout;
     float *mean1, *rstd1, *mean2, *rstd2, *lse;
+    void* keep = nullptr;
 };
 
 struct uvit_engine {
@@ -151,6 +152,9 @@
     size_t n_nd;
     bool slab_started;
     bool last_dropout; uint32_t last_seed;
+    bool keep_enable = true;
+    bool last_keep = false;
+    void* keep_pool = nullptr;
     int bwd_next = -1;
     int compact_R = 0;
     bool dual = true;
@@ -328,6 +332,11 @@
         hipMemcpyAsync(e->tdesc, td.data(), td.size() * sizeof(TransposeDesc), hipMemcpyHostToDevice, s) != hipSuccess ||
         hipStreamSynchronize(s) != hipSuccess) { delete e; return fail(UVIT_ERR_LAUNCH); }
     e->slab_started = false; e->last_dropout = false; e->last_seed = 0;
+    if (e->S == 1 && cfg->attn_drop_rate > 0.f) {
+        const size_t per = roundup(uvit_attn_keep_bytes(e->B, e->H, e->N), 256);
+        if (hipMalloc(&e->keep_pool, per * cfg->depth) != hipSuccess) { e->keep_pool = nullptr; delete e; return fail(UVIT_ERR_LAUNCH); }
+        for (int i = 0; i < cfg->depth; ++i) e->acts[i].keep = (char*)e->keep_pool + per * i;
+    }
     {
         const char* env = getenv("UVIT_SINGLE_STREAM");
         e->dual = !(env && env[0] == '1');
@@ -354,6 +363,7 @@
     if (e->ev_ds) (void)hipEventDestroy(e->ev_ds);
     if (e->ev_x) (void)hipEventDestroy(e->ev_x);
     for (int i = 0; i < UVIT_MAX_DEPTH; ++i) if (e->ev_wdone[i]) (void)hipEventDestroy(e->ev_wdone[i]);
+    if (e->keep_pool) (void)hipFree(e->keep_pool);
     delete e;
 }
 
@@ -390,6 +400,12 @@
 extern "C" int uvit_engine_set_drop_path_rows(uvit_engine* e, int on) {
     if (!e) return UVIT_ERR_ARG;
     e->dpl_enable = on != 0;
+    return UVIT_OK;
+}
+
+extern "C" int uvit_engine_set_attn_keep_bits(uvit_engine* e, int on) {
+    if (!e) return UVIT_ERR_ARG;
+    e->keep_enable = on != 0;
     return UVIT_OK;
 }
 
@@ -593,7 +609,7 @@
     }
     if (S == 1) {
         CHECK(uvit_attn_fwd_launch(a.qkv, p.biasP, a.attn, a.lse, at.K, e->H, e->N, e->NP, e->attn_scale, p.pdrop, p.aseed, (uint32_t)l, s, at.d[0].bmap,
-                                   e->head_dim));
+                                   e->head_dim, save && e->last_keep ? a.keep : nullptr));
     } else {
         CHECK(uvit_attn2_fwd_launch(a.qkv, a.qkv + Mp * 3 * C, p.biasP, a.attn, a.attn + Mp * C, a.lse, Bc, e->H, e->N, e->NP, 0.125f,
                                     p.pdrop, p.aseed, (uint32_t)l, s));
@@ -704,6 +720,7 @@
         e->dpl_on = false;
         if (p.dp_on && p.kind == PASS_STUDENT && e->dpl_enable && Bc == e->B) CHECK(dp_lists_begin(e, p.draw.seed, p.draw.it, Bc, s));
         e->last_dropout = p.draw.on; e->last_seed = p.aseed;
+        e->last_keep = e->keep_enable && p.kind == PASS_STUDENT;
     }
     const bool keep = p.kind != PASS_TEACHER;
     CHECK(embed(e, p.w, mask, keep ? e->X[0] : e->tX[0], Bc, s));
@@ -951,7 +968,8 @@
             if (at.mode == ROWS_LIST && ml.mode == ROWS_MASKED && at.red > at.rows)
                 CHECK(uvit_zero_launch(dqkv + (size_t)at.rows * 3 * C, (size_t)(at.red - at.rows) * 3 * C * sizeof(bf16), s));
             CHECK(uvit_attn_bwd_fused_launch(a.qkv, a.attn, e->dAttn, biasP, a.lse, e->delta, dqkv, dsw, dsw != nullptr, at.K, e->H,
-                                             e->N, e->NP, e->attn_scale, pdrop, e->last_seed, (uint32_t)l, s, at.d[0].bmap, e->head_dim));
+                                             e->N, e->NP, e->attn_scale, pdrop, e->last_seed, (uint32_t)l, s, at.d[0].bmap, e->head_dim,
+                                             e->last_keep ? a.keep : nullptr));
         } else {
             CHECK(uvit_attn2_bwd_launch(a.qkv, a.qkv + Mp * 3 * C, a.attn, a.attn + Mp * C, e->dAttn, e->dAttn + Mp * C, biasP, a.lse,
                                         e->delta, dqkv, dqkv + Mp * 3 * C, dsw, dsw != nullptr, e->B, e->H, e->N, e->NP, 0.125f, pdrop,
@@ -1153,6 +1171,25 @@
     if (slab) CHECK(uvit_attn_dbias_reduce_launch(ds_ws, slab, acc, B, H, N, NP, S(st)));
     return UVIT_OK;
 }
+extern "C" int64_t uvit_op_attn_keep_bytes(int B, int H, int N) {
+    if (B < 1 || H < 1 || N < 1 || N > 208) return UVIT_ERR_SHAPE;
+    return (int64_t)uvit_attn_keep_bytes(B, H, N);
+}
+extern "C" int uvit_op_attn_fwd_ex(const void* qkv, const float* biasP, void* out, float* lse, void* keep_bits, const int* bmap, int generic,
+                                   int B, int H, int N, int NP, int head_dim, float scale, float p_drop, uint32_t seed, uint32_t layer,
+                                   uvit_stream st) {
+    if (!qkv || !out || !lse) return UVIT_ERR_ARG;
+    if (head_dim != 64 && head_dim != 80) return UVIT_ERR_SHAPE;
+    return uvit_attn_fwd_launch(qkv, biasP, out, lse, B, H, N, NP, scale, p_drop, seed, layer, S(st), bmap, head_dim, keep_bits, generic != 0);
+}
+extern "C" int uvit_op_attn_bwd_ex(const void* qkv, const void* o_fwd, const void* d_o, const float* biasP, const float* lse, float* delta,
+                                   void* dqkv, void* ds_ws, const void* keep_bits, const int* bmap, int B, int H, int N, int NP, int head_dim,
+                                   float scale, float p_drop, uint32_t seed, uint32_t layer, uvit_stream st) {
+    if (!qkv || !o_fwd || !d_o || !lse || !delta || !dqkv) return UVIT_ERR_ARG;
+    if (head_dim != 64 && head_dim != 80) return UVIT_ERR_SHAPE;
+    return uvit_attn_bwd_fused_launch(qkv, o_fwd, d_o, biasP, lse, delta, dqkv, ds_ws, ds_ws != nullptr, B, H, N, NP, scale, p_drop, seed, layer,
+                                      S(st), bmap, head_dim, keep_bits);
+}
 extern "C" int uvit_op_attn2_fwd(const void* qkv_m, const void* qkv_c, const float* biasP, void* out_m, void* out_c, float* lse, int B,
                                  int H, int N, int NP, float scale, float p_drop, uint32_t seed, uint32_t layer, uvit_stream st) {
     if (!qkv_m || !qkv_c || !out_m || !out_c || !lse) return UVIT_ERR_ARG;
diff --git a/uncertainty-vit_amd/csrc/uvit_internal.h b/uncertainty-vit_amd/csrc/uvit_internal.h
--- a/uncertainty-vit_amd/csrc/uvit_internal.h
+++ b/uncertainty-vit_amd/csrc/uvit_internal.h
@@ -61,14 +61,16 @@
 bool uvit_gemm_tn_group_ok(const TnProb* probs, int n, const GemmTune* tune = nullptr);
 int uvit_gemm_tn_group_launch(const TnProb* probs, int n, hipStream_t s, const GemmTune* tune = nullptr);
 
+size_t uvit_attn_keep_bytes(int B, int H, int N);
 int uvit_attn_fwd_launch(const void* qkv, const float* biasP, void* out, float* lse, int B, int H, int N, int NP,
                          float scale, float p_drop, uint32_t seed, uint32_t layer, hipStream_t s, const int* bmap = nullptr,
-                         int head_dim = 64);
+                         int head_dim = 64,
+                         void* keep_bits = nullptr, bool generic = false);
 size_t uvit_attn_bwd_fused_ws_bytes(int B, int H, int N);
 int uvit_attn_bwd_fused_launch(const void* qkv, const void* o_fwd, const void* d_o, const float* biasP, const float* lse,
                                float* delta, void* dqkv, void* ds_ws, int want_ds, int B, int H, int N, int NP, float scale,
                                float p_drop, uint32_t seed, uint32_t layer, hipStream_t s, const int* bmap = nullptr,
-                               int head_dim = 64);
+                               int head_dim = 64, const void* keep_bits = nullptr);
 int uvit_attn_dbias_reduce_launch(const void* ds_ws, float* dbias_slab, int accumulate, int B, int H, int N, int NP, hipStream_t s);
 
 int uvit_attn2_fwd_launch(const void* qkv_m, const void* qkv_c, const float* biasP, void* out_m, void* out_c, float* lse,
diff --git a/uncertainty-vit_amd/modeling_cyclical.py b/uncertainty-vit_amd/modeling_cyclical.py
--- a/uncertainty-vit_amd/modeling_cyclical.py
+++ b/uncertainty-vit_amd/modeling_cyclical.py
@@ -98,6 +98,9 @@
         check(L.uvit_engine_set_streams(self.h, self.stream_mode), "set_streams")
         self.drop_path_rows = bool(getattr(model, "drop_path_rows", os.environ.get("UVIT_DP_ROWS", "1") != "0"))
         self.set_drop_path_rows(self.drop_path_rows)
+        self.attn_keep_bits = True
+        if not getattr(model, "attn_keep_bits", True):
+            self.set_attn_keep_bits(False)
         self.sync_shadows(3)
 
     @property
@@ -107,6 +110,10 @@
     def set_drop_path_rows(self, on):
         self.drop_path_rows = bool(on)
         check(lib().uvit_engine_set_drop_path_rows(self.h, 1 if on else 0), "set_drop_path_rows")
+
+    def set_attn_keep_bits(self, on):
+        self.attn_keep_bits = bool(on)
+        check(lib().uvit_engine_set_attn_keep_bits(self.h, 1 if on else 0), "set_attn_keep_bits")
 
     def sync_shadows(self, which=3):
         check(lib().uvit_engine_sync_shadows(self.h, which, cur_stream()), "sync_shadows")
diff --git a/uncertainty-vit_amd/native.py b/uncertainty-vit_amd/native.py
--- a/uncertainty-vit_amd/native.py
+++ b/uncertainty-vit_amd/native.py
@@ -132,6 +132,7 @@
     "uvit_op_wgrad_group": (_i, [_vp, _i, _vp, _vp]),
     "uvit_engine_set_streams": (_i, [_vp, _i]),
     "uvit_engine_set_drop_path_rows": (_i, [_vp, _i]),
+    "uvit_engine_set_attn_keep_bits": (_i, [_vp, _i]),
     "uvit_drop_path_kept_counts": (_i, [_i, _f, _i, _i, _u32, _u32, _vp]),
     "uvit_engine_profile": (_i, [_vp, _i, _i]),
     "uvit_engine_profile_read": (_i, [_vp, _vp, _vp, _vp]),
@@ -147,6 +148,9 @@
     "uvit_op_attn_bwd": (_i, [_vp, _vp, _vp, _vp, _vp, _vp, _vp, _vp, _i, _vp, _i, _i, _i, _i, _f, _f, _u32, _u32, _vp]),
     "uvit_op_attn_fwd_hd": (_i, [_vp, _vp, _vp, _vp, _i, _i, _i, _i, _i, _f, _f, _u32, _u32, _vp]),
     "uvit_op_attn_bwd_hd": (_i, [_vp, _vp, _vp, _vp, _vp, _vp, _vp, _vp, _i, _vp, _i, _i, _i, _i, _i, _f, _f, _u32, _u32, _vp]),
+    "uvit_op_attn_keep_bytes": (_i64, [_i, _i, _i]),
+    "uvit_op_attn_fwd_ex": (_i, [_vp] * 6 + [_i] * 6 + [_f, _f, _u32, _u32, _vp]),
+    "uvit_op_attn_bwd_ex": (_i, [_vp] * 10 + [_i] * 5 + [_f, _f, _u32, _u32, _vp]),
     "uvit_op_attn2_fwd": (_i, [_vp, _vp, _vp, _vp, _vp, _vp, _i, _i, _i, _i, _f, _f, _u32, _u32, _vp]),
     "uvit_op_attn2_bwd_ws_bytes": (_i64, [_i, _i, _i]),
     "uvit_op_attn2_bwd": (_i, [_vp] * 12 + [_i, _vp, _i, _i, _i, _i, _f, _f, _u32, _u32, _vp]),
```

After: 5584, median of 2. About the same (-0.0%).
